# OpenGene/gencore

Measured on AMD Instinct MI355X. Metric: consensus read-pairs/sec (whole node) + clustering HBM GB/s vs roofline, higher is better.
Workload: dtype u8

## Files before the change

gencore_amd/csrc/engine.hip:

```cpp
#include <hip/hip_runtime.h>
#include <hip/hip_ext.h>
#include <cstdio>
#include <cstdlib>
#include <algorithm>
#include <cstring>
#include <ctime>
#include <string>
#include <vector>

#include "gce_entry.h"
#include "gce_kernels.hpp"
#include "gce_params.hpp"
#include "gce_pair2.hpp"
#include "gce_vote.hpp"
#include "gce_deep.hpp"
#include "gce_output.hpp"
#include "gce_depth.hpp"
#include "gce_inflate.hpp"
#include "gce_deflate.hpp"

namespace {

static thread_local double t_alloc_s = 0.0; static thread_local long t_alloc_n = 0; static thread_local size_t t_alloc_bytes = 0;
static inline double mono_s() { struct timespec ts; clock_gettime(CLOCK_MONOTONIC, &ts); return (double)ts.tv_sec + 1e-9 * (double)ts.tv_nsec; }
long long g_dev_live = 0, g_dev_peak = 0;
static int64_t g_pass_idx_ctr[4] = {0, 0, 0, 0};
inline void dev_bytes_add(long long d) {
    const long long now = __atomic_add_fetch(&g_dev_live, d, __ATOMIC_RELAXED);
    long long pk = __atomic_load_n(&g_dev_peak, __ATOMIC_RELAXED);
    while (now > pk && !__atomic_compare_exchange_n(&g_dev_peak, &pk, now, true, __ATOMIC_RELAXED, __ATOMIC_RELAXED)) {}
}
struct DevBuf {
    void *p = nullptr; size_t cap = 0;
    static size_t padded(size_t bytes) { return bytes + bytes / 8 + 256; }
    hipError_t ensure(size_t bytes) { return bytes <= cap && p ? hipSuccess : take(padded(bytes)); }
    hipError_t take(size_t want) {
        const double t0 = mono_s();
        release();
        hipError_t e = hipMalloc(&p, want);
        if (e == hipSuccess) { cap = want; dev_bytes_add((long long)want); } else p = nullptr;
        t_alloc_s += mono_s() - t0; t_alloc_n++; t_alloc_bytes += want;
        return e;
    }
    void release() { if (p) { (void)hipFree(p); dev_bytes_add(-(long long)cap); } p = nullptr; cap = 0; }
    template <class T> T *as() const { return (T *)p; }
};
struct ScopedBuf : DevBuf { ~ScopedBuf() { release(); } };
template <class T> inline hipError_t ensure_as(DevBuf &d, T *&dst, size_t bytes) { const hipError_t r = d.ensure(bytes); dst = d.as<T>(); return r; }

enum { EV_START = 0, EV_CLUSTER, EV_CSR, EV_DESCRIBE, EV_PAIRING, EV_SCORE, EV_CONSENSUS, EV_FINISH, EV_OUTPUT, EV_COUNT };

}

#include "gce_devstream.hpp"

struct HostRaw {
    uint8_t *p = nullptr; size_t n = 0, cap = 0;
    ~HostRaw() { free(p); }
    void resize(size_t k) { if (k > cap) { free(p); p = (uint8_t *)malloc(k ? k : 1); cap = p ? k : 0; } n = p ? k : 0; }
    uint8_t *data() { return p; }
    size_t size() const { return n; }
    bool empty() const { return n == 0; }
};

struct gce_engine {
    gce_params prm{};
    bool vote_off_logged = false;
    std::vector<uint32_t> target_len;
    std::string err;
    hipStream_t stream = nullptr;
    hipEvent_t ev[EV_COUNT]{};
    std::vector<DevBuf> ref_buf; std::vector<const uint8_t *> ref_ptr; std::vector<int64_t> ref_len, ref_win; bool have_win = false;
    DevBuf d_ref_ptr, d_ref_len, d_ref_win, d_target_len, d_target_cum;
    std::vector<const uint8_t *> up_ref_ptr; std::vector<int64_t> up_ref_len, up_win; std::vector<uint32_t> up_tl; const void *up_dev[5]{}; bool up_valid = false;
    std::vector<gce_core> h_core; std::vector<uint64_t> h_qoff, h_coff, h_soff, h_loff, h_mioff;
    std::vector<char> h_qname, h_mi; std::vector<uint32_t> h_cigar; std::vector<uint8_t> h_seq, h_qual, h_nmt; std::vector<int32_t> h_nm; std::vector<uint64_t> h_tick;
    std::vector<int32_t> h_ev_tid, h_ev_pos;
    bool have_mi = false, have_tick = false, have_events = false, host_mode = false, device_mode = false, processed = false;
    bool reserved = false; hipStream_t up_stream = nullptr; std::vector<hipEvent_t> up_events;
    hipStream_t aux_stream = nullptr; hipEvent_t aux_ev[4]{};
    size_t rs_n = 0, rs_q = 0, rs_c = 0, rs_s = 0, rs_l = 0, st_n = 0, st_q = 0, st_c = 0, st_s = 0, st_l = 0, st_m = 0; bool dev_concat = false;
    gce_batch dev_batch{};
    DevBuf b_core, b_qoff, b_qname, b_coff, b_cigar, b_soff, b_seq, b_loff, b_qual, b_nm, b_nmt, b_mioff, b_mi, b_tick;
    DevBuf uinfo, rdesc, spatch, slot, score, out_flag, orec, out_index, nmx;
    DevBuf o_src, o_kind, o_qsrc, o_nm, o_fr, o_rr, o_mate, o_soff, o_qoff, o_seq, o_qual, o_key, o_rec, o_ksoff, o_kqoff, o_krow, o_rank64, o_part3, ref_ascii;
    int64_t n_out = 0; size_t out_seq_bytes = 0, out_qual_bytes = 0; int dev_error = 0; uint32_t dev_error_read = 0;
    DevBuf lrec, lout, bhdr, blk_base, ev_tid, ev_pos, ev_read, table, toff;
    DevBuf raw, rw_tmp, rw_ncig, rw_nmpos, rw_rsize, rw_roff, rw_body; RecIdx rw;
    size_t raw_n = 0; bool raw_mode = false; int64_t raw_records = 0; uint64_t raw_body_bytes = 0;
    int64_t idx_ctr[4] = {0, 0, 0, 0};
    DevBuf z_comp, z_dir, z_err; size_t z_n = 0; std::vector<InfDir> z_members;
    DevBuf zo_slots, zo_sizes, zo_off, zo_out; uint64_t zo_bytes = 0;
    DevBuf sf_text; uint64_t sf_bytes = 0; int64_t raw_body_nrec = -1;
    std::vector<gce_engine *> mirrors;
    DevBuf sh_tickall, sh_shard, sh_flag, sh_sel, sh_core, sh_qoff, sh_coff, sh_soff, sh_loff, sh_nm, sh_nmt, sh_mioff, sh_tick, sh_roff, sh_nmpos, sh_keys, sh_stage; int64_t shard_n = -1;
    bool shard_cut_done = false;
    bool tab_clean = false; const void *tab_clean_ptr = nullptr; size_t tab_clean_cap = 0;
    DevBuf cl_ikey, cl_start, cl_n, cl_npairs, cl_ngroups, cl_gbase, cl_nresult, cl_hasumi, cl_tier;
    DevBuf members, sorted, pl, pr, pu, pg, gpl, gpr, grp_begin, grp_n, gl_cluster, g_begin, g_np;
    DevBuf slow_args, deep_list, k64, slow_list, left_list, pf_flag, pf_list, pq_flag, pq_list, p16_flag, p16_list, pd_slab, gen_flag, gen_list, score_list, gw, vlive, vb_start, rp_left, rp_right, rp_merge, rp_rmerge, rp_umi, rp_umilen, rp_state, rp_supp, rp_nm, rp_qsl, rp_qsr, scan_part, si;
    StreamInfo h_si{};
    void *si_pin = nullptr, *si_pin_dev = nullptr; unsigned long long si_seq = 0;
    gce_timing timing{};
    int64_t n = 0, n_pre = 0;
    DevBuf dp_binoff, dp_regoff, dp_rs, dp_re, dp_pmax, dp_sorted, dp_depth, dp_bed, dp_where;
    std::vector<int64_t> h_binoff, h_depth_pre, h_depth_post, h_bed_pre, h_bed_post; int64_t payload_words = 0;
    std::vector<uint8_t> r_kind; HostRaw r_seq, r_qual; std::vector<uint32_t> r_src, r_qsrc, r_mate; std::vector<int32_t> r_nm; std::vector<int16_t> r_fr, r_rr;
    std::vector<uint64_t> r_soff, r_qoff;
};

static int fail(gce_engine *e, int code, const std::string &msg) { if (e) e->err = msg; return code; }
#define HIPCHK(call) do { hipError_t _e = (call); if (_e != hipSuccess) return fail(e, _e == hipErrorOutOfMemory ? GCE_ERR_OOM : GCE_ERR_HIP, std::string(#call) + ": " + hipGetErrorString(_e)); } while (0)

extern "C" {

int gce_abi_version(void) { return GCE_ABI_VERSION; }

void gce_params_default(gce_params *p) {
    memset(p, 0, sizeof *p);
    p->abi_version = GCE_ABI_VERSION;
    p->proper_umi_diff_threshold = 1; p->unproper_umi_diff_threshold = 0; p->duplex_mismatch_threshold = 2;
    p->cluster_size_req = 1; p->base_score_req = 6; p->high_quality = 30; p->moderate_quality = 20; p->low_quality = 15;
    p->score_high = 8; p->score_moderate = 6; p->score_low = 4; p->score_bad = 2;
    p->skip_low_complexity_cluster_threshold = 1000; p->flush_period = 10000; p->score_percent_req = 0.8;
}

void gce_detect_umi_prefix(const char *q, char out[32]) {
    memset(out, 0, 32);
    if (strstr(q, "umi_")) strcpy(out, "umi");
    else if (strstr(q, "UMI_")) strcpy(out, "UMI");
}

const char *gce_status_message(int s) {
    switch (s) {
    case GCE_OK: return "ok";
    case GCE_ERR_INVALID: return "invalid argument or call order";
    case GCE_ERR_NO_DEVICE: return "no HIP device available (this engine has no CPU fallback)";
    case GCE_ERR_HIP: return "HIP runtime error";
    case GCE_ERR_OOM: return "out of device memory";
    case GCE_ERR_UNSORTED: return "ERROR: the input is unsorted. Please sort the input first.";
    case GCE_ERR_UMI_MISMATCH: return "The UMI of a read pair should be identical";
    case GCE_ERR_NM_MISSING: return "NM tag missing on a consensus template whose mismatch count changed";
    case GCE_ERR_UMI_PARSE: return "UMI parse: substr start beyond the end of the read name";
    case GCE_ERR_QNAME_SHORT: return "copyQName ERROR: desitination qname is shorter";
    case GCE_ERR_REF_WINDOW: return "reference window: a clustered read lies outside the bases staged for its contig";
    default: return "unknown status";
    }
}

const char *gce_last_error(const gce_engine *e) { return e ? e->err.c_str() : "null engine"; }

int gce_create(const gce_params *params, gce_engine **out) {
    if (!params || !out || params->abi_version != GCE_ABI_VERSION) return GCE_ERR_INVALID;
    if (params->proper_umi_diff_threshold < 0 || params->unproper_umi_diff_threshold < 0 || params->flush_period < 0) return GCE_ERR_INVALID;
    int ndev = 0;
    if (hipGetDeviceCount(&ndev) != hipSuccess || ndev <= 0 || params->device >= ndev) return GCE_ERR_NO_DEVICE;
    gce_engine *e = new gce_engine();
    e->prm = *params;
    if (e->prm.flush_period == 0) e->prm.flush_period = 10000;
    if (params->n_targets > 0 && params->target_len) e->target_len.assign(params->target_len, params->target_len + params->n_targets);
    e->prm.target_len = nullptr;
    if (hipSetDevice(params->device) != hipSuccess || hipStreamCreate(&e->stream) != hipSuccess) { delete e; return GCE_ERR_HIP; }
    for (auto &v : e->ev) (void)hipEventCreate(&v);
    *out = e;
    return GCE_OK;
}

void gce_destroy(gce_engine *e) {
    if (!e) return;
    (void)hipSetDevice(e->prm.device);
    (void)hipStreamSynchronize(e->stream);
    DevBuf *all[] = {&e->d_ref_ptr, &e->d_ref_len, &e->d_ref_win, &e->d_target_len, &e->d_target_cum, &e->b_core, &e->b_qoff, &e->b_qname, &e->b_coff, &e->b_cigar, &e->b_soff,
                     &e->b_seq, &e->b_loff, &e->b_qual, &e->b_nm, &e->b_nmt, &e->b_mioff, &e->b_mi, &e->b_tick, &e->uinfo, &e->rdesc, &e->spatch,
                     &e->slot, &e->score, &e->out_flag, &e->orec, &e->out_index, &e->nmx, &e->o_src, &e->o_kind, &e->o_qsrc, &e->o_nm, &e->o_fr, &e->o_rr, &e->o_mate,
                     &e->o_key, &e->o_rec, &e->o_ksoff, &e->o_kqoff, &e->o_krow, &e->o_rank64, &e->o_part3, &e->o_soff, &e->o_qoff, &e->o_seq, &e->o_qual, &e->ref_ascii, &e->lrec, &e->lout, &e->bhdr,
                     &e->blk_base, &e->ev_tid, &e->ev_pos, &e->ev_read, &e->table, &e->toff, &e->cl_ikey, &e->cl_start, &e->cl_n,
                     &e->cl_npairs, &e->cl_ngroups, &e->cl_gbase, &e->cl_nresult, &e->cl_hasumi, &e->cl_tier, &e->members, &e->sorted, &e->pl, &e->pr, &e->pu,
                     &e->pg, &e->gpl, &e->gpr, &e->grp_begin, &e->grp_n, &e->gl_cluster, &e->g_begin, &e->g_np, &e->deep_list, &e->k64, &e->slow_list, &e->pf_flag, &e->pf_list, &e->pq_flag, &e->pq_list, &e->left_list, &e->slow_args, &e->pd_slab, &e->gen_flag, &e->gen_list, &e->score_list, &e->gw, &e->vlive, &e->vb_start, &e->rp_left, &e->rp_right, &e->rp_merge, &e->rp_rmerge,
                     &e->rp_umi, &e->rp_umilen, &e->rp_state, &e->rp_supp, &e->rp_nm, &e->rp_qsl, &e->rp_qsr, &e->scan_part, &e->si};
    for (auto *b : all) b->release();
    for (DevBuf *b : {&e->z_comp, &e->z_dir, &e->z_err, &e->raw, &e->rw_tmp, &e->rw_ncig, &e->rw_nmpos, &e->rw_rsize, &e->rw_roff, &e->rw_body, &e->sf_text}) b->release();
    e->rw.release();
    for (DevBuf *b : {&e->zo_slots, &e->zo_sizes, &e->zo_off, &e->zo_out, &e->p16_flag, &e->p16_list}) b->release();
    for (DevBuf *b : {&e->sh_tickall, &e->sh_shard, &e->sh_flag, &e->sh_sel, &e->sh_core, &e->sh_qoff, &e->sh_coff, &e->sh_soff, &e->sh_loff, &e->sh_nm, &e->sh_nmt, &e->sh_mioff, &e->sh_tick, &e->sh_roff, &e->sh_nmpos, &e->sh_keys, &e->sh_stage}) b->release();
    for (DevBuf *b : {&e->dp_binoff, &e->dp_regoff, &e->dp_rs, &e->dp_re, &e->dp_pmax, &e->dp_sorted, &e->dp_depth, &e->dp_bed, &e->dp_where}) b->release();
    for (auto ev : e->up_events) (void)hipEventDestroy(ev);
    if (e->up_stream) { (void)hipStreamSynchronize(e->up_stream); (void)hipStreamDestroy(e->up_stream); }
    if (e->aux_stream) { (void)hipStreamSynchronize(e->aux_stream); (void)hipStreamDestroy(e->aux_stream); }
    for (auto &v : e->aux_ev) if (v) (void)hipEventDestroy(v);
    for (auto &b : e->ref_buf) b.release();
    for (auto &v : e->ev) if (v) (void)hipEventDestroy(v);
    if (e->stream) (void)hipStreamDestroy(e->stream);
    if (e->si_pin) (void)hipHostFree(e->si_pin);
    delete e;
}

void gce_pack_reference(const char *bases, int64_t n, uint8_t *out) {
    memset(out, 0, (size_t)((n + 1) / 2));
    for (int64_t i = 0; i < n; i++) {
        uint8_t code;
        switch (bases[i]) { case 'A': code = 1; break; case 'T': code = 2; break; case 'C': code = 3; break; case 'G': code = 4; break; default: code = 0; }
        out[i >> 1] |= (i & 1) ? (uint8_t)(code << 4) : code;
    }
}

int gce_set_reference(gce_engine *e, int32_t tid, const uint8_t *nibbles, int64_t n_bases) {
    if (!e || tid < 0 || n_bases < 0) return GCE_ERR_INVALID;
    (void)hipSetDevice(e->prm.device);
    if ((size_t)tid >= e->ref_buf.size()) { e->ref_buf.resize(tid + 1); e->ref_ptr.resize(tid + 1, nullptr); e->ref_len.resize(tid + 1, 0); }
    if (!nibbles) { e->ref_ptr[tid] = nullptr; e->ref_len[tid] = 0; return GCE_OK; }
    size_t bytes = (size_t)((n_bases + 1) / 2);
    HIPCHK(e->ref_buf[tid].ensure(bytes + 16));
    hipPointerAttribute_t attr; bool is_dev = hipPointerGetAttributes(&attr, nibbles) == hipSuccess && attr.type == hipMemoryTypeDevice;
    (void)hipGetLastError();
    HIPCHK(hipMemcpyAsync(e->ref_buf[tid].p, nibbles, bytes, is_dev ? hipMemcpyDeviceToDevice : hipMemcpyHostToDevice, e->stream));
    HIPCHK(hipStreamSynchronize(e->stream));
    e->ref_ptr[tid] = e->ref_buf[tid].as<uint8_t>(); e->ref_len[tid] = n_bases;
    if (2 * (size_t)tid + 1 < e->ref_win.size()) e->ref_win[2 * tid] = e->ref_win[2 * tid + 1] = 0;
    return GCE_OK;
}

int gce_set_reference_ascii(gce_engine *e, int32_t tid, const char *bases, int64_t n_bases) {
    if (!e || tid < 0 || n_bases < 0 || (!bases && n_bases > 0)) return GCE_ERR_INVALID;
    (void)hipSetDevice(e->prm.device);
    if ((size_t)tid >= e->ref_buf.size()) { e->ref_buf.resize(tid + 1); e->ref_ptr.resize(tid + 1, nullptr); e->ref_len.resize(tid + 1, 0); }
    const size_t bytes = (size_t)((n_bases + 1) / 2);
    HIPCHK(e->ref_buf[tid].ensure(bytes + 16));
    HIPCHK(e->ref_ascii.ensure((size_t)n_bases + 16));
    hipPointerAttribute_t attr; const bool is_dev = hipPointerGetAttributes(&attr, bases) == hipSuccess && attr.type == hipMemoryTypeDevice;
    (void)hipGetLastError();
    if (n_bases) {
        HIPCHK(hipMemcpyAsync(e->ref_ascii.p, bases, (size_t)n_bases, is_dev ? hipMemcpyDeviceToDevice : hipMemcpyHostToDevice, e->stream));
        const unsigned grid = (unsigned)std::min<uint64_t>((bytes + 255) / 256, 65535u * 4u);
        hipLaunchKernelGGL(k_pack_reference, dim3(grid), dim3(256), 0, e->stream, (const char *)e->ref_ascii.p, n_bases, e->ref_buf[tid].as<uint8_t>());
    }
    HIPCHK(hipStreamSynchronize(e->stream));
    HIPCHK(hipGetLastError());
    e->ref_ptr[tid] = e->ref_buf[tid].as<uint8_t>(); e->ref_len[tid] = n_bases;
    if (2 * (size_t)tid + 1 < e->ref_win.size()) e->ref_win[2 * tid] = e->ref_win[2 * tid + 1] = 0;
    return GCE_OK;
}

int gce_set_reference_window(gce_engine *e, int32_t tid, int64_t contig_len, int64_t win_start, const char *bases, int64_t n_bases) {
    if (!e || tid < 0 || contig_len < 0 || win_start < 0 || (win_start & 1) || n_bases < 0 || win_start + n_bases > contig_len || (!bases && n_bases > 0)) return GCE_ERR_INVALID;
    const int rc = gce_set_reference_ascii(e, tid, bases, n_bases);
    if (rc != GCE_OK) return rc;
    if (e->ref_win.size() < 2 * e->ref_ptr.size()) e->ref_win.resize(2 * e->ref_ptr.size(), 0);
    e->ref_ptr[tid] = e->ref_buf[tid].as<uint8_t>() - (win_start >> 1);
    e->ref_len[tid] = contig_len;
    e->ref_win[2 * tid] = win_start; e->ref_win[2 * tid + 1] = win_start + n_bases;
    e->have_win = true;
    return GCE_OK;
}

int gce_reset(gce_engine *e) {
    if (!e) return GCE_ERR_INVALID;
    e->h_core.clear(); e->h_qoff.clear(); e->h_coff.clear(); e->h_soff.clear(); e->h_loff.clear(); e->h_mioff.clear(); e->h_tick.clear();
    e->h_qname.clear(); e->h_mi.clear(); e->h_cigar.clear(); e->h_seq.clear(); e->h_qual.clear(); e->h_nmt.clear(); e->h_nm.clear();
    e->have_mi = e->have_tick = e->host_mode = e->device_mode = e->processed = e->raw_mode = false; e->n = 0; e->n_out = 0; e->shard_n = -1; e->shard_cut_done = false;
    e->st_n = e->st_q = e->st_c = e->st_s = e->st_l = e->st_m = 0; e->dev_concat = false;
    return GCE_OK;
}

int gce_set_flush_events(gce_engine *e, int32_t n_events, const int32_t *ev_tid, const int32_t *ev_pos) {
    if (!e || n_events < 0 || (n_events > 0 && (!ev_tid || !ev_pos))) return GCE_ERR_INVALID;
    e->h_ev_tid.assign(ev_tid, ev_tid + n_events); e->h_ev_pos.assign(ev_pos, ev_pos + n_events);
    e->have_events = true;
    return GCE_OK;
}

struct PreExtra { long long v[6]; };
__global__ void k_fold_stats(StreamInfo *si, PreExtra x) {
    const int k = threadIdx.x;
    if (k < 6) {
        long long a = 0, c = 0;
        for (int q = 0; q < GCE_PRE_SLOTS; q++) { a += si->pre_slot[q][k]; c += si->post_slot[q][k]; si->pre_slot[q][k] = 0; si->post_slot[q][k] = 0; }
        si->pre[k] += a + x.v[k]; si->post[k] += c;
    }
}
__global__ void k_first_contig_ge(const gce_core *core, int64_t n, int32_t maxc, unsigned int *out) {
    const int64_t i = (int64_t)blockIdx.x * blockDim.x + threadIdx.x;
    const bool hit = i < n && core[i].tid >= maxc;
    const unsigned long long m = __ballot(hit);
    if (m && (threadIdx.x & 63) == 0) { const unsigned int v = (unsigned int)(i + __ffsll((long long)m) - 1); if (v < *(volatile unsigned int *)out) atomicMin(out, v); }
}

__global__ void k_add_u64(uint64_t *a, uint64_t n, uint64_t base) {
    const uint64_t i = (uint64_t)blockIdx.x * blockDim.x + threadIdx.x;
    if (i < n) a[i] += base;
}

int gce_reserve(gce_engine *e, int64_t n_reads, size_t qname_bytes, size_t cigar_words, size_t seq_bytes, size_t qual_bytes) {
    if (!e || n_reads < 0) return GCE_ERR_INVALID;
    if (e->processed) gce_reset(e);
    if (e->host_mode || e->device_mode) return fail(e, GCE_ERR_INVALID, "gce_reserve after a submit");
    (void)hipSetDevice(e->prm.device);
    const size_t n = (size_t)n_reads;
    HIPCHK(e->b_core.ensure(n * sizeof(gce_core) + 64)); HIPCHK(e->b_qoff.ensure(n * 8 + 64)); HIPCHK(e->b_coff.ensure(n * 8 + 64));
    HIPCHK(e->b_soff.ensure(n * 8 + 64)); HIPCHK(e->b_loff.ensure(n * 8 + 64)); HIPCHK(e->b_nm.ensure(n * 4 + 64)); HIPCHK(e->b_nmt.ensure(n + 64));
    HIPCHK(e->b_qname.ensure(qname_bytes + 64)); HIPCHK(e->b_cigar.ensure(cigar_words * 4 + 64)); HIPCHK(e->b_seq.ensure(seq_bytes + 64)); HIPCHK(e->b_qual.ensure(qual_bytes + 64));
    if (!e->up_stream) HIPCHK(hipStreamCreate(&e->up_stream));
    e->reserved = true; e->rs_n = n; e->rs_q = qname_bytes; e->rs_c = cigar_words; e->rs_s = seq_bytes; e->rs_l = qual_bytes;
    e->st_n = e->st_q = e->st_c = e->st_s = e->st_l = 0;
    return GCE_OK;
}

static hipError_t grow_keep(DevBuf &d, size_t used, size_t need, hipStream_t s) {
    if (d.p && need <= d.cap) return hipSuccess;
    DevBuf nb;
    hipError_t rc = nb.ensure(need + need / 2 + 256);
    if (rc != hipSuccess) return rc;
    if (used && d.p && (rc = hipMemcpyAsync(nb.p, d.p, used, hipMemcpyDeviceToDevice, s)) != hipSuccess) { nb.release(); return rc; }
    if ((rc = hipStreamSynchronize(s)) != hipSuccess) { nb.release(); return rc; }
    d.release(); d = nb;
    return hipSuccess;
}
__global__ void k_rebase_mioff(uint64_t *a, uint64_t n, uint64_t base) {
    const uint64_t i = (uint64_t)blockIdx.x * blockDim.x + threadIdx.x;
    if (i < n && a[i] != 0xFFFFFFFFFFFFFFFFull) a[i] += base;
}

static int append_batch(gce_engine *e, const gce_batch *b, hipMemcpyKind kind) {
    const size_t n = (size_t)b->n_reads;
    if (!n) return GCE_OK;
    if (!b->core || !b->qname_off || !b->qname || !b->cigar_off || !b->seq_off || !b->seq || !b->qual_off || !b->qual || !b->nm || !b->nm_type)
        return fail(e, GCE_ERR_INVALID, "null array in gce_batch");
    if (e->st_n > 0 && (b->tick != nullptr) != e->have_tick) return fail(e, GCE_ERR_INVALID, "gce_batch.tick must be given for every batch of a stream or for none");
    if (!e->up_stream) HIPCHK(hipStreamCreate(&e->up_stream));
    hipStream_t s = e->up_stream;
    const bool mi = b->mi && b->mi_off;
    HIPCHK(grow_keep(e->b_core, e->st_n * sizeof(gce_core), (e->st_n + n) * sizeof(gce_core) + 64, s)); HIPCHK(grow_keep(e->b_nm, e->st_n * 4, (e->st_n + n) * 4 + 64, s)); HIPCHK(grow_keep(e->b_nmt, e->st_n, e->st_n + n + 64, s));
    HIPCHK(grow_keep(e->b_qoff, e->st_n * 8, (e->st_n + n) * 8 + 64, s)); HIPCHK(grow_keep(e->b_coff, e->st_n * 8, (e->st_n + n) * 8 + 64, s));
    HIPCHK(grow_keep(e->b_soff, e->st_n * 8, (e->st_n + n) * 8 + 64, s)); HIPCHK(grow_keep(e->b_loff, e->st_n * 8, (e->st_n + n) * 8 + 64, s));
    HIPCHK(grow_keep(e->b_qname, e->st_q, e->st_q + b->qname_bytes + 64, s)); HIPCHK(grow_keep(e->b_cigar, e->st_c * 4, (e->st_c + b->cigar_words) * 4 + 64, s));
    HIPCHK(grow_keep(e->b_seq, e->st_s, e->st_s + b->seq_bytes + 64, s)); HIPCHK(grow_keep(e->b_qual, e->st_l, e->st_l + b->qual_bytes + 64, s));
    auto cp = [&](DevBuf &d, size_t at, const void *src, size_t bytes) { return bytes ? hipMemcpyAsync((char *)d.p + at, src, bytes, kind, s) : hipSuccess; };
    HIPCHK(cp(e->b_core, e->st_n * sizeof(gce_core), b->core, n * sizeof(gce_core)));
    HIPCHK(cp(e->b_nm, e->st_n * 4, b->nm, n * 4)); HIPCHK(cp(e->b_nmt, e->st_n, b->nm_type, n));
    HIPCHK(cp(e->b_qoff, e->st_n * 8, b->qname_off, n * 8)); HIPCHK(cp(e->b_coff, e->st_n * 8, b->cigar_off, n * 8));
    HIPCHK(cp(e->b_soff, e->st_n * 8, b->seq_off, n * 8)); HIPCHK(cp(e->b_loff, e->st_n * 8, b->qual_off, n * 8));
    HIPCHK(cp(e->b_qname, e->st_q, b->qname, b->qname_bytes)); HIPCHK(cp(e->b_cigar, e->st_c * 4, b->cigar, b->cigar_words * 4));
    HIPCHK(cp(e->b_seq, e->st_s, b->seq, b->seq_bytes)); HIPCHK(cp(e->b_qual, e->st_l, b->qual, b->qual_bytes));
    const unsigned nb = (unsigned)((n + 255) / 256);
    if (e->st_q) hipLaunchKernelGGL(k_add_u64, dim3(nb), dim3(256), 0, s, e->b_qoff.as<uint64_t>() + e->st_n, (uint64_t)n, (uint64_t)e->st_q);
    if (e->st_c) hipLaunchKernelGGL(k_add_u64, dim3(nb), dim3(256), 0, s, e->b_coff.as<uint64_t>() + e->st_n, (uint64_t)n, (uint64_t)e->st_c);
    if (e->st_s) hipLaunchKernelGGL(k_add_u64, dim3(nb), dim3(256), 0, s, e->b_soff.as<uint64_t>() + e->st_n, (uint64_t)n, (uint64_t)e->st_s);
    if (e->st_l) hipLaunchKernelGGL(k_add_u64, dim3(nb), dim3(256), 0, s, e->b_loff.as<uint64_t>() + e->st_n, (uint64_t)n, (uint64_t)e->st_l);
    if (b->tick) {
        HIPCHK(grow_keep(e->b_tick, e->st_n * 8, (e->st_n + n) * 8 + 64, s));
        HIPCHK(cp(e->b_tick, e->st_n * 8, b->tick, n * 8));
        e->have_tick = true;
    }
    if (mi || e->have_mi) {
        const bool first = !e->have_mi;
        HIPCHK(grow_keep(e->b_mioff, first ? 0 : e->st_n * 8, (e->st_n + n) * 8 + 64, s));
        if (first && e->st_n) HIPCHK(hipMemsetAsync(e->b_mioff.p, 0xFF, e->st_n * 8, s));
        if (mi) {
            HIPCHK(grow_keep(e->b_mi, e->st_m, e->st_m + b->mi_bytes + 64, s));
            HIPCHK(cp(e->b_mioff, e->st_n * 8, b->mi_off, n * 8)); HIPCHK(cp(e->b_mi, e->st_m, b->mi, b->mi_bytes));
            if (e->st_m) hipLaunchKernelGGL(k_rebase_mioff, dim3(nb), dim3(256), 0, s, e->b_mioff.as<uint64_t>() + e->st_n, (uint64_t)n, (uint64_t)e->st_m);
            e->st_m += b->mi_bytes;
        } else HIPCHK(hipMemsetAsync((char *)e->b_mioff.p + e->st_n * 8, 0xFF, n * 8, s));
        e->have_mi = true;
    }
    e->st_n += n; e->st_q += b->qname_bytes; e->st_c += b->cigar_words; e->st_s += b->seq_bytes; e->st_l += b->qual_bytes;
    return GCE_OK;
}
static void publish_own_copy(gce_engine *e) {
    gce_batch &d = e->dev_batch; memset(&d, 0, sizeof d);
    d.n_reads = (int64_t)e->st_n; d.core = e->b_core.as<gce_core>();
    d.qname_off = e->b_qoff.as<uint64_t>(); d.qname = e->b_qname.as<char>(); d.cigar_off = e->b_coff.as<uint64_t>(); d.cigar = e->b_cigar.as<uint32_t>();
    d.seq_off = e->b_soff.as<uint64_t>(); d.seq = e->b_seq.as<uint8_t>(); d.qual_off = e->b_loff.as<uint64_t>(); d.qual = e->b_qual.as<uint8_t>();
    d.nm = e->b_nm.as<int32_t>(); d.nm_type = e->b_nmt.as<uint8_t>();
    d.qname_bytes = e->st_q; d.cigar_words = e->st_c; d.seq_bytes = e->st_s; d.qual_bytes = e->st_l;
    if (e->have_mi) { d.mi_off = e->b_mioff.as<uint64_t>(); d.mi = e->b_mi.as<char>(); d.mi_bytes = e->st_m; }
    if (e->have_tick) d.tick = e->b_tick.as<uint64_t>();
}

int gce_submit_async(gce_engine *e, const gce_batch *b, int32_t *ticket) {
    if (!e || !b || b->n_reads < 0) return GCE_ERR_INVALID;
    if (!e->reserved) return fail(e, GCE_ERR_INVALID, "gce_submit_async needs gce_reserve");
    if (e->device_mode && !e->processed) return fail(e, GCE_ERR_INVALID, "gce_submit after gce_submit_device");
    if (e->processed) gce_reset(e);
    (void)hipSetDevice(e->prm.device);
    e->host_mode = true;
    int rc = append_batch(e, b, hipMemcpyHostToDevice);
    if (rc != GCE_OK) return rc;
    hipEvent_t ev;
    HIPCHK(hipEventCreateWithFlags(&ev, hipEventDisableTiming));
    HIPCHK(hipEventRecord(ev, e->up_stream));
    e->up_events.push_back(ev);
    if (ticket) *ticket = (int32_t)e->up_events.size() - 1;
    return GCE_OK;
}

int gce_submit_wait(gce_engine *e, int32_t ticket) {
    if (!e || ticket < 0 || (size_t)ticket >= e->up_events.size()) return GCE_ERR_INVALID;
    HIPCHK(hipEventSynchronize(e->up_events[ticket]));
    for (gce_engine *m : e->mirrors)
        if ((size_t)ticket < m->up_events.size() && hipEventSynchronize(m->up_events[ticket]) != hipSuccess) return fail(e, GCE_ERR_HIP, "mirror engine: copy failed");
    return GCE_OK;
}

int gce_submit(gce_engine *e, const gce_batch *b) {
    if (!e || !b || b->n_reads < 0) return GCE_ERR_INVALID;
    if (e->device_mode && !e->processed) return fail(e, GCE_ERR_INVALID, "gce_submit after gce_submit_device");
    if (e->reserved) {
        int32_t t; int rc = gce_submit_async(e, b, &t);
        return rc != GCE_OK ? rc : gce_submit_wait(e, t);
    }
    if (e->processed) gce_reset(e);
    e->host_mode = true;
    const int64_t n = b->n_reads;
    if (n == 0) return GCE_OK;
    if (!b->core || !b->qname_off || !b->qname || !b->cigar_off || !b->seq_off || !b->seq || !b->qual_off || !b->qual || !b->nm || !b->nm_type)
        return fail(e, GCE_ERR_INVALID, "null array in gce_batch");
    const size_t old = e->h_core.size();
    if (old > 0 && (b->tick != nullptr) != e->have_tick) return fail(e, GCE_ERR_INVALID, "gce_batch.tick must be given for every batch of a stream or for none");
    const uint64_t q0 = e->h_qname.size(), c0 = e->h_cigar.size(), s0 = e->h_seq.size(), l0 = e->h_qual.size(), m0 = e->h_mi.size();
    e->h_core.insert(e->h_core.end(), b->core, b->core + n);
    e->h_nm.insert(e->h_nm.end(), b->nm, b->nm + n);
    e->h_nmt.insert(e->h_nmt.end(), b->nm_type, b->nm_type + n);
    e->h_qname.insert(e->h_qname.end(), b->qname, b->qname + b->qname_bytes);
    if (b->cigar_words) e->h_cigar.insert(e->h_cigar.end(), b->cigar, b->cigar + b->cigar_words);
    e->h_seq.insert(e->h_seq.end(), b->seq, b->seq + b->seq_bytes);
    e->h_qual.insert(e->h_qual.end(), b->qual, b->qual + b->qual_bytes);
    if (b->tick) { e->h_tick.insert(e->h_tick.end(), b->tick, b->tick + n); e->have_tick = true; }
    bool mi = b->mi && b->mi_off;
    if (mi && !e->have_mi) { e->h_mioff.assign(old, UINT64_MAX); e->have_mi = true; }
    if (mi) e->h_mi.insert(e->h_mi.end(), b->mi, b->mi + b->mi_bytes);
    e->h_qoff.reserve(old + n); e->h_coff.reserve(old + n); e->h_soff.reserve(old + n); e->h_loff.reserve(old + n);
    for (int64_t i = 0; i < n; i++) {
        e->h_qoff.push_back(b->qname_off[i] + q0); e->h_coff.push_back(b->cigar_off[i] + c0);
        e->h_soff.push_back(b->seq_off[i] + s0); e->h_loff.push_back(b->qual_off[i] + l0);
        if (e->have_mi) e->h_mioff.push_back(mi && b->mi_off[i] != UINT64_MAX ? b->mi_off[i] + m0 : UINT64_MAX);
    }
    return GCE_OK;
}

int gce_submit_device(gce_engine *e, const gce_batch *b) {
    if (!e || !b || b->n_reads < 0) return GCE_ERR_INVALID;
    if (e->processed) gce_reset(e);
    if (e->host_mode) return fail(e, GCE_ERR_INVALID, "gce_submit_device after gce_submit");
    (void)hipSetDevice(e->prm.device);
    if (!e->device_mode) {
        e->device_mode = true; e->dev_concat = false;
        e->dev_batch = *b;
        e->have_tick = b->tick != nullptr;
        return GCE_OK;
    }
    int rc;
    if (!e->dev_concat) {
        const gce_batch first = e->dev_batch;
        e->st_n = e->st_q = e->st_c = e->st_s = e->st_l = e->st_m = 0; e->have_tick = false; e->have_mi = false;
        if ((rc = append_batch(e, &first, hipMemcpyDeviceToDevice)) != GCE_OK) return rc;
        e->dev_concat = true;
    }
    if ((rc = append_batch(e, b, hipMemcpyDeviceToDevice)) != GCE_OK) return rc;
    HIPCHK(hipStreamSynchronize(e->up_stream));
    publish_own_copy(e);
    return GCE_OK;
}

static int upload(gce_engine *e) {
    if (e->reserved) {
        HIPCHK(hipStreamSynchronize(e->up_stream));
        for (auto ev : e->up_events) (void)hipEventDestroy(ev);
        e->up_events.clear();
        publish_own_copy(e);
        return GCE_OK;
    }
    struct { DevBuf *d; const void *src; size_t bytes; const void **dst; } items[] = {
        {&e->b_core, e->h_core.data(), e->h_core.size() * sizeof(gce_core), (const void **)&e->dev_batch.core},
        {&e->b_qoff, e->h_qoff.data(), e->h_qoff.size() * 8, (const void **)&e->dev_batch.qname_off},
        {&e->b_qname, e->h_qname.data(), e->h_qname.size(), (const void **)&e->dev_batch.qname},
        {&e->b_coff, e->h_coff.data(), e->h_coff.size() * 8, (const void **)&e->dev_batch.cigar_off},
        {&e->b_cigar, e->h_cigar.data(), e->h_cigar.size() * 4, (const void **)&e->dev_batch.cigar},
        {&e->b_soff, e->h_soff.data(), e->h_soff.size() * 8, (const void **)&e->dev_batch.seq_off},
        {&e->b_seq, e->h_seq.data(), e->h_seq.size(), (const void **)&e->dev_batch.seq},
        {&e->b_loff, e->h_loff.data(), e->h_loff.size() * 8, (const void **)&e->dev_batch.qual_off},
        {&e->b_qual, e->h_qual.data(), e->h_qual.size(), (const void **)&e->dev_batch.qual},
        {&e->b_nm, e->h_nm.data(), e->h_nm.size() * 4, (const void **)&e->dev_batch.nm},
        {&e->b_nmt, e->h_nmt.data(), e->h_nmt.size(), (const void **)&e->dev_batch.nm_type},
        {&e->b_mioff, e->h_mioff.data(), e->h_mioff.size() * 8, (const void **)&e->dev_batch.mi_off},
        {&e->b_mi, e->h_mi.data(), e->h_mi.size(), (const void **)&e->dev_batch.mi},
        {&e->b_tick, e->h_tick.data(), e->h_tick.size() * 8, (const void **)&e->dev_batch.tick},
    };
    for (auto &it : items) {
        HIPCHK(it.d->ensure(it.bytes + 64));
        if (it.bytes) HIPCHK(hipMemcpyAsync(it.d->p, it.src, it.bytes, hipMemcpyHostToDevice, e->stream));
        *it.dst = it.bytes ? it.d->p : nullptr;
    }
    if (!e->have_mi) { e->dev_batch.mi = nullptr; e->dev_batch.mi_off = nullptr; }
    if (!e->have_tick) e->dev_batch.tick = nullptr;
    e->dev_batch.n_reads = (int64_t)e->h_core.size();
    e->dev_batch.qname_bytes = e->h_qname.size(); e->dev_batch.cigar_words = e->h_cigar.size();
    e->dev_batch.seq_bytes = e->h_seq.size(); e->dev_batch.qual_bytes = e->h_qual.size(); e->dev_batch.mi_bytes = e->h_mi.size();
    if (e->h_cigar.empty()) e->dev_batch.cigar = e->b_cigar.as<uint32_t>();
    return GCE_OK;
}

__global__ __launch_bounds__(256) void k_publish_si(const StreamInfo *si, StreamInfo *host, unsigned long long *flag, unsigned long long seq) {
    const uint32_t *src = reinterpret_cast<const uint32_t *>(si);
    uint32_t *dst = reinterpret_cast<uint32_t *>(host);
    for (unsigned i = threadIdx.x; i < sizeof(StreamInfo) / 4; i += 256) dst[i] = src[i];
    __threadfence_system();
    __syncthreads();
    if (threadIdx.x == 0) __hip_atomic_store(flag, seq, __ATOMIC_RELEASE, __HIP_MEMORY_SCOPE_SYSTEM);
}
static_assert(sizeof(StreamInfo) % 4 == 0, "k_publish_si copies words");
static int read_si_begin(gce_engine *e, unsigned long long *seq_out) {
    *seq_out = 0;
    static const bool sync_copy = getenv("GCE_SYNC_COPY") != nullptr;
    if (!sync_copy && !e->si_pin) {
        void *hp = nullptr;
        if (hipHostMalloc(&hp, sizeof(StreamInfo) + 64, hipHostMallocMapped | hipHostMallocCoherent | hipHostMallocPortable) == hipSuccess) {
            void *dp = nullptr;
            if (hipHostGetDevicePointer(&dp, hp, 0) == hipSuccess) { memset(hp, 0, sizeof(StreamInfo) + 64); e->si_pin = hp; e->si_pin_dev = dp; }
            else (void)hipHostFree(hp);
        }
        (void)hipGetLastError();
    }
    if (!sync_copy && e->si_pin) {
        unsigned long long *dflag = reinterpret_cast<unsigned long long *>(reinterpret_cast<char *>(e->si_pin_dev) + ((sizeof(StreamInfo) + 7) & ~size_t(7)));
        const unsigned long long seq = ++e->si_seq;
        hipLaunchKernelGGL(k_publish_si, dim3(1), dim3(256), 0, e->stream, (const StreamInfo *)e->si.p, reinterpret_cast<StreamInfo *>(e->si_pin_dev), dflag, seq);
        HIPCHK(hipGetLastError());
        *seq_out = seq;
    }
    return GCE_OK;
}
static int read_si_end(gce_engine *e, unsigned long long seq) {
    bool published = false;
    if (seq) {
        StreamInfo *hs = reinterpret_cast<StreamInfo *>(e->si_pin);
        unsigned long long *hflag = reinterpret_cast<unsigned long long *>(reinterpret_cast<char *>(e->si_pin) + ((sizeof(StreamInfo) + 7) & ~size_t(7)));
        for (unsigned spins = 1;; spins++) {
            if (__atomic_load_n(hflag, __ATOMIC_ACQUIRE) == seq) { published = true; break; }
            if ((spins & 0x3FFF) == 0) {
                const hipError_t q = hipStreamQuery(e->stream);
                if (q == hipSuccess) { published = __atomic_load_n(hflag, __ATOMIC_ACQUIRE) == seq; break; }
                if (q != hipErrorNotReady) HIPCHK(q);
            }
            __builtin_ia32_pause();
        }
        if (published) memcpy(&e->h_si, hs, sizeof(StreamInfo));
    }
    if (!published) {
        HIPCHK(hipMemcpyAsync(&e->h_si, e->si.p, sizeof(StreamInfo), hipMemcpyDeviceToHost, e->stream));
        HIPCHK(hipStreamSynchronize(e->stream));
    }
    for (int k = 0; k < 6; k++) for (int q = 0; q < GCE_PRE_SLOTS; q++) { e->h_si.pre[k] += e->h_si.pre_slot[q][k]; e->h_si.post[k] += e->h_si.post_slot[q][k]; }
    if (e->h_si.err_key != ~0ull) { e->dev_error = -(int)(e->h_si.err_key & 0xFF); e->dev_error_read = (uint32_t)(e->h_si.err_key >> 8); }
    return GCE_OK;
}
static int read_si(gce_engine *e) {
    unsigned long long seq = 0;
    const int rc = read_si_begin(e, &seq);
    return rc != GCE_OK ? rc : read_si_end(e, seq);
}

static inline unsigned cdiv(uint64_t a, uint64_t b) { return (unsigned)((a + b - 1) / b); }
static const bool g_record_events = getenv("GCE_RECORD_EVENTS") != nullptr;
#define LAUNCH_EV(kernel, grid, block, stream, ev, ...) do { \
    if (g_record_events) { hipLaunchKernelGGL(kernel, grid, block, 0, stream, __VA_ARGS__); (void)hipEventRecord(ev, stream); } \
    else hipExtLaunchKernelGGL(kernel, grid, block, 0, stream, nullptr, ev, 0, __VA_ARGS__); } while (0)

struct FillSeg { void *p; uint64_t bytes; uint32_t val; uint32_t pad; };
struct FillArgs { FillSeg s[6]; };
__global__ __launch_bounds__(256) void k_fill_many(FillArgs a) {
    const FillSeg g = a.s[blockIdx.y];
    const uint64_t n16 = g.bytes >> 4;
    const uint32_t v = g.val * 0x01010101u;
    uint4 *q = reinterpret_cast<uint4 *>(g.p);
    for (uint64_t i = (uint64_t)blockIdx.x * 256 + threadIdx.x; i < n16; i += (uint64_t)gridDim.x * 256) q[i] = make_uint4(v, v, v, v);
    if (blockIdx.x == 0 && threadIdx.x < (g.bytes & 15)) reinterpret_cast<uint8_t *>(g.p)[(n16 << 4) + threadIdx.x] = (uint8_t)g.val;
}
static void fill_many(hipStream_t s, std::initializer_list<FillSeg> segs) {
    FillArgs a{}; int n = 0; uint64_t mx = 0;
    for (const FillSeg &g : segs) { a.s[n++] = g; mx = std::max<uint64_t>(mx, g.bytes); }
    const unsigned gx = (unsigned)std::min<uint64_t>(std::max<uint64_t>((mx >> 4) / (256 * 8), 1), 2048);
    hipLaunchKernelGGL(k_fill_many, dim3(gx, (unsigned)n), dim3(256), 0, s, a);
}

static int aux_ready(gce_engine *e) {
    if (e->aux_stream) return GCE_OK;
    HIPCHK(hipStreamCreateWithFlags(&e->aux_stream, hipStreamNonBlocking));
    for (auto &v : e->aux_ev) HIPCHK(hipEventCreateWithFlags(&v, hipEventDisableTiming));
    return GCE_OK;
}

#ifdef GCE_SI_CANARY
static void si_canary(gce_engine *e, const char *phase) {
    StreamInfo hs; (void)hipStreamSynchronize(e->stream); (void)hipMemcpy(&hs, e->si.p, sizeof hs, hipMemcpyDeviceToHost);
    for (int k = 14; k < GCE_STATS_WORDS; k++) if ((k != 15 && hs.post[k] != 0) || hs.pre[k] < 0 || hs.post[k] < 0) { fprintf(stderr, "SI_CANARY after %s: pre[%d] = %lld post[%d] = %lld\n", phase, k, hs.pre[k], k, hs.post[k]); break; }
}
#define CANARY(x) si_canary(e, x)
#else
#define CANARY(x) do { } while (0)
#endif

static int gce_process_impl(gce_engine *e);
int gce_process(gce_engine *e) {
    static const bool tlog = getenv("GCE_RAW_TIMING") != nullptr;
    if (!tlog) return gce_process_impl(e);
    const double a0 = t_alloc_s, w0 = mono_s(); const long n0 = t_alloc_n; const size_t b0 = t_alloc_bytes;
    const int rc = gce_process_impl(e);
    fprintf(stderr, "gce_process (device %d): %.4f s wall, of it %.4f s in %ld hipMalloc / hipFree calls for %.2f GB; kernels %.1f ms\n", e ? e->prm.device : -1, mono_s() - w0, t_alloc_s - a0, t_alloc_n - n0,
            (double)(t_alloc_bytes - b0) / 1e9, e ? e->timing.total_ms : 0.0);
    return rc;
}
#define TAKE(buf, dst, bytes) HIPCHK(ensure_as(e->buf, dst, bytes))
namespace {
struct Step {
    gce_engine *const e; const hipStream_t s; const gce_batch &hb;
    DevBatch b{}; DevParams p{}; Work w{}; OutTable o{};
    int64_t N = 0; size_t n1 = 1; uint32_t C = 0, NG = 0;
    PreExtra pre_extra{};
    int64_t n_sblk = 0, max_events = 0; unsigned nblk_N = 0;
    bool si_behind_describe = false;
    explicit Step(gce_engine *e_) : e(e_), s(e_->stream), hb(e_->dev_batch) {}

    int check_and_cut() {
        if (!e->host_mode && !e->device_mode) return fail(e, GCE_ERR_INVALID, "nothing submitted");
        if (e->processed) return fail(e, GCE_ERR_INVALID, "gce_process called twice without a new submit (the stream was mutated in place)");
        if (e->have_tick && !e->have_events) return fail(e, GCE_ERR_INVALID, "gce_batch.tick needs gce_set_flush_events");
        (void)hipSetDevice(e->prm.device);
        int rc;
        if (e->host_mode && (rc = upload(e)) != GCE_OK) return rc;
        N = hb.n_reads;
        e->n_pre = N;
        if (e->prm.max_contig > 0 && N > 0 && !e->shard_cut_done) {
            HIPCHK(e->si.ensure(sizeof(StreamInfo)));
            unsigned int first = NONE32;
            HIPCHK(hipMemcpyAsync(e->si.p, &first, 4, hipMemcpyHostToDevice, s));
            hipLaunchKernelGGL(k_first_contig_ge, dim3((unsigned)((N + 255) / 256)), dim3(256), 0, s, hb.core, N, e->prm.max_contig, (unsigned int *)e->si.p);
            HIPCHK(hipMemcpyAsync(&first, e->si.p, 4, hipMemcpyDeviceToHost, s));
            HIPCHK(hipStreamSynchronize(s));
            if (first != NONE32) {
                gce_core c2; int32_t nm = 0; uint8_t nmt = 0;
                HIPCHK(hipMemcpy(&c2, hb.core + first, sizeof(gce_core), hipMemcpyDeviceToHost));
                HIPCHK(hipMemcpy(&nm, hb.nm + first, 4, hipMemcpyDeviceToHost)); HIPCHK(hipMemcpy(&nmt, hb.nm_type + first, 1, hipMemcpyDeviceToHost));
                const int mism = nmt != 0 ? nm : 0;
                pre_extra.v[0] = 1; pre_extra.v[1] = c2.l_qseq; pre_extra.v[4] = mism; pre_extra.v[5] = mism > 0;
                N = (int64_t)first; e->n_pre = N + 1;
            }
        }
        e->n = N; e->n_out = 0; e->out_seq_bytes = e->out_qual_bytes = 0; e->dev_error = 0; e->dev_error_read = 0;
        e->processed = true;
        memset(&e->timing, 0, sizeof e->timing);
        memset(&e->h_si, 0, sizeof e->h_si);
        if (N >= (int64_t)0xFFFFFC00ll) return fail(e, GCE_ERR_INVALID, "more than 2^32 reads in one engine");
        if ((uint64_t)(VB_MINW + 3) * (uint64_t)(N > 0 ? N : 0) >= (1ull << 32)) return fail(e, GCE_ERR_INVALID, "too many reads in one engine for the batch scan of k_vote (weight sum >= 2^32)");
        n1 = (size_t)(N > 0 ? N : 1);
        b.n = N; b.core = hb.core; b.qname_off = hb.qname_off; b.qname = hb.qname; b.cigar_off = hb.cigar_off; b.cigar = hb.cigar;
        b.seq_off = hb.seq_off; b.seq = hb.seq; b.qual_off = hb.qual_off; b.qual = hb.qual; b.nm = hb.nm; b.nm_type = hb.nm_type;
        b.mi_off = hb.mi_off; b.mi = hb.mi; b.tick = e->have_tick ? hb.tick : nullptr;
        return GCE_OK;
    }

    int stage_constants() {
        const int nref = (int)e->ref_ptr.size();
        HIPCHK(e->d_ref_ptr.ensure((size_t)(nref + 1) * 8)); HIPCHK(e->d_ref_len.ensure((size_t)(nref + 1) * 8));
        HIPCHK(e->d_target_len.ensure(e->target_len.size() * 4 + 4));
        HIPCHK(e->d_target_cum.ensure(e->target_len.size() * 8 + 8));
        std::vector<int64_t> win;
        if (e->have_win && nref) {
            win.assign(2 * (size_t)nref, 0);
            for (int t = 0; t < nref; t++) { const bool wd = 2 * (size_t)t + 1 < e->ref_win.size() && e->ref_win[2 * t + 1] > 0; win[2 * t] = wd ? e->ref_win[2 * t] : 0; win[2 * t + 1] = wd ? e->ref_win[2 * t + 1] : e->ref_len[t]; }
            HIPCHK(e->d_ref_win.ensure(win.size() * 8));
        }
        const void *dev_now[5] = {e->d_ref_ptr.p, e->d_ref_len.p, e->d_target_len.p, e->d_target_cum.p, e->d_ref_win.p};
        const bool same = e->up_valid && e->up_ref_ptr == e->ref_ptr && e->up_ref_len == e->ref_len && e->up_tl == e->target_len && e->up_win == win && memcmp(dev_now, e->up_dev, sizeof dev_now) == 0;
        if (!same) {
            e->up_valid = false;
            if (nref) {
                HIPCHK(hipMemcpyAsync(e->d_ref_ptr.p, e->ref_ptr.data(), (size_t)nref * 8, hipMemcpyHostToDevice, s));
                HIPCHK(hipMemcpyAsync(e->d_ref_len.p, e->ref_len.data(), (size_t)nref * 8, hipMemcpyHostToDevice, s));
            }
            std::vector<uint64_t> cum(e->target_len.size()); uint64_t acc = 0;
            for (size_t i = 0; i < cum.size(); i++) { cum[i] = acc; acc += e->target_len[i]; }
            if (!e->target_len.empty()) {
                HIPCHK(hipMemcpyAsync(e->d_target_len.p, e->target_len.data(), e->target_len.size() * 4, hipMemcpyHostToDevice, s));
                HIPCHK(hipMemcpyAsync(e->d_target_cum.p, cum.data(), cum.size() * 8, hipMemcpyHostToDevice, s));
            }
            if (!win.empty()) HIPCHK(hipMemcpyAsync(e->d_ref_win.p, win.data(), win.size() * 8, hipMemcpyHostToDevice, s));
            HIPCHK(hipStreamSynchronize(s));
            e->up_ref_ptr = e->ref_ptr; e->up_ref_len = e->ref_len; e->up_tl = e->target_len; e->up_win = win; memcpy(e->up_dev, dev_now, sizeof dev_now);
            e->up_valid = true;
        }
        p.target_len = e->d_target_len.as<uint32_t>(); p.target_cum = e->target_len.empty() ? nullptr : e->d_target_cum.as<uint64_t>();
        p.n_ref = nref; p.ref_data = e->d_ref_ptr.as<const uint8_t *>(); p.ref_len = e->d_ref_len.as<int64_t>(); p.ref_win = win.empty() ? nullptr : e->d_ref_win.as<int64_t>();
        return GCE_OK;
    }

    int size_by_reads() {
        const uint64_t T = ((uint64_t)n1 + (uint64_t)n1 / 4 + 2 * SCAN_TILE - 1) / SCAN_TILE * SCAN_TILE;
        const char *vote_off_why = nullptr;
        if (make_dev_params(e->prm, e->target_len, e->have_tick, N, T, &p, &vote_off_why) != GCE_OK) return fail(e, GCE_ERR_INVALID, "score constants out of range");
        if (vote_off_why && !e->vote_off_logged) {
            e->vote_off_logged = true;
            fprintf(stderr, "gencore_amd: k_vote off for this engine (%s): every group goes to the per-side kernels\n", vote_off_why);
        }
        n_sblk = (N + SB_READS - 1) / SB_READS;
        w.n_sblk = n_sblk;
        max_events = e->have_tick ? (int64_t)e->h_ev_tid.size() + 2 : (p.tick_offset % p.period + N) / p.period + 2;
        w.max_events = (int)max_events;
        w.tsize = T; w.tinv = 1.0 / (double)T;
        const size_t qual_bytes = hb.qual_bytes ? hb.qual_bytes : 1;
        const size_t nsb1 = (size_t)(n_sblk > 0 ? n_sblk : 1);
        TAKE(uinfo, w.uinfo, n1 * 8); TAKE(rdesc, w.rdesc, n1 * sizeof(ReadDescP)); TAKE(spatch, w.spatch, n1 * 4); TAKE(slot, w.slot, n1 * 4 + 16); TAKE(score, w.score, qual_bytes + 64);
        TAKE(out_flag, w.out_flag, n1 + 144);        TAKE(nmx, w.nmx, n1 * 4); TAKE(orec, w.orec, n1 * sizeof(OutRec)); TAKE(out_index, w.out_index, n1 * 4);
        TAKE(lrec, w.lrec, nsb1 * SB_READS * sizeof(LeadRec)); TAKE(lout, w.lout, nsb1 * SB_READS * sizeof(LeadOut));
        TAKE(bhdr, w.bhdr, nsb1 * sizeof(BlkHdr)); TAKE(blk_base, w.blk_base, nsb1 * 4);
        TAKE(ev_tid, w.ev_tid, (size_t)max_events * 4); TAKE(ev_pos, w.ev_pos, (size_t)max_events * 4); TAKE(ev_read, w.ev_read, (size_t)max_events * 4);
        TAKE(table, w.tab, T * sizeof(TabEntry)); TAKE(toff, w.toff, T * 4);
        TAKE(k64, w.k64, n1 * 24); TAKE(members, w.members, n1 * 4); TAKE(sorted, w.sorted, n1 * 4); TAKE(pl, w.pl, n1 * 4); TAKE(pr, w.pr, n1 * 4); TAKE(pu, w.pu, n1 * 4); TAKE(pg, w.pg, n1 * 4);
        TAKE(gpl, w.gpl, n1 * 4); TAKE(gpr, w.gpr, n1 * 4); TAKE(grp_begin, w.grp_begin, n1 * 4); TAKE(grp_n, w.grp_n, n1 * 4); TAKE(slow_list, w.slow_list, n1 * 4 + 64);
        TAKE(deep_list, w.deep_list, (n1 / 64 + 64) * 16);
        nblk_N = cdiv(n1, SCAN_TILE);
        TAKE(scan_part, w.scan_part, std::max<size_t>(2 * nsb1, (size_t)2 * nblk_N) * 8 + 16);
        TAKE(si, w.si, sizeof(StreamInfo));
        TAKE(cl_ikey, w.cl_ikey, n1 * 4); TAKE(cl_start, w.cl_start, n1 * 4); TAKE(cl_n, w.cl_n, n1 * 4);

        StreamInfo init{}; init.first_unmapped = NONE32; init.err_key = ~0ull; init.lq_min = 0x7FFFFFFF; init.lq_max = -1;
        if (e->have_tick) { init.n_events = init.n_events_a = (int)e->h_ev_tid.size(); }
        HIPCHK(hipMemcpyAsync(e->si.p, &init, sizeof init, hipMemcpyHostToDevice, s));
        if (e->have_tick && !e->h_ev_tid.empty()) {
            HIPCHK(hipMemcpyAsync(e->ev_tid.p, e->h_ev_tid.data(), e->h_ev_tid.size() * 4, hipMemcpyHostToDevice, s));
            HIPCHK(hipMemcpyAsync(e->ev_pos.p, e->h_ev_pos.data(), e->h_ev_pos.size() * 4, hipMemcpyHostToDevice, s));
        }
        if (!e->tab_clean || e->tab_clean_ptr != e->table.p || e->tab_clean_cap != e->table.cap) {
            HIPCHK(hipMemsetAsync(e->table.p, 0, e->table.cap, s));
            e->tab_clean_ptr = e->table.p; e->tab_clean_cap = e->table.cap;
        }
        e->tab_clean = false;
        HIPCHK(hipEventRecord(e->ev[EV_START], s));
        HIPCHK(hipMemsetAsync(e->out_flag.p, 0, n1, s));
        return GCE_OK;
    }

    int form_clusters() {
        if (N > 0) LAUNCH_EV(k_cluster, dim3((unsigned)n_sblk), dim3(SB_T), s, e->ev[EV_CLUSTER], b, p, w);
#ifdef CL_PROF
        dump_cluster_prof();
#endif
        if (N <= 0) HIPCHK(hipEventRecord(e->ev[EV_CLUSTER], s));
        CANARY("EV_CLUSTER");
        if (N > 0) {
            if (!e->have_tick) {
                hipLaunchKernelGGL(k_blk_scan, dim3(1), dim3(1024), 0, s, w, p);
                hipLaunchKernelGGL(k_events, dim3(cdiv(max_events, EV_T / 64)), dim3(EV_T), 0, s, b, p, w);
            }
            const unsigned nb4 = cdiv(n_sblk, 4);
            hipLaunchKernelGGL(k_leaders, dim3(nb4), dim3(256), 0, s, b, p, w);
            hipLaunchKernelGGL(k_num_reduce, dim3(nb4), dim3(256), 0, s, w, p.nw_cb);
            hipLaunchKernelGGL(k_scan_partials, dim3(1), dim3(1024), 0, s, w.scan_part, (uint64_t)nb4, &w.si->n_clusters, (unsigned long long *)nullptr);
            hipLaunchKernelGGL(k_num_apply, dim3(nb4), dim3(256), 0, s, w);
            LAUNCH_EV(k_scatter, dim3((unsigned)n_sblk), dim3(SB_T), s, e->ev[EV_CSR], N, w);
        } else HIPCHK(hipEventRecord(e->ev[EV_CSR], s));
        CANARY("EV_CSR");
        return GCE_OK;
    }

    int describe() {
        int rc;
        unsigned long long si_seq1 = 0;
        if ((rc = read_si_begin(e, &si_seq1)) != GCE_OK) return rc;
        if (N > 0) {
#ifndef GCE_DESCRIBE_BLOCKS
#define GCE_DESCRIBE_BLOCKS 32768
#endif
            const int64_t n_tiles = (N + 255) / 256;
            int tpb = (int)((n_tiles + GCE_DESCRIBE_BLOCKS - 1) / GCE_DESCRIBE_BLOCKS); if (tpb < 1) tpb = 1;
            LAUNCH_EV(k_describe, dim3(cdiv(n_tiles, tpb)), dim3(256), s, e->ev[EV_DESCRIBE], b, p, w, tpb);
        } else HIPCHK(hipEventRecord(e->ev[EV_DESCRIBE], s));
        CANARY("EV_DESCRIBE");
        if ((rc = read_si_end(e, si_seq1)) != GCE_OK) return rc;
        HIPCHK(hipGetLastError());
        e->tab_clean = true;
        C = (uint32_t)e->h_si.n_clusters;
        const size_t c1 = C ? C : 1;
        TAKE(cl_npairs, w.cl_npairs, c1 * 4); TAKE(cl_ngroups, w.cl_ngroups, c1 * 4); TAKE(cl_gbase, w.cl_gbase, c1 * 4); TAKE(cl_nresult, w.cl_nresult, c1 * 4);
        TAKE(cl_hasumi, w.cl_hasumi, c1); TAKE(cl_tier, w.cl_tier, c1);
        return GCE_OK;
    }

    void compact_flags(uint8_t *flag, uint32_t *list, unsigned long long *count) {
        const unsigned nbc = cdiv(C, SCAN_TILE);
        hipLaunchKernelGGL(k_flag_reduce, dim3(nbc), dim3(256), 0, s, (const uint8_t *)flag, (uint64_t)C, w.scan_part);
        hipLaunchKernelGGL(k_scan_partials, dim3(1), dim3(1024), 0, s, w.scan_part, (uint64_t)nbc, count, (unsigned long long *)nullptr);
        hipLaunchKernelGGL(k_flag_apply, dim3(nbc), dim3(256), 0, s, (const uint8_t *)flag, (uint64_t)C, (const uint64_t *)w.scan_part, list);
    }

    int pair_clusters() {
        if (!(C > 0 && e->dev_error == 0)) { HIPCHK(hipEventRecord(e->ev[EV_PAIRING], s)); return GCE_OK; }
        int rc;
        const size_t c1 = C;
        TAKE(left_list, w.left_list, c1 * 4 + 64);
        TAKE(pf_flag, w.pf_flag, c1 + 64); TAKE(pf_list, w.pf_list, c1 * 4); TAKE(pq_flag, w.pq_flag, c1 + 64); TAKE(pq_list, w.pq_list, c1 * 4); TAKE(p16_flag, w.p16_flag, c1 + 64); TAKE(p16_list, w.p16_list, c1 * 4);
        const bool pair_classes = (double)N > 10.0 * (double)C;
        if (!pair_classes) fill_many(s, {FillSeg{e->pf_flag.p, c1, 0u, 0u}, FillSeg{e->pq_flag.p, c1, 0u, 0u}});
        const unsigned nbc = cdiv(C, SCAN_TILE);
#ifdef PS_STOP
        return time_pairing_sub_and_stop();
#endif
        HIPCHK(e->pd_slab.ensure(PD_BIG_BLOCKS * PD_SLAB));
        if (pair_classes) {
            hipLaunchKernelGGL(k_pair_class_reduce, dim3(nbc), dim3(256), 0, s, (const uint32_t *)w.cl_n, C, w.scan_part);
            hipLaunchKernelGGL(k_scan_partials, dim3(1), dim3(1024), 0, s, w.scan_part, (uint64_t)nbc, &w.si->n_p16_items, &w.si->n_pq_items);
            hipLaunchKernelGGL(k_pair_class_apply, dim3(nbc), dim3(256), 0, s, (const uint32_t *)w.cl_n, C, (const uint64_t *)w.scan_part, w.p16_list, w.pq_list, w.pf_list, w.si);
            static const bool tiers_aux = getenv("GCE_NO_AUX_STREAM") == nullptr;
            hipStream_t s2 = s;
            if (tiers_aux) {
                if ((rc = aux_ready(e)) != GCE_OK) return rc;
                s2 = e->aux_stream;
                HIPCHK(hipEventRecord(e->aux_ev[0], s));
                HIPCHK(hipStreamWaitEvent(s2, e->aux_ev[0], 0));
            }
            hipLaunchKernelGGL(k_pairing_fast, dim3(2048), dim3(256), 0, s2, b, p, w, C, (const uint32_t *)w.pf_list);
            hipLaunchKernelGGL(k_pairing_deep<false>, dim3(256), dim3(PD_T), 0, s2, b, p, w, (uint8_t *)nullptr);
            if (tiers_aux) HIPCHK(hipEventRecord(e->aux_ev[1], s2));
            hipLaunchKernelGGL(k_pairing_sub<16>, dim3(cdiv(C, 4 * WAVES_PER_BLOCK)), dim3(256), 0, s, b, p, w, C, (const uint32_t *)w.p16_list, (const unsigned long long *)&w.si->n_p16_items, w.pq_flag, 1);
            hipLaunchKernelGGL(k_pairing_sub<32>, dim3(cdiv(C, 2 * WAVES_PER_BLOCK)), dim3(256), 0, s, b, p, w, C, (const uint32_t *)w.pq_list, (const unsigned long long *)&w.si->n_pq_items, w.pf_flag, 1);
            if (tiers_aux) HIPCHK(hipStreamWaitEvent(s, e->aux_ev[1], 0));
        } else {
            hipLaunchKernelGGL(k_pairing_sub<16>, dim3(cdiv(C, 4 * WAVES_PER_BLOCK)), dim3(256), 0, s, b, p, w, C, (const uint32_t *)nullptr, (const unsigned long long *)nullptr, w.pq_flag, 0);
            compact_flags(w.pq_flag, w.pq_list, &w.si->n_pq_items);
            hipLaunchKernelGGL(k_pairing_sub<32>, dim3(cdiv(C, 2 * WAVES_PER_BLOCK)), dim3(256), 0, s, b, p, w, C, (const uint32_t *)w.pq_list, (const unsigned long long *)&w.si->n_pq_items, w.pf_flag, 0);
            compact_flags(w.pf_flag, w.pf_list, &w.si->n_pf_items);
            hipLaunchKernelGGL(k_pairing_fast, dim3(2048), dim3(256), 0, s, b, p, w, C, (const uint32_t *)w.pf_list);
            hipLaunchKernelGGL(k_pairing_deep<false>, dim3(256), dim3(PD_T), 0, s, b, p, w, (uint8_t *)nullptr);
        }
        hipLaunchKernelGGL(k_pairing_deep<true>, dim3(PD_BIG_BLOCKS), dim3(PD_T), 0, s, b, p, w, e->pd_slab.as<uint8_t>());
        hipLaunchKernelGGL(k_pairing_slow<0>, dim3(1024), dim3(256), 0, s, b, p, w);
        hipLaunchKernelGGL(k_pairing_slow<1>, dim3(1024, 16), dim3(256), 0, s, b, p, w);
        hipLaunchKernelGGL(k_pairing_slow<2>, dim3(1024), dim3(256), 0, s, b, p, w);
        hipLaunchKernelGGL(k_scan_reduce, dim3(nbc), dim3(256), 0, s, (const uint32_t *)w.cl_ngroups, (uint64_t)C, w.scan_part);
        hipLaunchKernelGGL(k_scan_partials, dim3(1), dim3(1024), 0, s, w.scan_part, (uint64_t)nbc, &w.si->n_pairs , &w.si->n_groups);
        hipLaunchKernelGGL(k_u32_apply, dim3(nbc), dim3(256), 0, s, (const uint32_t *)w.cl_ngroups, w.cl_gbase, (uint64_t)C, (const uint64_t *)w.scan_part);
        TAKE(gl_cluster, w.gl_cluster, n1 * 4); TAKE(g_begin, w.g_begin, n1 * 4); TAKE(g_np, w.g_np, n1 * 4); TAKE(gw, w.gw, n1 * 8); TAKE(vlive, w.vlive, n1 * 16);
        const size_t vb_cap = ((VB_MINW + 3) * n1) / VB_W + 8;
        TAKE(vb_start, w.vb_start, vb_cap * 4);
        HIPCHK(hipMemsetAsync(e->vb_start.p, 0xFF, vb_cap * 4, s));
        hipLaunchKernelGGL(k_group_fill, dim3(cdiv(C, 256)), dim3(256), 0, s, p, w, C, (uint32_t)VB_W, (uint32_t)VB_MINW);
        hipLaunchKernelGGL(k_u64_reduce, dim3(nblk_N), dim3(256), 0, s, (const uint64_t *)w.gw, (const unsigned long long *)&w.si->n_groups, w.scan_part);
        hipLaunchKernelGGL(k_u64_partials, dim3(1), dim3(1024), 0, s, w.scan_part, (const unsigned long long *)&w.si->n_groups, &w.si->vote_weight, &w.si->n_live);
        LAUNCH_EV(k_vote_batches, dim3(nblk_N), dim3(256), s, e->ev[EV_PAIRING], w, (const unsigned long long *)&w.si->n_groups, (const uint64_t *)w.scan_part);
        CANARY("EV_PAIRING");
        if ((rc = read_si(e)) != GCE_OK) return rc;
        HIPCHK(hipGetLastError());
        si_behind_describe = true;
        NG = (uint32_t)e->h_si.n_groups;
        return GCE_OK;
    }

    int consensus() {
        int rc;
        const size_t g1 = NG ? NG : 1;
        TAKE(gen_list, w.gen_list, g1 * 8); TAKE(gen_flag, w.gen_flag, g1 * 2 + 64);
        TAKE(score_list, w.score_list, n1 * 4 + 64);
        TAKE(rp_left, w.rp_left, g1 * 4); TAKE(rp_right, w.rp_right, g1 * 4); TAKE(rp_merge, w.rp_merge, g1 * 4); TAKE(rp_rmerge, w.rp_rmerge, g1 * 4); TAKE(rp_umi, w.rp_umi, g1 * 8);
        TAKE(rp_umilen, w.rp_umilen, g1 * 2); TAKE(rp_state, w.rp_state, g1); TAKE(rp_supp, w.rp_supp, g1 * 4); TAKE(rp_nm, w.rp_nm, g1 * 8); TAKE(rp_qsl, w.rp_qsl, g1 * 4); TAKE(rp_qsr, w.rp_qsr, g1 * 4);
        if (NG > 0 && e->dev_error == 0) {
            {
                SlowArgs sa; sa.b = b; sa.p = p; sa.w = w;
                HIPCHK(e->slow_args.ensure(sizeof sa));
                HIPCHK(hipMemcpyAsync(e->slow_args.p, &sa, sizeof sa, hipMemcpyHostToDevice, s));
            }
            fill_many(s, {FillSeg{e->gen_flag.p, g1 * 2, 0u, 0u},
                          FillSeg{e->rp_nm.p, g1 * 8, 0xFFu, 0u},
                          FillSeg{e->rp_left.p, g1 * 4, 0xFFu, 0u}, FillSeg{e->rp_right.p, g1 * 4, 0xFFu, 0u}});
            const uint32_t n_live = (uint32_t)e->h_si.n_live;
#ifdef VB_XCD
            const unsigned nbatch = (((unsigned)(e->h_si.vote_weight / VB_W) + 1u) + 7u) & ~7u;
#else
            const unsigned nbatch = (unsigned)(e->h_si.vote_weight / VB_W) + 1u;
#endif
#ifdef VB_STOP
            return time_vote_and_stop(nbatch, n_live);
#endif
            LAUNCH_EV(k_vote, dim3(nbatch), dim3(VB_T), s, e->ev[EV_SCORE], b, p, w, n_live);
            CANARY("EV_SCORE");
            const bool deep_stream = ((double)N > 48.0 * (double)NG || getenv("GCE_FORCE_AUX_STREAM")) && !getenv("GCE_NO_AUX_STREAM");
            const unsigned cf_cap = deep_stream ? 32768u : 4096u, sc2_cap = deep_stream ? 16384u : 2048u;
            const unsigned cf_grid = std::min<unsigned>(cdiv(2ull * NG, WAVES_PER_BLOCK), cf_cap);
            const unsigned sc2_grid = std::min<unsigned>(cdiv(N, 2 * WAVES_PER_BLOCK * 64), sc2_cap);
            if (deep_stream) {
                if ((rc = aux_ready(e)) != GCE_OK) return rc;
                HIPCHK(hipEventRecord(e->aux_ev[0], s));
                HIPCHK(hipStreamWaitEvent(e->aux_stream, e->aux_ev[0], 0));
                hipLaunchKernelGGL(k_score2, dim3(sc2_grid), dim3(256), 0, e->aux_stream, b, p, w);
                HIPCHK(hipEventRecord(e->aux_ev[1], e->aux_stream));
                hipLaunchKernelGGL(k_deep_prepare, dim3(1024), dim3(256), 0, s, b, p, w);
                HIPCHK(hipStreamWaitEvent(s, e->aux_ev[1], 0));
                hipLaunchKernelGGL(k_consensus_fast, dim3(cf_grid), dim3(256), 0, s, b, p, w);
            } else {
                hipLaunchKernelGGL(k_score2, dim3(sc2_grid), dim3(256), 0, s, b, p, w);
                hipLaunchKernelGGL(k_deep_prepare, dim3(1024), dim3(256), 0, s, b, p, w);
                hipLaunchKernelGGL(k_consensus_fast, dim3(cf_grid), dim3(256), 0, s, b, p, w);
            }
            hipLaunchKernelGGL(k_vote_deep, dim3(1024), dim3(DV_T), 0, s, b, p, w);
            LAUNCH_EV(k_consensus_slow, dim3(512), dim3(256), s, e->ev[EV_CONSENSUS], (const SlowArgs *)e->slow_args.p);
            CANARY("EV_CONSENSUS");
            hipLaunchKernelGGL(k_group_tail, dim3(cdiv(NG, 256)), dim3(256), 0, s, b, p, w, NG);
            if (!p.disable_duplex) {
                hipLaunchKernelGGL(k_finish_screen, dim3(cdiv(C, 256)), dim3(256), 0, s, w, C, w.pf_flag);
                compact_flags(w.pf_flag, w.pf_list, &w.si->n_pf_items);
                hipLaunchKernelGGL(k_finish, dim3(4096), dim3(256), 0, s, b, p, w, (const uint32_t *)w.pf_list, (const unsigned long long *)&w.si->n_pf_items);
            }
        } else { HIPCHK(hipEventRecord(e->ev[EV_SCORE], s)); HIPCHK(hipEventRecord(e->ev[EV_CONSENSUS], s)); }
#ifdef VB_PROF
        dump_vote_prof();
#endif
        return GCE_OK;
    }

    int output_table() {
        HIPCHK(hipEventRecord(e->ev[EV_FINISH], s));
        CANARY("EV_FINISH");
        if (N > 0 && e->dev_error == 0) {
            size_t seq_cap = hb.seq_bytes + 16 * n1 + 64, qual_cap = hb.qual_bytes + 16 * n1 + 64;
            if (e->h_si.lq_max >= 0) {
                const size_t lqm = (size_t)e->h_si.lq_max;
                seq_cap = std::min(seq_cap, n1 * ((lqm + 1) / 2 + 16) + 64); qual_cap = std::min(qual_cap, n1 * (lqm + 16) + 64);
            }
            TAKE(o_src, o.src, n1 * 4); TAKE(o_kind, o.kind, n1); TAKE(o_qsrc, o.qname_src, n1 * 4); TAKE(o_nm, o.nm_new, n1 * 4); TAKE(o_fr, o.fr, n1 * 2); TAKE(o_rr, o.rr, n1 * 2); TAKE(o_mate, o.mate, n1 * 4);
            TAKE(o_soff, o.seq_off, n1 * 8); TAKE(o_qoff, o.qual_off, n1 * 8); TAKE(o_seq, o.seq, seq_cap); TAKE(o_qual, o.qual, qual_cap);
            TAKE(o_key, o.key, n1 * sizeof(OutKey)); TAKE(o_rec, o.rec, n1 * sizeof(OutRec)); TAKE(o_ksoff, o.ksoff, n1 * 8); TAKE(o_kqoff, o.kqoff, n1 * 8); TAKE(o_krow, o.krow, n1 * 4); TAKE(o_rank64, o.rank64, (n1 / 64 + 2) * 4);
            const unsigned nblk_O = cdiv(n1, OUT_TILE); TAKE(o_part3, o.part3, (size_t)nblk_O * 24 + 64);
            if (e->h_si.n_raw > 0 && C > 0) hipLaunchKernelGGL(k_raw_emit, dim3(cdiv(C, 256)), dim3(256), 0, s, b, p, w, C);
            hipLaunchKernelGGL(k_stats, dim3(1024), dim3(256), 0, s, b, w, (NG > 0 ? C : 0u), NG);
            CANARY("k_stats");
            hipLaunchKernelGGL(k_out_reduce, dim3(nblk_O), dim3(OUT_T), 0, s, b, w, o);
            CANARY("k_out_reduce");
            hipLaunchKernelGGL(k_out_partials, dim3(1), dim3(1024), 0, s, o, (uint64_t)nblk_O, w);
            CANARY("k_out_partials");
            const bool lq_uniform = si_behind_describe && e->h_si.lq_max >= 0 && e->h_si.lq_min == e->h_si.lq_max;
            if (lq_uniform) hipLaunchKernelGGL(k_out_meta<true>, dim3(nblk_O), dim3(OUT_T), 0, s, b, w, o, (int)e->h_si.lq_max);
            else hipLaunchKernelGGL(k_out_meta<false>, dim3(nblk_O), dim3(OUT_T), 0, s, b, w, o, -1);
            CANARY("k_out_meta");
            const unsigned og = std::min<unsigned>(cdiv(n1, 256), 8192u);
            hipLaunchKernelGGL(k_out_rows, dim3(og), dim3(256), 0, s, w, o);
            CANARY("k_out_rows");
            hipLaunchKernelGGL(k_out_mate, dim3(og), dim3(256), 0, s, w, o);
            CANARY("k_out_mate");
            hipLaunchKernelGGL(k_out_gather, dim3(std::min<unsigned>(cdiv(n1, 16), 16384u)), dim3(256), 0, s, b, w, o);
            CANARY("k_out_gather");
        }
        HIPCHK(hipEventRecord(e->ev[EV_OUTPUT], s));
        CANARY("EV_OUTPUT");
        return GCE_OK;
    }

    int close_step() {
        int rc;
        hipLaunchKernelGGL(k_fold_stats, dim3(1), dim3(64), 0, s, w.si, pre_extra);
        if ((rc = read_si(e)) != GCE_OK) return rc;
        HIPCHK(hipGetLastError());
#ifdef GCE_SI_CHECK
        si_check();
#endif
        e->h_si.n_groups = NG;
        float ms = 0;
        auto el = [&](int a, int c) { ms = 0; (void)hipEventElapsedTime(&ms, e->ev[a], e->ev[c]); return (double)ms; };
        e->timing.total_ms = el(EV_START, EV_OUTPUT);
        e->timing.cluster_ms = el(EV_START, EV_CLUSTER); e->timing.csr_ms = el(EV_CLUSTER, EV_CSR); e->timing.describe_ms = el(EV_CSR, EV_DESCRIBE);
        e->timing.pairing_ms = el(EV_DESCRIBE, EV_PAIRING); e->timing.score_ms = el(EV_PAIRING, EV_SCORE); e->timing.consensus_ms = el(EV_SCORE, EV_CONSENSUS);
        e->timing.finish_ms = el(EV_CONSENSUS, EV_FINISH); e->timing.output_ms = el(EV_FINISH, EV_OUTPUT);
        e->timing.n_clusters = C; e->timing.n_groups = NG;
        if (e->dev_error != 0) {
            char buf[160]; snprintf(buf, sizeof buf, "%s (read %u)", gce_status_message(e->dev_error), e->dev_error_read);
            return fail(e, e->dev_error, buf);
        }
        e->n_out = (int64_t)e->h_si.n_out;
        e->out_seq_bytes = (size_t)(e->h_si.out_units >> 32) * 16; e->out_qual_bytes = (size_t)(e->h_si.out_units & 0xFFFFFFFFull) * 16;
        e->timing.n_pairs = (int64_t)e->h_si.n_pairs_total; e->timing.n_leaders = (int64_t)e->h_si.n_leaders;
        return GCE_OK;
    }

#ifdef CL_PROF
    void dump_cluster_prof() {
        if (N <= 0) return;
        StreamInfo hs; (void)hipStreamSynchronize(s); (void)hipMemcpy(&hs, e->si.p, sizeof hs, hipMemcpyDeviceToHost);
        static const char *nm[3] = {"key records + keys", "LDS leaders", "stores"};
        const double blocks = (double)hs.prof[15];
        fprintf(stderr, "k_cluster phases, mean per block (us), %.0f blocks:", blocks);
        for (int k = 0; k < 3; k++) fprintf(stderr, " %s %.2f;", nm[k], blocks ? hs.prof[k] / blocks / 100.0 : 0.0);
        fprintf(stderr, "\n");
    }
#endif
#ifdef PS_STOP
    int time_pairing_sub_and_stop() {
        hipEvent_t a_, b_, c_; (void)hipEventCreate(&a_); (void)hipEventCreate(&b_); (void)hipEventCreate(&c_);
        (void)hipEventRecord(a_, s);
        hipLaunchKernelGGL(k_pairing_sub<16>, dim3(cdiv(C, 4 * WAVES_PER_BLOCK)), dim3(256), 0, s, b, p, w, C, (const uint32_t *)nullptr, (const unsigned long long *)nullptr, w.pq_flag, 0);
        (void)hipEventRecord(b_, s);
        hipLaunchKernelGGL(k_pairing_sub<32>, dim3(cdiv(C, 2 * WAVES_PER_BLOCK)), dim3(256), 0, s, b, p, w, C, (const uint32_t *)nullptr, (const unsigned long long *)nullptr, w.pf_flag, 0);
        (void)hipEventRecord(c_, s); (void)hipEventSynchronize(c_);
        float m1 = 0, m2 = 0; (void)hipEventElapsedTime(&m1, a_, b_); (void)hipEventElapsedTime(&m2, b_, c_);
        fprintf(stderr, "k_pairing_sub up to tick %d: <16> %.3f ms, <32> over ALL clusters %.3f ms\n", PS_STOP, m1, m2);
        return fail(e, GCE_ERR_INVALID, "experiment build");
    }
#endif
#ifdef VB_STOP
    int time_vote_and_stop(unsigned nbatch, uint32_t n_live) {
        hipEvent_t a_, b_; (void)hipEventCreate(&a_); (void)hipEventCreate(&b_);
        (void)hipEventRecord(a_, s); hipLaunchKernelGGL(k_vote, dim3(nbatch), dim3(VB_T), 0, s, b, p, w, n_live); (void)hipEventRecord(b_, s); (void)hipEventSynchronize(b_);
        float ms_ = 0; (void)hipEventElapsedTime(&ms_, a_, b_); fprintf(stderr, "k_vote up to tick %d: %.3f ms\n", VB_STOP, ms_);
        return fail(e, GCE_ERR_INVALID, "experiment build");
    }
#endif
#ifdef VB_PROF
    void dump_vote_prof() {
        if (NG == 0) return;
        StreamInfo hs; (void)hipStreamSynchronize(s); (void)hipMemcpy(&hs, e->si.p, sizeof hs, hipMemcpyDeviceToHost);
        static const char *nm[11] = {"P0 groups", "P1 pairs", "P2 classes", "P3 overlap", "P4 pass A", "P5 lists", "P5 items", "P5 decide", "P5 tail", "P6 results", "P7 write"};
        const double blocks = (double)hs.prof[15];
        fprintf(stderr, "k_vote phases, mean per block (100 MHz ticks -> us), %.0f blocks:", blocks);
        for (int k = 0; k < 11; k++) fprintf(stderr, " %s %.2f;", nm[k], blocks ? hs.prof[k] / blocks / 100.0 : 0.0);
#ifndef VB_COUNT
        fprintf(stderr, " [of P2: (a) reads vs class %.2f; (b) sides' states %.2f; the rest = order, prefixes, barrier]", blocks ? hs.prof[11] / blocks / 100.0 : 0.0, blocks ? hs.prof[12] / blocks / 100.0 : 0.0);
#endif
        fprintf(stderr, "\n");
#ifdef VB_COUNT
        fprintf(stderr, "k_vote columns in the full vote: %.0f, one base only: %.0f, of those unchanged: %.0f\n", (double)hs.prof[11], (double)hs.prof[12], (double)hs.prof[13]);
#endif
#ifdef DV_PROF
        fprintf(stderr, "k_deep_prepare: %.0f sides, mean %.1f us per side, mean %.0f pairs per side\n", (double)hs.prof[14], hs.prof[14] ? hs.prof[6] / (double)hs.prof[14] / 100.0 : 0.0, hs.prof[14] ? hs.prof[7] / (double)hs.prof[14] / 100.0 : 0.0);
#endif
        static const char *pn[8] = {"windows", "name sort", "pairs", "umi words", "umi sort", "grouping", "layout sort", "layout write"};
        const double cl = (double)hs.prof[30];
        fprintf(stderr, "k_pairing_deep phases, mean per cluster (us), %.0f clusters:", cl);
        for (int k = 0; k < 8; k++) fprintf(stderr, " %s %.1f;", pn[k], cl ? hs.prof[16 + k] / cl / 100.0 : 0.0);
        fprintf(stderr, "\n");
    }
#endif
#ifdef GCE_SI_CHECK
    void si_check() {
        bool badw = false;
        for (int k = 14; k < GCE_STATS_WORDS; k++) if ((k != 15 && e->h_si.post[k] != 0) || e->h_si.pre[k] < 0) badw = true;
        if (!badw) return;
        StreamInfo again; (void)hipMemcpy(&again, e->si.p, sizeof again, hipMemcpyDeviceToHost);
        fprintf(stderr, "SI_CHECK: N %lld NG %u C %u n_out %llu\n post:", (long long)N, NG, C, (unsigned long long)e->h_si.n_out);
        for (int k = 0; k < 30; k++) fprintf(stderr, " %lld", e->h_si.post[k]);
        fprintf(stderr, "\n post again:"); for (int k = 0; k < 30; k++) fprintf(stderr, " %lld", again.post[k]);
        fprintf(stderr, "\n pre:"); for (int k = 0; k < 30; k++) fprintf(stderr, " %lld", e->h_si.pre[k]);
        fprintf(stderr, "\n other nonzero post words:"); for (int k = 30; k < GCE_STATS_WORDS; k++) if (e->h_si.post[k]) fprintf(stderr, " [%d]=%lld", k, e->h_si.post[k]);
        fprintf(stderr, "\n post_slot col 0..7 sums:"); for (int k = 0; k < 8; k++) { long long a = 0; for (int q = 0; q < GCE_PRE_SLOTS; q++) a += e->h_si.post_slot[q][k]; fprintf(stderr, " %lld", a); }
        fprintf(stderr, "\n scalars: n_clustered %llu n_slow %u n_deep %u n_slow_pair %u n_gen %llu n_pf %llu n_pq %llu vote_weight %llu\n", e->h_si.n_clustered, e->h_si.n_slow, e->h_si.n_deep, e->h_si.n_slow_pair, (unsigned long long)(e->h_si.hand_on >> 32), e->h_si.n_pf_items, e->h_si.n_pq_items, e->h_si.vote_weight);
    }
#endif
};
}
#undef TAKE

static int gce_process_impl(gce_engine *e) {
    if (!e) return GCE_ERR_INVALID;
    Step st(e);
    int (Step::*const stages[])() = {&Step::check_and_cut, &Step::stage_constants, &Step::size_by_reads, &Step::form_clusters, &Step::describe,
                                     &Step::pair_clusters, &Step::consensus, &Step::output_table, &Step::close_step};
    for (auto stage : stages) { const int rc = (st.*stage)(); if (rc != GCE_OK) return rc; }
    return GCE_OK;
}

static void fill_stats(gce_stats *dst, const long long *src) { memcpy(dst, src, sizeof(gce_stats)); }

int gce_result_device(gce_engine *e, gce_result *out) {
    if (!e || !out || !e->processed || e->dev_error) return GCE_ERR_INVALID;
    memset(out, 0, sizeof *out);
    out->n_reads = e->n; out->n_out = e->n_out;
    out->src = e->o_src.as<uint32_t>(); out->kind = e->o_kind.as<uint8_t>(); out->qname_src = e->o_qsrc.as<uint32_t>(); out->nm_new = e->o_nm.as<int32_t>();
    out->fr = e->o_fr.as<int16_t>(); out->rr = e->o_rr.as<int16_t>(); out->mate = e->o_mate.as<uint32_t>();
    out->seq_off = e->o_soff.as<uint64_t>(); out->qual_off = e->o_qoff.as<uint64_t>(); out->seq = e->o_seq.as<uint8_t>(); out->qual = e->o_qual.as<uint8_t>();
    out->seq_bytes = e->out_seq_bytes; out->qual_bytes = e->out_qual_bytes;
    fill_stats(&out->pre, e->h_si.pre); fill_stats(&out->post, e->h_si.post);
    return GCE_OK;
}

int gce_drain(gce_engine *e, gce_result *out) {
    if (!e || !out || !e->processed || e->dev_error) return GCE_ERR_INVALID;
    (void)hipSetDevice(e->prm.device);
    const size_t n = (size_t)e->n_out;
    e->r_src.resize(n); e->r_kind.resize(n); e->r_qsrc.resize(n); e->r_nm.resize(n); e->r_fr.resize(n); e->r_rr.resize(n); e->r_mate.resize(n);
    e->r_soff.resize(n); e->r_qoff.resize(n); e->r_seq.resize(e->out_seq_bytes); e->r_qual.resize(e->out_qual_bytes);
    if (e->r_seq.size() != e->out_seq_bytes || e->r_qual.size() != e->out_qual_bytes) return GCE_ERR_OOM;
    hipStream_t s = e->stream;
    if (n) {
        HIPCHK(hipMemcpyAsync(e->r_src.data(), e->o_src.p, n * 4, hipMemcpyDeviceToHost, s));
        HIPCHK(hipMemcpyAsync(e->r_kind.data(), e->o_kind.p, n, hipMemcpyDeviceToHost, s));
        HIPCHK(hipMemcpyAsync(e->r_qsrc.data(), e->o_qsrc.p, n * 4, hipMemcpyDeviceToHost, s));
        HIPCHK(hipMemcpyAsync(e->r_nm.data(), e->o_nm.p, n * 4, hipMemcpyDeviceToHost, s));
        HIPCHK(hipMemcpyAsync(e->r_fr.data(), e->o_fr.p, n * 2, hipMemcpyDeviceToHost, s));
        HIPCHK(hipMemcpyAsync(e->r_rr.data(), e->o_rr.p, n * 2, hipMemcpyDeviceToHost, s));
        HIPCHK(hipMemcpyAsync(e->r_mate.data(), e->o_mate.p, n * 4, hipMemcpyDeviceToHost, s));
        HIPCHK(hipMemcpyAsync(e->r_soff.data(), e->o_soff.p, n * 8, hipMemcpyDeviceToHost, s));
        HIPCHK(hipMemcpyAsync(e->r_qoff.data(), e->o_qoff.p, n * 8, hipMemcpyDeviceToHost, s));
        if (!e->r_seq.empty()) HIPCHK(hipMemcpyAsync(e->r_seq.data(), e->o_seq.p, e->r_seq.size(), hipMemcpyDeviceToHost, s));
        if (!e->r_qual.empty()) HIPCHK(hipMemcpyAsync(e->r_qual.data(), e->o_qual.p, e->r_qual.size(), hipMemcpyDeviceToHost, s));
        HIPCHK(hipStreamSynchronize(s));
    }
    memset(out, 0, sizeof *out);
    out->n_reads = e->n; out->n_out = e->n_out;
    out->src = e->r_src.data(); out->kind = e->r_kind.data(); out->qname_src = e->r_qsrc.data(); out->nm_new = e->r_nm.data();
    out->fr = e->r_fr.data(); out->rr = e->r_rr.data(); out->mate = e->r_mate.data();
    out->seq_off = e->r_soff.data(); out->qual_off = e->r_qoff.data(); out->seq = e->r_seq.data(); out->qual = e->r_qual.data();
    out->seq_bytes = e->out_seq_bytes; out->qual_bytes = e->out_qual_bytes;
#ifdef GCE_SI_CHECK
    for (int k = 14; k < GCE_STATS_WORDS; k++) if (k != 15 && e->h_si.post[k] != 0) fprintf(stderr, "SI_CHECK(gce_drain): the engine's host copy has post[%d] = %lld\n", k, e->h_si.post[k]);
#endif
    fill_stats(&out->pre, e->h_si.pre); fill_stats(&out->post, e->h_si.post);
    return GCE_OK;
}

__global__ void k_payload_finish(const StreamInfo *si, const int32_t *where, int32_t n_regions, const unsigned long long *bed_grouped, int32_t nreg, long long *payload, int64_t nbins) {
    const int i = blockIdx.x * blockDim.x + threadIdx.x;
    if (i < 2 * GCE_STATS_WORDS) payload[i] = i < GCE_STATS_WORDS ? si->pre[i] : si->post[i - GCE_STATS_WORDS];
    if (i < n_regions) {
        const int w = where[i];
        long long *bed = payload + 2 * GCE_STATS_WORDS + 2 * nbins;
        bed[i] = w >= 0 ? (long long)bed_grouped[w] : 0; bed[n_regions + i] = w >= 0 ? (long long)bed_grouped[nreg + w] : 0;
    }
}

int gce_stats_payload_device(gce_engine *e, int32_t step, int32_t n_regions, const int32_t *r_tid, const int32_t *r_start, const int32_t *r_end, const int64_t **payload, gce_payload_layout *layout) {
    if (!e || !payload || !layout || step <= 0 || n_regions < 0 || (n_regions > 0 && (!r_tid || !r_start || !r_end))) return GCE_ERR_INVALID;
    if (!e->processed || e->dev_error) return fail(e, GCE_ERR_INVALID, "gce_stats_payload_device before a successful gce_process");
    (void)hipSetDevice(e->prm.device);
    hipStream_t s = e->stream;
    const int nt = (int)e->target_len.size();
    e->h_binoff.assign(nt + 1, 0);
    for (int t = 0; t < nt; t++) e->h_binoff[t + 1] = e->h_binoff[t] + 1 + (int64_t)e->target_len[t] / step;
    const int64_t nbins = e->h_binoff[nt];
    std::vector<int32_t> off(nt + 1, 0), rs(n_regions), re(n_regions), pm(n_regions), where(n_regions);
    for (int k = 0; k < n_regions; k++) if (r_tid[k] >= 0 && r_tid[k] < nt) off[r_tid[k] + 1]++;
    for (int t = 0; t < nt; t++) off[t + 1] += off[t];
    std::vector<int32_t> fill(off.begin(), off.end() - 1);
    std::vector<uint8_t> sorted(std::max(nt, 1), 1);
    std::fill(where.begin(), where.end(), -1);
    for (int k = 0; k < n_regions; k++) {
        if (r_tid[k] < 0 || r_tid[k] >= nt) continue;
        const int t = r_tid[k], at = fill[t]++;
        rs[at] = r_start[k]; re[at] = r_end[k]; where[k] = at;
        pm[at] = at > off[t] ? std::max(pm[at - 1], r_end[k]) : r_end[k];
        if (at > off[t] && rs[at] < rs[at - 1]) sorted[t] = 0;
    }
    const int nreg = off[nt];
    auto up = [&](DevBuf &d, const void *src, size_t bytes) -> int { HIPCHK(d.ensure(bytes + 64)); if (bytes) HIPCHK(hipMemcpyAsync(d.p, src, bytes, hipMemcpyHostToDevice, s)); return GCE_OK; };
    int rc;
    if ((rc = up(e->dp_binoff, e->h_binoff.data(), (nt + 1) * 8)) || (rc = up(e->dp_regoff, off.data(), (nt + 1) * 4)) || (rc = up(e->dp_rs, rs.data(), (size_t)nreg * 4)) ||
        (rc = up(e->dp_re, re.data(), (size_t)nreg * 4)) || (rc = up(e->dp_pmax, pm.data(), (size_t)nreg * 4)) || (rc = up(e->dp_sorted, sorted.data(), sorted.size())) ||
        (rc = up(e->dp_where, where.data(), (size_t)n_regions * 4))) return rc;
    const int64_t words = 2 * GCE_STATS_WORDS + 2 * nbins + 2 * (int64_t)n_regions;
    HIPCHK(e->dp_depth.ensure((size_t)words * 8 + 64)); HIPCHK(e->dp_bed.ensure((size_t)nreg * 16 + 64));
    HIPCHK(hipMemsetAsync(e->dp_depth.p, 0, (size_t)words * 8, s)); HIPCHK(hipMemsetAsync(e->dp_bed.p, 0, (size_t)nreg * 16 + 16, s));
    DepthCtx c; c.bin_off = e->dp_binoff.as<int64_t>(); c.n_targets = nt; c.step = step; c.reg_off = e->dp_regoff.as<int32_t>();
    c.r_start = e->dp_rs.as<int32_t>(); c.r_end = e->dp_re.as<int32_t>(); c.r_pmax = e->dp_pmax.as<int32_t>(); c.contig_sorted = e->dp_sorted.as<uint8_t>();
    long long *pay = e->dp_depth.as<long long>();
    unsigned long long *dpre = (unsigned long long *)pay + 2 * GCE_STATS_WORDS, *dpost = dpre + nbins, *bpre = e->dp_bed.as<unsigned long long>(), *bpost = bpre + nreg;
    const uint64_t n = (uint64_t)e->n_pre, no = (uint64_t)e->n_out;
    if (n) hipLaunchKernelGGL(k_depth, dim3(cdiv(n, DP_T * DP_RPT)), dim3(DP_T), 0, s, e->dev_batch.core, (const uint32_t *)nullptr, n, c, dpre, bpre);
    if (no) hipLaunchKernelGGL(k_depth, dim3(cdiv(no, DP_T * DP_RPT)), dim3(DP_T), 0, s, e->dev_batch.core, (const uint32_t *)e->o_src.p, no, c, dpost, bpost);
    const int fin = std::max(2 * GCE_STATS_WORDS, (int)n_regions);
    hipLaunchKernelGGL(k_payload_finish, dim3(cdiv(fin, 256)), dim3(256), 0, s, (const StreamInfo *)e->si.p, (const int32_t *)e->dp_where.p, n_regions, (const unsigned long long *)e->dp_bed.p, nreg, pay, nbins);
    HIPCHK(hipGetLastError());
    HIPCHK(hipStreamSynchronize(s));
    layout->stats_words = 2 * GCE_STATS_WORDS; layout->n_targets = nt; layout->n_bins = nbins; layout->n_regions = n_regions; layout->total_words = words; layout->bin_off = e->h_binoff.data();
    e->payload_words = words;
    *payload = (const int64_t *)pay;
    return GCE_OK;
}

int gce_stats_payload_read(gce_engine *e, const int64_t *payload, int64_t n_words, int64_t *host) {
    if (!e || !payload || !host || n_words < 0) return GCE_ERR_INVALID;
    (void)hipSetDevice(e->prm.device);
    if (n_words) HIPCHK(hipMemcpyAsync(host, payload, (size_t)n_words * 8, hipMemcpyDeviceToHost, e->stream));
    HIPCHK(hipStreamSynchronize(e->stream));
    return GCE_OK;
}

int gce_depth_stats(gce_engine *e, int32_t step, int32_t n_regions, const int32_t *r_tid, const int32_t *r_start, const int32_t *r_end, gce_depth *out) {
    if (!e || !out) return GCE_ERR_INVALID;
    const int64_t *pay = nullptr; gce_payload_layout lay;
    int rc = gce_stats_payload_device(e, step, n_regions, r_tid, r_start, r_end, &pay, &lay);
    if (rc != GCE_OK) return rc;
    hipStream_t s = e->stream;
    const int64_t nbins = lay.n_bins;
    e->h_depth_pre.resize(nbins); e->h_depth_post.resize(nbins); e->h_bed_pre.assign(n_regions, 0); e->h_bed_post.assign(n_regions, 0);
    const int64_t *d0 = pay + lay.stats_words;
    if (nbins) { HIPCHK(hipMemcpyAsync(e->h_depth_pre.data(), d0, nbins * 8, hipMemcpyDeviceToHost, s)); HIPCHK(hipMemcpyAsync(e->h_depth_post.data(), d0 + nbins, nbins * 8, hipMemcpyDeviceToHost, s)); }
    if (n_regions) { HIPCHK(hipMemcpyAsync(e->h_bed_pre.data(), d0 + 2 * nbins, (size_t)n_regions * 8, hipMemcpyDeviceToHost, s)); HIPCHK(hipMemcpyAsync(e->h_bed_post.data(), d0 + 2 * nbins + n_regions, (size_t)n_regions * 8, hipMemcpyDeviceToHost, s)); }
    HIPCHK(hipStreamSynchronize(s));
    out->n_targets = lay.n_targets; out->bin_off = e->h_binoff.data(); out->pre_depth = e->h_depth_pre.data(); out->post_depth = e->h_depth_post.data();
    out->n_regions = n_regions; out->pre_bed = e->h_bed_pre.data(); out->post_bed = e->h_bed_post.data();
    return GCE_OK;
}

int gce_stats_device(gce_engine *e, const int64_t **pre_then_post) {
    if (!e || !pre_then_post || !e->processed || e->dev_error) return GCE_ERR_INVALID;
    *pre_then_post = (const int64_t *)e->si.as<StreamInfo>()->pre;
    return GCE_OK;
}

int gce_get_timing(gce_engine *e, gce_timing *out) {
    if (!e || !out) return GCE_ERR_INVALID;
    *out = e->timing;
    return GCE_OK;
}

int gce_get_vote_counters(gce_engine *e, int64_t out[4]) {
    if (!e || !out || !e->processed) return GCE_ERR_INVALID;
    out[0] = (int64_t)e->h_si.vote_rounds2; out[1] = (int64_t)e->h_si.vote_rounds2_unaligned;
    out[2] = (int64_t)(e->h_si.hand_on >> 32); out[3] = (int64_t)e->h_si.n_groups;
    return GCE_OK;
}

int gce_get_consensus_counters(gce_engine *e, int64_t out[5]) {
    if (!e || !out || !e->processed) return GCE_ERR_INVALID;
    out[0] = 2 * (int64_t)(e->h_si.n_groups ? e->h_si.n_live : 0) - (int64_t)(e->h_si.hand_on >> 32);
    out[1] = (int64_t)e->h_si.cs_fast; out[2] = (int64_t)e->h_si.cs_prep; out[3] = (int64_t)e->h_si.cs_deep; out[4] = (int64_t)e->h_si.cs_slow;
    return GCE_OK;
}

int gce_get_skipped_groups(gce_engine *e, int64_t out[2]) {
    if (!e || !out || !e->processed) return GCE_ERR_INVALID;
    out[0] = e->h_si.n_groups ? (int64_t)e->h_si.n_groups - (int64_t)e->h_si.n_live : 0;
    out[1] = e->h_si.n_groups ? (int64_t)(e->h_si.vote_weight / VB_W) + 1 : 0;
    return GCE_OK;
}

int gce_get_index_counters(gce_engine *e, int64_t out[4]) {
    if (!out) return GCE_ERR_INVALID;
    for (int k = 0; k < 4; k++) out[k] = e ? e->idx_ctr[k] : __atomic_load_n(&g_pass_idx_ctr[k], __ATOMIC_RELAXED);
    return GCE_OK;
}
// ... 38 lines not shown
```

gencore_amd/csrc/gce_cluster.hpp:

```cpp
#pragma once

#ifndef SB_T
#define SB_T 512
#endif
#ifndef SB_U
#define SB_U 2
#endif
#define SB_READS (SB_T * SB_U)
#define SB_LDS_SLOTS (2 * SB_READS)
#define SB_OFF_BITS (SB_READS == 1024 ? 10 : 9)
static_assert(SB_READS == 512 || SB_READS == 1024, "LeadRec.info packs a place and a count of SB_READS");

struct __attribute__((aligned(16))) LeadRec { unsigned long long kw; uint32_t info, runlen; };
static_assert(sizeof(LeadRec) == 16, "LeadRec must stay 16 bytes");
#define LI_ODD (1u << 22)
struct __attribute__((aligned(8))) BlkHdr { uint32_t n_lead, n_clu; };
struct __attribute__((aligned(8))) LeadOut { uint32_t h, rb; };
#define LO_OWNER 0x80000000u

#define IKEY_RAW (1u << 30)
__device__ __forceinline__ uint32_t d_thr_mode(uint32_t ikey, const StreamInfo *si, const DevParams &p) {
    uint32_t inst = ikey & 0x3FFFFFFFu, seg_b = ikey >> 31;
    if (!seg_b) {
        if ((int)(inst + 1) <= si->n_events_a) return THR_PROPER;
// ... 167 lines not shown
        }
    };
    unsigned int v = 0, nl = 0;
    for (int64_t i = w0 + 4 * lane; i < w1; i += 256) { unsigned int c[4]; load4(i, c, nl); v += c[0] + c[1] + c[2] + c[3]; }
    v = (unsigned int)wave_sum((int)v); nl = (unsigned int)wave_sum((int)nl);
    if (lane == 0) { s_w[wv] = v; s_l[wv] = nl; }
    __syncthreads();
    unsigned int carry = 0, tot = 0; unsigned long long leaders = 0;
#pragma unroll
    for (int k = 0; k < 16; k++) { const unsigned int t = s_w[k]; tot += t; carry += k < wv ? t : 0u; leaders += s_l[k]; }
    for (int64_t i0 = w0; i0 < w1; i0 += 256) {
        const int64_t i = i0 + 4 * lane;
        unsigned int c[4], dummy = 0; load4(i, c, dummy);
        const unsigned int sum = c[0] + c[1] + c[2] + c[3];
        const unsigned int x = (unsigned int)wave_scan_incl((int)sum);
        unsigned int run = carry + x - sum;
#pragma unroll
        for (int k = 0; k < 4; k++) { if (i + k < w1) w.blk_base[i + k] = run; run += c[k]; }
        carry += (unsigned int)__builtin_amdgcn_readlane((int)x, 63);
    }
    if (threadIdx.x == 0) {
        unsigned long long total = tot;
        w.si->n_clustered = total;
        w.si->n_leaders = leaders;
        long long per_ = p.period;
        long long e = (p.tick_offset + (long long)total) / per_ - p.tick_offset / per_;
        w.si->n_events = (int)(e < w.max_events ? e : w.max_events);
        if (e > w.max_events) raise_error(w.si, GCE_ERR_INVALID, 0);
    }
}

#define EV_T 1024
__global__ __launch_bounds__(EV_T) void k_events(DevBatch b, DevParams p, Work w) {
    __shared__ int s_a;
    if (threadIdx.x == 0) s_a = 0;
    __syncthreads();
    const int j = (int)((blockIdx.x * blockDim.x + threadIdx.x) >> 6), lane = lane_id();
    const int E = w.si->n_events;
    if (j < E) {
        const long long per = p.period;
        const long long gt = (p.tick_offset / per + (j + 1)) * per;
        const unsigned int t = (unsigned int)(gt - p.tick_offset);
        int64_t lo = 0, hi = w.n_sblk - 1;
        while (lo < hi) {
            const int64_t step = (hi - lo + 63) / 64, probe = lo + (int64_t)(lane + 1) * step;
            const bool below = probe <= hi && w.blk_base[probe] < t;
            const int k = __popcll(__ballot(below));
            hi = min(hi, lo + (int64_t)(k + 1) * step - 1);
            lo = lo + (int64_t)k * step;
        }
        unsigned int need = t - w.blk_base[lo];
        const int64_t i0 = lo * SB_READS, end = min(b.n, i0 + SB_READS);
        int64_t i = end;
        bool clq[SB_READS / 64];
#pragma unroll
        for (int q = 0; q < SB_READS / 64; q++) {
            const int64_t idx = i0 + 64 * q + lane;
            clq[q] = idx < end && w.slot[idx] != NONE32;
        }
#pragma unroll
        for (int q = 0; q < SB_READS / 64; q++) {
            const bool cl = clq[q];
            const unsigned long long m = __ballot(cl);
            const unsigned int cnt = (unsigned int)__popcll(m);
            if (need <= cnt) {
                const unsigned long long hit = __ballot(cl && (unsigned int)__popcll(m & ((1ull << lane) - 1ull)) + 1u == need);
                i = i0 + 64 * q + (__ffsll((long long)hit) - 1);
                break;
            }
            need -= cnt;
        }
        if (lane == 0) {
            w.ev_read[j] = (uint32_t)i;
            w.ev_tid[j] = b.core[i].tid;
            w.ev_pos[j] = b.core[i].pos;
            if ((uint32_t)i < w.si->first_unmapped) atomicAdd(&s_a, 1);
        }
    }
    __syncthreads();
    if (threadIdx.x == 0 && s_a) atomicAdd(&w.si->n_events_a, s_a);
}

__global__ __launch_bounds__(256) void k_leaders(DevBatch b, DevParams p, Work w) {
    const int lane = lane_id();
    const int64_t blk = (int64_t)blockIdx.x * (blockDim.x >> 6) + (threadIdx.x >> 6);
    if (blk >= w.n_sblk) return;
    const uint32_t nl = w.bhdr[blk].n_lead;
    if (nl == 0) return;
    const StreamInfo *si = w.si;
    const unsigned int first_unm = si->first_unmapped;
    const int n_ev_a = si->n_events_a, n_ev = si->n_events;
    const long long per = p.period;
    const int ev_last = max(n_ev - 1, 0);
    unsigned int E = 0, r = 0;
    if (!b.tick) {
        const unsigned long long t0 = (unsigned long long)(unsigned int)p.tick_rem0 + w.blk_base[blk];
        const unsigned int uper = (unsigned int)per;
        if ((t0 >> 32) == 0) { E = (unsigned int)t0 / uper; r = (unsigned int)t0 - E * uper; }
        else { E = (unsigned int)(t0 / uper); r = (unsigned int)(t0 - (unsigned long long)E * uper); }
    }
    for (uint32_t kq = (uint32_t)lane; kq < nl; kq += 64) {
        const size_t LR = (size_t)blk * SB_READS + kq;
        union { LeadRec r; uint4 q; } in; in.q = *reinterpret_cast<const uint4 *>(w.lrec + LR);
        const uint32_t off = in.r.info & ((1u << SB_OFF_BITS) - 1u), rk = (in.r.info >> SB_OFF_BITS) & 0x7FFu;
        const bool odd = (in.r.info & LI_ODD) != 0;
        const uint32_t idx = (uint32_t)(blk * SB_READS + off);
        ClusterKey key;
        if (in.r.kw) key = d_unpack_key(in.r.kw, p);
        else {
            union { gce_core c; uint4 q[2]; } t; const uint4 *src = reinterpret_cast<const uint4 *>(b.core + idx); t.q[0] = src[0]; t.q[1] = src[1];
            key = d_key(t.c, p);
        }
        int e;
        if (b.tick) e = (int)(((long long)b.tick[idx] - 1) / per - p.tick_epoch0);
        else { const unsigned int x = r + rk; e = (int)(E + x / (unsigned int)per); }
        const bool seg_b = (first_unm != NONE32) && (idx > first_unm);
        const int lo = seg_b ? n_ev_a : 0, hi = seg_b ? n_ev : n_ev_a;
        const int g = min(max(e, lo), hi);
        auto takes = [&](int T, int P) { return key.tid < T || (key.tid == T && key.left < P && key.right < (long long)P); };
        const int j0 = min(max(g - 1, 0), ev_last), j1 = min(g, ev_last), j2 = min(g + 1, ev_last);
        const int T0 = w.ev_tid[j0], P0 = w.ev_pos[j0], T1 = w.ev_tid[j1], P1 = w.ev_pos[j1], T2 = w.ev_tid[j2], P2 = w.ev_pos[j2];
        const int cb = p.nw_cb, bd = p.nw_bd;
        const long long delta1 = key.right - (long long)key.left + 1;
        bool fits = false; uint64_t h = 0; unsigned long long id_w = 0, cur = 0;
        if (p.nw_ok && in.r.kw != 0ull && !seg_b && key.tid < p.n_targets && (uint32_t)key.left < p.target_len[key.tid]) {
            uint64_t q;
            d_divmod(d_tab_index(key, 0u, p), w.tsize, w.tinv, q, h);
            fits = (q >> (62 - cb - bd)) == 0 && ((uint64_t)delta1 >> bd) == 0;
            id_w = TAB_OCC | (q << (cb + bd)) | ((uint64_t)delta1 << cb);
        }
        const bool early = fits && !odd;
        if (early) cur = __hip_atomic_load(&w.tab[h].key, __ATOMIC_RELAXED, __HIP_MEMORY_SCOPE_AGENT);
        int a, z;
        if (odd && g > lo && takes(T0, P0)) { a = lo; z = g - 1; }
        else if (g >= hi || takes(T1, P1)) a = z = g;
        else if (g + 1 >= hi || takes(T2, P2)) a = z = g + 1;
        else { a = g + 2; z = hi; }
        while (a < z) {
            const int mid = (a + z) >> 1;
            if (takes(w.ev_tid[mid], w.ev_pos[mid])) z = mid; else a = mid + 1;
        }
        const bool implied = e <= a;
        const uint32_t ikey = (seg_b ? 0x80000000u : 0u) | (key.left < 0 ? IKEY_RAW : 0u) | (uint32_t)max(e, a);
        const bool normal = fits && implied;
        bool owner = false, exotic = !normal, first_miss = true; uint32_t rbase = 0;
        auto next_probe = [&]() {
            if (first_miss) {
                uint64_t x = ((uint64_t)(uint32_t)key.tid * 0x9E3779B97F4A7C15ull) ^ ((uint64_t)(uint32_t)key.left * 0xC2B2AE3D27D4EB4Full) ^ ((uint64_t)key.right * 0x165667B19E3779F9ull) ^ ((uint64_t)ikey * 0xD6E8FEB86659FD93ull);
                x ^= x >> 31; x *= 0xBF58476D1CE4E5B9ull; x ^= x >> 29;
                h = d_bucket(x >> 14, w.tsize, w.tinv);
                first_miss = false;
            } else h = h + 1 == w.tsize ? 0 : h + 1;
        };
        if (normal) {
            const unsigned long long cmask = (1ull << cb) - 1ull;
            if (!early) cur = __hip_atomic_load(&w.tab[h].key, __ATOMIC_RELAXED, __HIP_MEMORY_SCOPE_AGENT);
            for (;;) {
                if (cur == 0ull) {
                    const unsigned long long o = atomicCAS(&w.tab[h].key, 0ull, id_w | in.r.runlen);
                    if (o == 0ull) { owner = true; break; }
                    cur = o;
                }
                if ((cur >> cb) != (id_w >> cb)) { exotic = true; break; }
                if ((cur & cmask) + in.r.runlen > cmask) { raise_error(w.si, GCE_ERR_INVALID, idx); break; }
                const unsigned long long o = atomicCAS(&w.tab[h].key, cur, cur + in.r.runlen);
                if (o == cur) { rbase = (uint32_t)(cur & cmask); break; }
                cur = o;
            }
            if (owner) w.lrec[LR].runlen = ikey;
            if (exotic) next_probe();
        } else h = d_bucket(d_tab_index(key, ikey, p), w.tsize, w.tinv);
        if (exotic) {
            const unsigned long long tk = d_exotic_key(ikey, idx);
            if ((ikey & 0x3FFFFFFFu) >= (1u << 29)) raise_error(w.si, GCE_ERR_INVALID, idx);
            for (;;) {
                const unsigned long long c = atomicCAS(&w.tab[h].key, 0ull, tk);
                if (c == 0ull) { owner = true; break; }
                bool mine = false;
                if ((c >> 32) == (tk >> 32)) { const ClusterKey ok = d_key(b.core[(uint32_t)c], p); mine = ok.tid == key.tid && ok.left == key.left && ok.right == key.right; }
                if (mine) break;
                next_probe();
            }
            rbase = (uint32_t)atomicAdd(&w.tab[h].ic, (unsigned long long)in.r.runlen | (owner ? (unsigned long long)ikey << 32 : 0ull));
            if (owner && (ikey & IKEY_RAW)) atomicAdd(&w.si->n_raw, 1u);
        }
        LeadOut o; o.h = (uint32_t)h; o.rb = rbase | (owner ? LO_OWNER : 0u);
        w.lout[LR] = o;
    }
}

#define SCAN_TILE 2048
__global__ __launch_bounds__(256) void k_num_reduce(Work w, int p_cb) {
    const int lane = lane_id();
    const int64_t blk = (int64_t)blockIdx.x * (blockDim.x >> 6) + (threadIdx.x >> 6);
    const bool on = blk < w.n_sblk;
    const uint32_t nl = on ? w.bhdr[blk].n_lead : 0u;
    uint64_t v = 0;
    for (uint32_t kq = (uint32_t)lane; kq < nl; kq += 64) {
        const size_t LR = (size_t)blk * SB_READS + kq;
        const LeadOut o = w.lout[LR];
        if (o.rb & LO_OWNER) {
            const TabEntry t = w.tab[o.h];
            const unsigned long long ic = (t.key & TAB_EXO) ? t.ic : (((unsigned long long)w.lrec[LR].runlen << 32) | (t.key & ((1ull << p_cb) - 1ull)));
            w.lrec[LR].kw = ic;
            v += (1ull << 32) | (uint32_t)ic;
        }
    }
    v = (uint64_t)wave_sum64((long long)v);
    __shared__ uint64_t s_v[4];
    if (lane == 0) { s_v[threadIdx.x >> 6] = v; if (on) w.scan_part[gridDim.x + blk] = v; }
    __syncthreads();
    if (threadIdx.x == 0) w.scan_part[blockIdx.x] = s_v[0] + s_v[1] + s_v[2] + s_v[3];
}
__device__ __forceinline__ uint64_t tab_elem(const uint32_t *cnt, uint64_t h, uint64_t n) {
    if (h >= n) return 0;
    uint32_t c = cnt[h];
    return ((uint64_t)(c > 0) << 32) | c;
}
__global__ __launch_bounds__(256) void k_scan_reduce(const uint32_t *cnt, uint64_t n, uint64_t *part) {
    __shared__ uint64_t s[4];
    uint64_t base = (uint64_t)blockIdx.x * SCAN_TILE, v = 0;
    for (int k = 0; k < SCAN_TILE / 256; k++) v += tab_elem(cnt, base + k * 256 + threadIdx.x, n);
    v = (uint64_t)wave_sum64((long long)v);
    if (lane_id() == 0) s[threadIdx.x >> 6] = v;
    __syncthreads();
    if (threadIdx.x == 0) part[blockIdx.x] = s[0] + s[1] + s[2] + s[3];
}
__global__ __launch_bounds__(1024) void k_scan_partials(uint64_t *part, uint64_t nparts, unsigned long long *total_hi, unsigned long long *total_lo) {
    __shared__ uint64_t s_w[2][16];
    const int lane = lane_id(), wv = threadIdx.x >> 6;
    uint64_t carry = 0;
    int it = 0;
    for (uint64_t base = 0; base < nparts; base += 8192, it ^= 1) {
        const uint64_t i0 = base + 8 * (uint64_t)threadIdx.x;
        uint64_t c[8], v = 0;
#pragma unroll
        for (int k = 0; k < 8; k++) { c[k] = i0 + k < nparts ? part[i0 + k] : 0; v += c[k]; }
        uint64_t x = v;
        for (int o = 1; o < 64; o <<= 1) { uint64_t t = (uint64_t)__shfl_up((long long)x, o); if (lane >= o) x += t; }
        if (lane == 63) s_w[it][wv] = x;
        __syncthreads();
        uint64_t woff = 0, tot = 0;
#pragma unroll
        for (int k = 0; k < 16; k++) { const uint64_t t = s_w[it][k]; tot += t; woff += k < wv ? t : 0ull; }
        uint64_t run = carry + woff + x - v;
#pragma unroll
        for (int k = 0; k < 8; k++) { if (i0 + k < nparts) part[i0 + k] = run; run += c[k]; }
        carry += tot;
    }
    if (threadIdx.x == 0) { *total_hi = carry >> 32; if (total_lo) *total_lo = carry & 0xFFFFFFFFull; }
}
__global__ __launch_bounds__(256) void k_num_apply(Work w) {
    const int lane = lane_id();
    const int64_t blk = (int64_t)blockIdx.x * (blockDim.x >> 6) + (threadIdx.x >> 6);
    if (blk >= w.n_sblk) return;
    const uint32_t nl = w.bhdr[blk].n_lead;
    uint64_t carry = w.scan_part[blockIdx.x];
    for (int q = 0; q < (int)(threadIdx.x >> 6); q++) carry += w.scan_part[gridDim.x + blk - (threadIdx.x >> 6) + q];
    for (uint32_t k0 = 0; k0 < nl; k0 += 64) {
        const uint32_t kq = k0 + (uint32_t)lane;
        uint64_t v = 0, ic = 0; uint32_t h = 0;
        if (kq < nl) {
            const size_t LR = (size_t)blk * SB_READS + kq;
            const LeadOut o = w.lout[LR];
            if (o.rb & LO_OWNER) { h = o.h; ic = w.lrec[LR].kw; v = (1ull << 32) | (uint32_t)ic; }
        }
        uint64_t x = v;
        for (int o = 1; o < 64; o <<= 1) { uint64_t t = (uint64_t)__shfl_up((long long)x, o); if (lane >= o) x += t; }
        if (v) {
            const uint64_t ex = carry + x - v;
            const uint32_t cid = (uint32_t)(ex >> 32);
            w.cl_start[cid] = (uint32_t)ex; w.cl_n[cid] = (uint32_t)v; w.cl_ikey[cid] = (uint32_t)(ic >> 32); w.toff[h] = (uint32_t)ex;
        }
        carry += rl64(x, 63);
    }
}
__global__ __launch_bounds__(SB_T) void k_scatter(int64_t n, Work w) {
    __shared__ uint32_t s_dst[SB_READS];
    const int64_t blk = blockIdx.x;
    const uint32_t nl = w.bhdr[blk].n_lead;
    uint32_t v[SB_U];
#pragma unroll
    for (int u = 0; u < SB_U; u++) { const int64_t i = (blk * SB_U + u) * SB_T + threadIdx.x; v[u] = i < n ? w.slot[i] : NONE32; }
    for (uint32_t kq = threadIdx.x; kq < nl; kq += SB_T) {
        const LeadOut o = w.lout[(size_t)blk * SB_READS + kq];
        s_dst[kq] = w.toff[o.h] + (o.rb & ~LO_OWNER);
        if (o.rb & LO_OWNER) *reinterpret_cast<uint4 *>(&w.tab[o.h]) = make_uint4(0, 0, 0, 0);
    }
    __syncthreads();
#pragma unroll
    for (int u = 0; u < SB_U; u++) {
        const int64_t i = (blk * SB_U + u) * SB_T + threadIdx.x;
        if (v[u] != NONE32) w.members[s_dst[v[u] & 0xFFFFu] + (v[u] >> 16)] = (uint32_t)i;
    }
}

#ifndef DESC_WPE
#define DESC_WPE 8
#endif
__global__ __launch_bounds__(256, DESC_WPE) void k_describe(DevBatch b, DevParams p, Work w, int tiles_per_block) {
    __shared__ long long s_stat[WAVES_PER_BLOCK][6];
    long long st[6] = {0, 0, 0, 0, 0, 0};
    int lqmin = 0x7FFFFFFF, lqmax = -1;
    const int lane = lane_id(), wv = threadIdx.x >> 6;
    for (int cb = 0; cb < tiles_per_block; cb++) {
        const int64_t i = ((int64_t)blockIdx.x * tiles_per_block + cb) * 256 + threadIdx.x;
        if (i < b.n) {
            union { gce_core c; uint4 q[2]; } t; const uint4 *src = reinterpret_cast<const uint4 *>(b.core + i); t.q[0] = src[0]; t.q[1] = src[1];
            const gce_core k = t.c;
            const uint8_t c = d_classify(k);
            bool mapped = k.tid >= 0;
            const int nmv = b.nm[i]; const bool has_nm = b.nm_type[i] != 0;
            int mism = (mapped && has_nm) ? nmv : 0;
            w.nmx[i] = ((uint32_t)nmv << 1) | (has_nm ? 1u : 0u);
            st[0] += 1; st[1] += k.l_qseq; st[4] += mism;
            if (!mapped) { st[2] += 1; st[3] += k.l_qseq; }
            if (mism > 0) st[5] += 1;
            if (c != CLS_DROP) { lqmin = min(lqmin, k.l_qseq); lqmax = max(lqmax, k.l_qseq); }
            if (c == CLS_CLUSTERED) {
                const uint32_t *cg = b.cigar + b.cigar_off[i];
                const uint32_t c0w = k.n_cigar ? cg[0] : 0;
                int mo_ = 0, ml_ = 0;
                if (k.n_cigar == 1) ml_ = cig_op(c0w) == 0 ? cig_len(c0w) : 0;
                else d_first_m(cg, k.n_cigar, mo_, ml_);
                if (k.l_qseq > 65535) raise_error(w.si, GCE_ERR_INVALID, (uint32_t)i);
                if (p.ref_win && k.isize != 0 && k.tid < p.n_ref && p.ref_data[k.tid]) {
                    const int64_t rl = k.n_cigar == 1 ? (int64_t)cig_len(c0w) * consumes_ref(cig_op(c0w)) : (int64_t)d_cigar_rlen(cg, k.n_cigar);
                    const int64_t end_in = min((int64_t)k.pos + rl, p.ref_len[k.tid]);
                    if ((int64_t)k.pos < p.ref_win[2 * k.tid] || end_in > p.ref_win[2 * k.tid + 1]) raise_error(w.si, GCE_ERR_REF_WINDOW, (uint32_t)i);
                }
                store_desc(w.rdesc, (uint64_t)i, b.seq_off[i], b.qual_off[i], c0w, k.pos, k.isize != 0, k.l_qseq, mo_, ml_, k.n_cigar, k.tid, k.n_cigar > 1 ? cg[k.n_cigar - 1] : c0w);
                const char *src2; uint8_t hm = 0;
                if (b.mi && b.mi_off[i] != 0xFFFFFFFFFFFFFFFFull) { src2 = b.mi + b.mi_off[i]; hm = 1; }
                else src2 = b.qname + b.qname_off[i];
                int s0, l0;
                if (!d_umi_slice(src2, p, s0, l0, hm ? -1 : (int)k.l_qname - 1)) { raise_error(w.si, GCE_ERR_UMI_PARSE, (uint32_t)i); s0 = 0; l0 = 0; }
                if (l0 > UINFO_MAXLEN) { raise_error(w.si, GCE_ERR_UMI_PARSE, (uint32_t)i); l0 = 0; }
                w.uinfo[i] = uinfo_pack((hm ? b.mi_off[i] : b.qname_off[i]) + (uint64_t)s0, hm != 0, k.l_qname, l0);
            }
        }
    }
    for (int k = 0; k < 6; k++) { long long v = wave_sum64(st[k]); if (lane == 0) s_stat[wv][k] = v; }
    lqmin = wave_min(lqmin); lqmax = wave_max(lqmax);
    if (lane == 0) {
        if (lqmin < *(volatile int *)&w.si->lq_min) atomicMin(&w.si->lq_min, lqmin);
        if (lqmax > *(volatile int *)&w.si->lq_max) atomicMax(&w.si->lq_max, lqmax);
    }
    __syncthreads();
    if (threadIdx.x < 6) {
        long long v = s_stat[0][threadIdx.x] + s_stat[1][threadIdx.x] + s_stat[2][threadIdx.x] + s_stat[3][threadIdx.x];
        if (v) atomicAdd((unsigned long long *)&w.si->pre_slot[blockIdx.x & (GCE_PRE_SLOTS - 1)][threadIdx.x], (unsigned long long)v);
    }
}
```

gencore_amd/csrc/gce_device.hpp:

```cpp
#pragma once
#include <hip/hip_runtime.h>
#include <stdint.h>
#include "../../include/gencore_amd.h"

#define GCE_WAVE 64
#define NONE32 0xFFFFFFFFu
#define EMPTY64 0xFFFFFFFFFFFFFFFFull

enum : uint32_t { THR_PROPER = 0, THR_UNPROPER = 1, THR_NEVER = 2, THR_RAW = 3 };
enum : uint8_t { TIER_NEVER = 0, TIER_SUB16 = 1, TIER_SUB32 = 2, TIER_FAST = 3, TIER_DEEP_LDS = 4, TIER_DEEP_DEVICE = 5, TIER_GENERIC = 6 };
enum : uint8_t { CLS_DROP = 0, CLS_CLUSTERED = 1, CLS_BYPASS = 2 };

struct DevBatch {
    int64_t n;
    const gce_core *core;
    const uint64_t *qname_off; const char *qname;
    const uint64_t *cigar_off; const uint32_t *cigar;
    const uint64_t *seq_off;   uint8_t *seq;
    const uint64_t *qual_off;  uint8_t *qual;
    const int32_t *nm; const uint8_t *nm_type;
    const uint64_t *mi_off; const char *mi;
    const uint64_t *tick;
};

struct DevParams {
    int32_t proper_thr, unproper_thr, duplex_mismatch_thr, cluster_size_req, base_score_req;
    int32_t high_q, moderate_q, low_q;
    int32_t s_high, s_moderate, s_low, s_bad;
    int32_t skip_low_complexity_thr, duplex_only, disable_duplex, period;
    int32_t score_bias, score_max;
    uint32_t q2s_lut;
    uint32_t thr_low4, thr_mod4, thr_high4;
    int32_t q2s_swar_ok;
    double score_percent_req;
    char prefix[32];
    int32_t prefix_len;
    int32_t n_targets;
    const uint32_t *target_len;
    const uint64_t *target_cum;
    int32_t key_bt, key_bl;
    int32_t nw_ok, nw_cb, nw_bd;
    int32_t vote_ok, vote_accept_by_qual, s_min_lb;
    int64_t tick_offset;
    int64_t tick_epoch0; int32_t tick_rem0;
    int32_t trailing_flush;
    int32_t n_ref;
    const uint8_t *const *ref_data;
    const int64_t *ref_len;
    const int64_t *ref_win;
};

#define GCE_PRE_SLOTS 64
struct StreamInfo {
    unsigned long long n_clustered;
    unsigned int first_unmapped;
    unsigned long long err_key;
    int n_events;
    int n_events_a;
    unsigned int n_slow;
    unsigned long long prof[32];
    unsigned int n_deep;
    unsigned long long hand_on;
    unsigned int n_slow_pair;
    unsigned int n_slow_pair2;
    unsigned int pair_next, pair_next2;
    unsigned int prep_next, deep_next;
    int lq_min, lq_max;
    unsigned long long n_clusters, n_groups, n_pairs, n_out;
    unsigned long long n_pairs_total;
    unsigned long long vote_weight;
    unsigned long long n_live;
    unsigned long long n_leaders;
    unsigned long long out_units;
    unsigned long long n_pf_items;
    unsigned long long n_pq_items;
    unsigned long long n_p16_items;
    unsigned long long vote_rounds2;
    unsigned long long vote_rounds2_unaligned;
    unsigned int n_raw;
    unsigned int cs_fast, cs_prep, cs_deep, cs_slow;
    long long pre[GCE_STATS_WORDS];
    long long post[GCE_STATS_WORDS];
    long long post_slot[GCE_PRE_SLOTS][8];
    long long pre_slot[GCE_PRE_SLOTS][8];
};

__device__ __forceinline__ void raise_error(StreamInfo *si, int code, uint32_t read) {
    atomicMin(&si->err_key, ((unsigned long long)read << 8) | (unsigned long long)((-code) & 0xFF));
}

__device__ __forceinline__ int lane_id() { return threadIdx.x & 63; }

__device__ __forceinline__ int cig_op(uint32_t w) { return (int)(w & 0xF); }
__device__ __forceinline__ int cig_len(uint32_t w) { return (int)(w >> 4); }
__device__ __forceinline__ int consumes_query(int op) { return (0x193 >> op) & 1; }
__device__ __forceinline__ int consumes_ref(int op) { return (0x18D >> op) & 1; }

struct __attribute__((aligned(16))) ReadDescP {
    uint32_t so_lo, qo_lo;
    uint32_t c0;
    uint32_t pos_fl;
    uint16_t lq, mo, ml, nc;
    int32_t tid;
    uint32_t hi;
};
static_assert(sizeof(ReadDescP) == 32, "ReadDescP must stay 32 bytes");
struct ReadDesc {
    uint64_t so, qo;
    uint32_t c0;
    int32_t pos, lq, isize;
    int32_t mo, ml;
    int32_t tid;
    uint16_t nc, lastm;
    int32_t rlen;
};
#define RLEN_WALK (-0x40000000)
__device__ __forceinline__ void store_desc(ReadDescP *base, uint64_t i, uint64_t so, uint64_t qo, uint32_t c0, int32_t pos, bool isize_nz, int lq, int mo, int ml, int nc, int32_t tid, uint32_t last_op) {
    union { ReadDescP d; uint4 q[2]; } u;
    u.d.so_lo = (uint32_t)so; u.d.qo_lo = (uint32_t)qo; const uint32_t lastm = cig_op(last_op) == 0 ? min((uint32_t)cig_len(last_op), 65535u) : 0u;
    u.d.hi = ((uint32_t)(so >> 32) & 0xFFu) | ((uint32_t)(qo >> 32) & 0xFFu) << 8 | lastm << 16;
    u.d.c0 = c0; u.d.pos_fl = (uint32_t)pos | (isize_nz ? 0x80000000u : 0u);
    u.d.lq = (uint16_t)lq; u.d.mo = (uint16_t)mo; u.d.ml = (uint16_t)ml; u.d.nc = (uint16_t)nc; u.d.tid = tid;
    uint4 *dst = reinterpret_cast<uint4 *>(base + i); dst[0] = u.q[0]; dst[1] = u.q[1];
}
__device__ __forceinline__ ReadDesc load_desc(const ReadDescP *base, uint32_t i) {
    union { ReadDescP d; uint4 q[2]; } u;
    const uint4 *src = reinterpret_cast<const uint4 *>(base + i);
    u.q[0] = src[0]; u.q[1] = src[1];
    ReadDesc r;
    r.so = (uint64_t)u.d.so_lo | (uint64_t)(u.d.hi & 0xFFu) << 32; r.qo = (uint64_t)u.d.qo_lo | (uint64_t)((u.d.hi >> 8) & 0xFFu) << 32;
    r.c0 = u.d.c0; r.pos = (int32_t)(u.d.pos_fl & 0x7FFFFFFFu); r.isize = (int32_t)(u.d.pos_fl >> 31);
    r.lq = u.d.lq; r.mo = u.d.mo; r.ml = u.d.ml; r.nc = u.d.nc; r.tid = u.d.tid; r.lastm = (uint16_t)(u.d.hi >> 16);
    r.rlen = u.d.nc == 1 ? (int32_t)(cig_len(u.d.c0) * consumes_ref(cig_op(u.d.c0))) : (u.d.nc == 0 ? 0 : RLEN_WALK);
    return r;
}


__device__ inline bool d_is_part_of(const uint32_t *part, int np, const uint32_t *whole, int nw, bool left) {
    if (nw < np) return false;
    for (int i = 0; i < np; i++) {
        uint32_t a = left ? part[i] : part[np - 1 - i];
        uint32_t b = left ? whole[i] : whole[nw - 1 - i];
        if (cig_op(a) != cig_op(b)) return false;
        int la = cig_len(a), lb = cig_len(b);
        if (la > lb) return false;
        if (la < lb && i != np - 1) {
            if (i != np - 2) return false;
            uint32_t nx = left ? part[i + 1] : part[np - 2 - i];
            if (cig_op(nx) != 5 ) return false;
        }
    }
    return true;
}

__device__ inline int d_ref_offset(const uint32_t *cig, int n, int qpos) {
    int ref = 0, query = 0;
    for (int i = 0; i < n; i++) {
        int op = cig_op(cig[i]), len = cig_len(cig[i]);
        int cq = consumes_query(op), cr = consumes_ref(op);
        query += len * cq;
        ref += len * cr;
        if (query > qpos) {
            if (op == 1 || op == 4) return -1;
            return ref - cr * (query - qpos);
        }
    }
    return -1;
}

__device__ inline void d_first_m(const uint32_t *cig, int n, int &off, int &len) {
    int query = 0;
    for (int i = 0; i < n; i++) {
        int op = cig_op(cig[i]), l = cig_len(cig[i]);
        if (op == 0) { off = query; len = l; return; }
        query += l * consumes_query(op);
    }
    off = 0; len = 0;
}

__device__ inline int d_cigar_rlen(const uint32_t *cig, int n) {
    int l = 0;
    for (int i = 0; i < n; i++) l += cig_len(cig[i]) * consumes_ref(cig_op(cig[i]));
    return l;
}

__device__ __forceinline__ int d_nib(const uint8_t *s, int i) {
    uint8_t b = s[i >> 1];
    return (i & 1) ? (b & 0xF) : (b >> 4);
}
__device__ __forceinline__ int d_base_class(int nib4) { return (nib4 == 1 || nib4 == 2 || nib4 == 4 || nib4 == 8) ? nib4 : 15; }

__device__ __forceinline__ int d_ref_nib(const uint8_t *ref, int64_t pos) {
    int b = ref[pos >> 1];
    int code = (pos & 1) ? (b >> 4) : (b & 0xF);
    return (int)((0x42810u >> (4 * (code < 5 ? code : 5))) & 0xFu);
}

__device__ __forceinline__ int d_qual2score(const DevParams &p, int q) {
    if (p.q2s_swar_ok) {
        const int nthr = (q >= p.low_q) + (q >= p.moderate_q) + (q >= p.high_q);
        return (int)((p.q2s_lut >> (8 * nthr)) & 0xFFu) - p.score_bias;
    }
    return q >= p.high_q ? p.s_high : q >= p.moderate_q ? p.s_moderate : q >= p.low_q ? p.s_low : p.s_bad;
}

__device__ __forceinline__ uint32_t d_q2s4_biased(const DevParams &p, uint32_t q4) {
    if (p.q2s_swar_ok) {
        const uint32_t t = q4 | 0x80808080u;
        const uint32_t c = (((t - p.thr_low4) & 0x80808080u) >> 7) + (((t - p.thr_mod4) & 0x80808080u) >> 7) + (((t - p.thr_high4) & 0x80808080u) >> 7);
        return __builtin_amdgcn_perm(0u, p.q2s_lut, c);
    }
    uint32_t r = 0;
#pragma unroll
    for (int k = 0; k < 4; k++) r |= (uint32_t)((d_qual2score(p, (q4 >> (8 * k)) & 0xFF) + p.score_bias) & 0xFF) << (8 * k);
    return r;
}
#define GCE_PATCH_CONST 0xFFFFFFFFu
__device__ __forceinline__ int d_score_at(const DevParams &p, const int8_t *score_row, uint32_t patch, int pos, int q) {
    if (patch == GCE_PATCH_CONST) return p.s_moderate;
    if ((unsigned)(pos - (int)(patch & 0xFFFF)) < (patch >> 16)) return (int)(uint8_t)score_row[pos] - p.score_bias;
    return d_qual2score(p, q);
}

__device__ __forceinline__ bool d_is_umi_char(char c) { return c == 'A' || c == 'T' || c == 'C' || c == 'G' || c == '_'; }

typedef uint64_t u64_unaligned_t __attribute__((aligned(1)));
__device__ __forceinline__ uint64_t d_zero_bytes(uint64_t x) {
    const uint64_t m = 0x7F7F7F7F7F7F7F7Full;
    return ~(((x & m) + m) | x | m);
}
__device__ __forceinline__ uint64_t d_eq_bytes(uint64_t w, char c) { return d_zero_bytes(w ^ (0x0101010101010101ull * (uint8_t)c)); }
__device__ __forceinline__ uint64_t d_umi_bytes(uint64_t w) {
    return d_eq_bytes(w, 'A') | d_eq_bytes(w, 'T') | d_eq_bytes(w, 'C') | d_eq_bytes(w, 'G') | d_eq_bytes(w, '_');
}
__device__ __forceinline__ uint64_t d_range_bytes(int lo, int hi, int k) {
    const int a = min(max(lo - 8 * k, 0), 8), z = min(max(hi - 8 * k, 0), 8);
    const uint64_t upto_z = z >= 8 ? ~0ull : ((1ull << (8 * z)) - 1ull), upto_a = a >= 8 ? ~0ull : ((1ull << (8 * a)) - 1ull);
    return upto_z & ~upto_a;
}

__device__ inline bool d_umi_slice_bytes(const char *s, const DevParams &p, int &start, int &len, int n);

__device__ inline bool d_umi_slice(const char *s, const DevParams &p, int &start, int &len, int n = -1) {
    if (n < 0 || p.prefix_len > 4) return d_umi_slice_bytes(s, p, start, len, n);
    const int base = n > 32 ? n - 32 : 0, nwin = n - base;
    uint64_t w[4];
#pragma unroll
    for (int k = 0; k < 4; k++) w[k] = 8 * k < nwin ? *(const u64_unaligned_t *)(s + base + 8 * k) : 0ull;
    start = 0; len = 0;
    int wpos = -1;
#pragma unroll
    for (int k = 3; k >= 0; k--) {
        if (wpos < 0 && 8 * k < nwin) {
            uint64_t h = 0;
            if (p.prefix_len > 0) { for (int c = 0; c < p.prefix_len; c++) h |= d_eq_bytes(w[k], p.prefix[c]); }
            else h = d_eq_bytes(w[k], ':');
            h &= d_range_bytes(0, nwin, k);
            if (h) wpos = 8 * k + ((63 - __clzll((long long)h)) >> 3);
        }
    }
    if (wpos < 0) {
        if (base == 0) return true;
        return d_umi_slice_bytes(s, p, start, len, n);
    }
    if (p.prefix_len > 0) {
        const int wst = wpos + 2;
        if (base + wst > n) return false;
        int l = nwin - wst;
        bool open = true;
#pragma unroll
        for (int k = 0; k < 4; k++) {
            if (open && 8 * k + 8 > wst && 8 * k < nwin) {
                const uint64_t stop = ~d_umi_bytes(w[k]) & 0x8080808080808080ull & d_range_bytes(wst, nwin, k);
                if (stop) { l = 8 * k + ((__ffsll((long long)stop) - 1) >> 3) - wst; open = false; }
            }
        }
        start = base + wst; len = l;
        return true;
    }
    const int sep = base + wpos;
    if (sep >= n - 1) return true;
    bool ok = true; int us = 0;
#pragma unroll
    for (int k = 0; k < 4; k++) {
        const uint64_t tail = d_range_bytes(wpos + 1, nwin, k);
        if (~d_umi_bytes(w[k]) & 0x8080808080808080ull & tail) ok = false;
        us += __popcll(d_eq_bytes(w[k], '_') & tail);
    }
    int st = sep + 1;
    { const int j = wpos + 1; const char c = (char)(w[j >> 3] >> (8 * (j & 7))); if (st < n - 1 && c == '_') { st++; us--; } }
    if (!ok || us > 1) return true;
    start = st; len = n - st;
    return true;
}

__device__ inline bool d_umi_slice_bytes(const char *s, const DevParams &p, int &start, int &len, int n) {
    if (n < 0) { n = 0; while (s[n]) n++; }
    start = 0; len = 0;
    if (p.prefix_len > 0) {
        int pos = -1;
        for (int i = n - 1; i >= 0; i--) {
            char c = s[i];
            bool hit = false;
            for (int k = 0; k < p.prefix_len; k++) hit |= (p.prefix[k] == c);
            if (hit) { pos = i; break; }
        }
        if (pos < 0) return true;
        int st = pos + 2;
        if (st > n) return false;
        int l = 0;
        while (st + l < n && d_is_umi_char(s[st + l])) l++;
        start = st; len = l;
        return true;
    }
    int sep = -1, us = 0;
    bool ok = true;
    for (int i = n - 1; i >= 0; i--) {
        char c = s[i];
        if (c == ':') { sep = i; break; }
        if (!d_is_umi_char(c)) ok = false;
        if (c == '_') us++;
    }
    if (sep < 0 || sep >= n - 1) return true;
    int st = sep + 1;
    if (st < n - 1 && s[st] == '_') { st++; us--; }
    if (!ok || us > 1) return true;
    start = st; len = n - st;
    return true;
}

__device__ inline int d_umi_diff(const char *a, int la, const char *b, int lb) {
    int m = la < lb ? la : lb;
    int d = la > lb ? la - lb : lb - la;
    for (int i = 0; i < m; i++) d += (a[i] != b[i]);
    return d;
}
__device__ inline bool d_bytes_equal(const char *a, int la, const char *b, int lb) {
    if (la != lb) return false;
    for (int i = 0; i < la; i++) if (a[i] != b[i]) return false;
    return true;
}
__device__ inline int d_slice_cmp(const char *a, int la, const char *b, int lb) {
    int m = la < lb ? la : lb;
    for (int i = 0; i < m; i++) {
        unsigned char x = (unsigned char)a[i], y = (unsigned char)b[i];
        if (x != y) return x < y ? -1 : 1;
    }
    return la - lb;
}
__device__ inline int d_strcmp(const char *a, const char *b) {
    for (int i = 0;; i++) {
        unsigned char x = (unsigned char)a[i], y = (unsigned char)b[i];
        if (x != y) return x < y ? -1 : 1;
        if (x == 0) return 0;
    }
}

__device__ inline int d_split2(const char *s, int n, int &s0, int &l0, int &s1, int &l1) {
    int i = 0;
    while (i < n && s[i] == '_') i++;
    if (i >= n) return 0;
    int cnt = 0, ts = i;
    s0 = l0 = s1 = l1 = 0;
    for (;; ) {
        int j = ts;
        while (j < n && s[j] != '_') j++;
        if (cnt == 0) { s0 = ts; l0 = j - ts; }
        else if (cnt == 1) { s1 = ts; l1 = j - ts; }
        cnt++;
        if (j >= n) break;
        ts = j + 1;
    }
    return cnt;
}
__device__ inline bool d_is_duplex(const char *a, int la, const char *b, int lb) {
    int a0, al0, a1, al1, b0, bl0, b1, bl1;
    if (d_split2(a, la, a0, al0, a1, al1) != 2) return false;
    if (d_split2(b, lb, b0, bl0, b1, bl1) != 2) return false;
    return d_bytes_equal(a + a0, al0, b + b1, bl1) && d_bytes_equal(a + a1, al1, b + b0, bl0);
}

struct ClusterKey { int32_t tid, left; int64_t right; };

__device__ __forceinline__ uint8_t d_classify(const gce_core &c) {
    if (c.tid < 0 || c.pos < 0) return CLS_DROP;
    if (c.flag & (0x100 | 0x800)) return CLS_DROP;
    long long d = (long long)c.mpos - (long long)c.pos;
    if (d < 0) d = -d;
    if (c.mtid == c.tid && d < 100000) return CLS_CLUSTERED;
    if (c.mtid < 0) return CLS_BYPASS;
    return CLS_CLUSTERED;
}
__device__ __forceinline__ ClusterKey d_key(const gce_core &c, const DevParams &p) {
    ClusterKey k;
    k.tid = c.tid; k.left = c.pos;
    long long d = (long long)c.mpos - (long long)c.pos;
    if (d < 0) d = -d;
    if (c.mtid == c.tid && d < 100000) {
        if (c.isize < 0) k.left = c.mpos;
        long long a = c.isize; if (a < 0) a = -a;
        k.right = (long long)k.left + a - 1;
    } else {
        long long tl = (c.tid < p.n_targets && p.target_len) ? (long long)p.target_len[c.tid] : 0;
        k.right = -1LL * tl * (long long)(c.mtid + 1) + (long long)c.mpos;
    }
    return k;
}
__device__ __forceinline__ void d_divmod(uint64_t x, uint64_t T, double tinv, uint64_t &q, uint64_t &r) {
    if (x >> 52) { q = x / T; r = x - q * T; return; }
    uint64_t qq = (uint64_t)((double)x * tinv);
    long long rr = (long long)(x - qq * T);
    while (rr < 0) { rr += (long long)T; qq--; }
    while (rr >= (long long)T) { rr -= (long long)T; qq++; }
    q = qq; r = (uint64_t)rr;
}
__device__ __forceinline__ uint64_t d_bucket(uint64_t x, uint64_t T, double tinv) {
    if (x >> 52) return x % T;
    const uint64_t q = (uint64_t)((double)x * tinv);
    long long r = (long long)(x - q * T);
    while (r < 0) r += (long long)T;
    while (r >= (long long)T) r -= (long long)T;
    return (uint64_t)r;
}

__device__ __forceinline__ int d_lqname_pad(const gce_core &c) { return ((int)c.l_qname + 3) & ~3; }

__device__ __forceinline__ int wave_sum(int v) {
    for (int o = 32; o > 0; o >>= 1) v += __shfl_xor(v, o);
    return v;
}
__device__ __forceinline__ int wave_max(int v) {
    for (int o = 32; o > 0; o >>= 1) { int t = __shfl_xor(v, o); v = t > v ? t : v; }
    return v;
}
__device__ __forceinline__ int wave_min(int v) {
    for (int o = 32; o > 0; o >>= 1) { int t = __shfl_xor(v, o); v = t < v ? t : v; }
    return v;
}
__device__ __forceinline__ int wave_scan_incl(int v) {
    v += __builtin_amdgcn_update_dpp(0, v, 0x111, 0xf, 0xf, false);
    v += __builtin_amdgcn_update_dpp(0, v, 0x112, 0xf, 0xf, false);
    v += __builtin_amdgcn_update_dpp(0, v, 0x114, 0xf, 0xf, false);
    v += __builtin_amdgcn_update_dpp(0, v, 0x118, 0xf, 0xf, false);
    v += __builtin_amdgcn_update_dpp(0, v, 0x142, 0xa, 0xf, false);
    v += __builtin_amdgcn_update_dpp(0, v, 0x143, 0xc, 0xf, false);
    return v;
}

template <int CTRL> __device__ __forceinline__ int dpp_move(int v) { return __builtin_amdgcn_update_dpp(v, v, CTRL, 0xf, 0xf, false); }
__device__ __forceinline__ int row_max16(int v) {
    v = max(v, dpp_move<0x128>(v));
    v = max(v, dpp_move<0x124>(v));
    v = max(v, dpp_move<0x122>(v));
    v = max(v, dpp_move<0x121>(v));
    return v;
}
__device__ __forceinline__ int wave_max_u(int v) {
    const int r = row_max16(v);
    return max(max(__builtin_amdgcn_readlane(r, 0), __builtin_amdgcn_readlane(r, 16)), max(__builtin_amdgcn_readlane(r, 32), __builtin_amdgcn_readlane(r, 48)));
}
__device__ __forceinline__ int lanes_below(unsigned long long mask) {
    return __popcll(mask & ((1ull << lane_id()) - 1ull));
}
```

gencore_amd/csrc/gce_kernels.hpp:

```cpp
#pragma once
#include "gce_device.hpp"

#define CHUNK 256
#define WAVES_PER_BLOCK 4

struct __attribute__((aligned(16))) OutRec { uint32_t qname_src, mate; int16_t nm_new, fr, rr; uint16_t pad; };
static_assert(sizeof(OutRec) == 16, "OutRec must stay 16 bytes");

struct Work {
    uint64_t *uinfo;
    ReadDescP *rdesc;
    uint32_t *spatch;
    uint32_t *slot;
    int8_t *score;
    uint8_t *out_flag; OutRec *orec;
    uint32_t *nmx;
    uint32_t *out_index;
    struct LeadRec *lrec; struct LeadOut *lout;
    struct BlkHdr *bhdr; uint32_t *blk_base; int64_t n_sblk;
    int32_t *ev_tid, *ev_pos; uint32_t *ev_read; int max_events;
    struct TabEntry *tab; uint32_t *toff; uint64_t tsize; double tinv;
    uint32_t *cl_ikey, *cl_start, *cl_n, *cl_npairs, *cl_ngroups, *cl_gbase, *cl_nresult; uint8_t *cl_hasumi;
    uint8_t *cl_tier;
    uint32_t *members, *sorted, *pl, *pr, *pu, *pg, *gpl, *gpr, *grp_begin, *grp_n;
// ... 1241 lines not shown
    if ((double)bc < (double)np * 0.4 && np != 1) { if (lane == 0) rp_out[gi] = NONE32; return true; }
    const uint32_t out = (uint32_t)rl32((int)rd, best);
    if (out == NONE32) { if (lane == 0) rp_out[gi] = NONE32; return true; }
    const int o_pos = rl32(pos, best), o_lq = rl32(lq, best), o_nc = rl32(nc, best); const uint32_t o_c0 = (uint32_t)rl32((int)c0, best);
    const uint64_t o_cigo = rl64(cigo, best), o_so = rl64(so, best), o_qo = rl64(qo, best);
    const uint32_t *ocig = b.cigar + o_cigo;
    bool take = false; int ld = 0;
    if (uniform) take = has;
    else if (has) {
        take = lane == best || part_of_fast(o_c0, o_nc, ocig, c0, nc, b.cigar + cigo, left_mode);
        if (take) { ld = lq - o_lq; if (ld != 0 && pos == o_pos && part_of_fast(o_c0, o_nc, ocig, c0, nc, b.cigar + cigo, true)) ld = 0; }
    }
    const unsigned long long vmask = __ballot(take);
    int len = o_lq;
    if (o_nc == 0) len = wave_min(take ? lq : 0x7FFFFFFF);
    const int nbytes = (len + 1) >> 1;
    if (nbytes > 256) {
        if (lane == 0) w.slow_list[atomicAdd(&w.si->n_slow, 1u)] = gi * 2 + (is_left ? 0 : 1);
        return false;
    }
    const int o_isz = rl32(isz, best), o_tid = rl32(rtid, best);
    const int o_nm_type = b.nm_type[out], o_nm = b.nm[out];
    const uint8_t *ref = nullptr; int64_t ref_len = 0;
    if (o_isz != 0 && o_tid >= 0 && o_tid < p.n_ref) {
        const uint8_t *rdp = p.ref_data[o_tid];
        int64_t need_len = (int64_t)ref_off_fast(ocig, o_nc, o_c0, len - 1) + 1;
        if (rdp && (int64_t)o_pos + need_len < p.ref_len[o_tid]) { ref = rdp; ref_len = p.ref_len[o_tid]; }
    }
    uint8_t *oseq = b.seq + o_so, *oqual = b.qual + o_qo;
    uint8_t *resb = s_res_wave, *resq = s_res_wave + 512;
    uint16_t *cplx = (uint16_t *)(s_res_wave + 1024);
    const int accept_score = max(p.base_score_req, 1);
    int n_cplx = 0; bool odd = false;
    const bool even_ld = left_mode || !__any(take && (ld & 1));
    const int nvot = __popcll(vmask);
    const bool swar_ok = even_ld && len <= 256 && nvot * (p.score_max + p.score_bias) <= 255 && p.q2s_swar_ok && accept_score + nvot * p.score_bias <= 255;
    if (swar_ok) {
        const int c4 = 4 * lane;
        const bool act = c4 < len;
        const int nval = act ? min(4, len - c4) : 0;
        const uint32_t nmask = nval >= 4 ? 0xFFFFu : nval == 3 ? 0xF0FFu : nval == 2 ? 0x00FFu : nval == 1 ? 0x00F0u : 0u;
        const uint32_t bmask = nval >= 4 ? 0xFFFFFFFFu : nval == 0 ? 0u : ((1u << (8 * nval)) - 1u);
        uint32_t t16 = 0;
        if (act) t16 = *(const u16_unaligned *)(oseq + 2 * lane);
        uint32_t dacc = 0, ssum = 0, tqm = 0, qor = 0, cnt = 0;
        const int s_min = min(min(p.s_high, p.s_moderate), min(p.s_low, p.s_bad));
        const bool lower_bound_ok = nvot * s_min >= accept_score;
        const uint32_t smin4 = 0x01010101u * (uint32_t)((s_min + p.score_bias) & 0xFF);
        unsigned long long m = vmask;
        while (m) {
            int vv[4]; uint32_t s16[4], q4[4], sc4[4], vm[4];
#pragma unroll
            for (int u = 0; u < 4; u++) { vv[u] = m ? __ffsll((long long)m) - 1 : -1; if (m) m &= m - 1; }
#pragma unroll
            for (int u = 0; u < 4; u++) {
                s16[u] = t16; q4[u] = 0; sc4[u] = 0; vm[u] = 0;
                if (vv[u] >= 0) {
                    const int v = vv[u];
                    const uint64_t vso = rl64(so, v), vqo = rl64(qo, v); const int vld = left_mode ? 0 : rl32(ld, v), vlq = rl32(lq, v);
                    const uint32_t vpatch = (uint32_t)rl32((int)patch, v);
                    const int r0 = c4 + vld;
                    if (act) {
                        if (r0 >= 0 && r0 + nval <= vlq) {
                            s16[u] = *(const u16_unaligned *)(b.seq + vso + (r0 >> 1));
                            q4[u] = *(const u32_unaligned *)(b.qual + vqo + r0);
                            if (vpatch == 0u) sc4[u] = lower_bound_ok ? smin4 : d_q2s4_biased(p, q4[u]);
                            else if (vpatch == GCE_PATCH_CONST) sc4[u] = 0x01010101u * (uint32_t)((p.s_moderate + p.score_bias) & 0xFF);
                            else {
                                const int ps = (int)(vpatch & 0xFFFF), pe = ps + (int)(vpatch >> 16);
                                const int a_ = max(ps - r0, 0), z_ = min(pe - r0, 4);
                                const uint32_t pmk = z_ > a_ ? ((z_ >= 4 ? 0xFFFFFFFFu : ((1u << (8 * z_)) - 1u)) & ~((1u << (8 * a_)) - 1u)) : 0u;
                                const uint32_t st4 = *(const u32_unaligned *)((const uint8_t *)w.score + vqo + r0);
                                sc4[u] = ((lower_bound_ok ? smin4 : d_q2s4_biased(p, q4[u])) & ~pmk) | (st4 & pmk);
                            }
                            vm[u] = bmask;
                        } else {
                            uint32_t sx = t16;
                            for (int k = 0; k < nval; k++) {
                                const int rp = r0 + k;
                                if (rp >= 0 && rp < vlq) {
                                    const int nb = d_nib(b.seq + vso, rp), sh = 8 * (k >> 1) + ((k & 1) ? 0 : 4);
                                    sx = (sx & ~(0xFu << sh)) | ((uint32_t)nb << sh);
                                    q4[u] |= (uint32_t)b.qual[vqo + rp] << (8 * k);
                                    sc4[u] |= (uint32_t)((d_score_at(p, w.score + vqo, vpatch, rp, b.qual[vqo + rp]) + p.score_bias) & 0xFF) << (8 * k);
                                    vm[u] |= 0xFFu << (8 * k);
                                }
                            }
                            s16[u] = sx;
                        }
                    }
                }
            }
#pragma unroll
            for (int u = 0; u < 4; u++) {
                const uint32_t qv = q4[u] & vm[u];
                dacc |= (s16[u] ^ t16) & nmask;
                ssum += sc4[u] & vm[u];
                cnt += vm[u] & 0x01010101u;
                qor |= qv;
                const uint32_t ge = ((tqm | 0x80808080u) - qv) & 0x80808080u;
                const uint32_t sel = (ge - (ge >> 7)) | ge;
                tqm = (tqm & sel) | (qv & ~sel);
            }
        }
        if (qor & 0x80808080u) odd = true;
        bool cq[4];
        {
            const uint32_t tn4 = __builtin_amdgcn_perm(0u, ((t16 >> 4) & 0x0F0Fu) | ((t16 & 0x0F0Fu) << 16), 0x03010200u);
            const uint32_t dn4 = __builtin_amdgcn_perm(0u, ((dacc >> 4) & 0x0F0Fu) | ((dacc & 0x0F0Fu) << 16), 0x03010200u);
            const uint32_t differ = (dn4 + 0x7F7F7F7Fu) & 0x80808080u;
            const uint32_t sel = tn4 & 0x07070707u;
            const uint32_t v_lo = __builtin_amdgcn_perm(0x000000FFu, 0x00FFFF00u, sel);
            const uint32_t v_hi = __builtin_amdgcn_perm(0xFF000000u, 0x000000FFu, sel);
            const uint32_t hi8 = ((tn4 >> 3) & 0x01010101u) * 0xFFu;
            const uint32_t valid = (v_hi & hi8) | (v_lo & ~hi8);
            const uint32_t ge_q = ((tqm | 0x80808080u) - 0x01010101u * (uint32_t)p.moderate_q) & 0x80808080u;
            const uint32_t rhs = cnt * (uint32_t)p.score_bias + 0x01010101u * (uint32_t)accept_score;
            const uint32_t ge_e = (((ssum & 0x00FF00FFu) | 0x01000100u) - (rhs & 0x00FF00FFu)) & 0x01000100u;
            const uint32_t ge_o = ((((ssum >> 8) & 0x00FF00FFu) | 0x01000100u) - ((rhs >> 8) & 0x00FF00FFu)) & 0x01000100u;
            const uint32_t ge_s = (ge_e >> 1) | (ge_o << 7);
            const uint32_t contested = ~(ge_q & ge_s & ~differ & valid) & bmask & 0x80808080u;
            if (act) { *(uint32_t *)(resb + c4) = tn4; *(uint32_t *)(resq + c4) = tqm; }
#pragma unroll
            for (int k = 0; k < 4; k++) cq[k] = (contested >> (8 * k + 7)) & 1u;
        }
#pragma unroll
        for (int k = 0; k < 4; k++) {
            const unsigned long long mk = __ballot(cq[k]);
            if (cq[k]) cplx[n_cplx + lanes_below(mk)] = (uint16_t)(c4 + k);
            n_cplx += __popcll(mk);
        }
    } else
    for (int it = 0; it * 64 < nbytes; it++) {
        const int bi = it * 64 + lane, col0 = bi * 2;
        const bool a0 = col0 < len, a1 = col0 + 1 < len;
        uint32_t pm0 = 0, pm1 = 0; int ss0 = 0, ss1 = 0, tq0 = 0, tq1 = 0, qor = 0;
        for (unsigned long long m = vmask; m; m &= m - 1) {
            const int v = __ffsll((long long)m) - 1;
            const uint64_t vso = rl64(so, v), vqo = rl64(qo, v); const int vld = left_mode ? 0 : rl32(ld, v), vlq = rl32(lq, v);
            const int r0 = col0 + vld, r1 = r0 + 1;
            const uint8_t *vs = b.seq + vso; const uint8_t *vq = b.qual + vqo; const int8_t *vsc = w.score + vqo;
            const uint32_t vpatch = (uint32_t)rl32((int)patch, v);
            const bool in0 = a0 && r0 >= 0 && r0 < vlq, in1 = a1 && r1 >= 0 && r1 < vlq;
            if (in0 && in1 && !(r0 & 1)) {
                uint8_t sb = vs[r0 >> 1];
                uint16_t qq = *(const u16_unaligned *)(vq + r0);
                int q0 = qq & 0xFF, q1 = qq >> 8;
                pm0 |= 1u << (sb >> 4); pm1 |= 1u << (sb & 0xF);
                ss0 += d_score_at(p, vsc, vpatch, r0, q0); ss1 += d_score_at(p, vsc, vpatch, r1, q1);
                tq0 = max(tq0, q0); tq1 = max(tq1, q1); qor |= q0 | q1;
            } else {
                if (in0) { int q0 = vq[r0]; pm0 |= 1u << d_nib(vs, r0); ss0 += d_score_at(p, vsc, vpatch, r0, q0); tq0 = max(tq0, q0); qor |= q0; }
                if (in1) { int q1 = vq[r1]; pm1 |= 1u << d_nib(vs, r1); ss1 += d_score_at(p, vsc, vpatch, r1, q1); tq1 = max(tq1, q1); qor |= q1; }
            }
        }
        if ((qor & 0x80) || ((pm0 | pm1) & ~0x8116u)) odd = true;
        bool c0 = false, c1 = false;
        if (a0) {
            uint8_t ob = oseq[bi];
            resb[col0] = ob >> 4; resq[col0] = (uint8_t)tq0;
            c0 = !(__popc(pm0) == 1 && ss0 >= accept_score && tq0 >= p.moderate_q);
            if (a1) { resb[col0 + 1] = ob & 0xF; resq[col0 + 1] = (uint8_t)tq1; c1 = !(__popc(pm1) == 1 && ss1 >= accept_score && tq1 >= p.moderate_q); }
        }
        unsigned long long m0 = __ballot(c0), m1 = __ballot(c1);
        if (c0) cplx[n_cplx + lanes_below(m0)] = (uint16_t)col0;
        n_cplx += __popcll(m0);
        if (c1) cplx[n_cplx + lanes_below(m1)] = (uint16_t)(col0 + 1);
        n_cplx += __popcll(m1);
    }
    WAVE_SYNC();
    int minc = 0;
    {
        uint32_t *tl = (uint32_t *)(s_res_wave + 2048);
        uint8_t *vlist = s_res_wave + 2048 + 32 * 5 * 4 * 4;
        if (take) vlist[lanes_below(vmask)] = (uint8_t)lane;
        const uint32_t magic = ((1u << 20) + (uint32_t)nvot - 1) / (uint32_t)nvot;
        for (int cbase = 0; cbase < n_cplx; cbase += 32) {
            const int ncol = min(32, n_cplx - cbase);
            for (int k = lane; k < 32 * 5; k += 64) *(uint4 *)(tl + 4 * k) = make_uint4(0, 0, 0, 0);
            WAVE_SYNC();
            int ref4 = 0;
            if (ref && lane < ncol) {
                const int ro = ref_off_fast(ocig, o_nc, o_c0, cplx[cbase + lane]);
                if (ro >= 0 && (int64_t)o_pos + ro < ref_len) ref4 = d_ref_nib(ref, (int64_t)o_pos + ro);
            }
            const int items = ncol * nvot;
            for (int ibase = 0; ibase < items; ibase += 64) {
                const int item = ibase + lane;
                const bool live = item < items;
                const int it_ = live ? item : 0;
                const int c = (int)(((uint32_t)it_ * magic) >> 20), kx = it_ - c * nvot;
                const int vl = vlist[kx], col = cplx[cbase + c];
                const uint64_t vso = (uint64_t)__shfl((long long)so, vl), vqo = (uint64_t)__shfl((long long)qo, vl);
                const int vld = left_mode ? 0 : __shfl(ld, vl), vlq = __shfl(lq, vl);
                const uint32_t vpatch = (uint32_t)__shfl((int)patch, vl);
                const int rp = col + vld;
                if (live && rp >= 0 && rp < vlq) {
                    const int nb = d_nib(b.seq + vso, rp), q = b.qual[vqo + rp], sc = d_score_at(p, w.score + vqo, vpatch, rp, q);
                    const int bin = nb == 1 ? 0 : nb == 2 ? 1 : nb == 4 ? 2 : nb == 8 ? 3 : nb == 15 ? 4 : -1;
                    if (bin < 0 || (q & 0x80)) odd = true;
                    else {
                        uint32_t *t4 = tl + (c * 5 + bin) * 4;
                        atomicAdd(t4, 1u); atomicAdd(t4 + 1, (uint32_t)sc); atomicAdd(t4 + 2, (uint32_t)q); atomicMax(t4 + 3, (uint32_t)q);
                    }
                }
            }
            WAVE_SYNC();
            if (lane < ncol) {
                const int col = cplx[cbase + lane];
                Tally5 t; t.total = 0;
#pragma unroll
                for (int k = 0; k < 5; k++) {
                    const uint4 v4 = *(const uint4 *)(tl + (lane * 5 + k) * 4);
                    t.cnt[k] = (int)v4.x; t.ss[k] = (int)v4.y; t.qs[k] = (int)v4.z; t.tq[k] = (int)v4.w; t.total += (int)v4.y;
                }
                ColOut r = decide_column_packed(t, p, resb[col], ref4);
                resb[col] = (uint8_t)r.base; resq[col] = (uint8_t)r.qual; minc += r.minc;
            }
            WAVE_SYNC();
        }
    }
    WAVE_SYNC();
    if (__any(odd)) {
        if (lane == 0) w.slow_list[atomicAdd(&w.si->n_slow, 1u)] = gi * 2 + (is_left ? 0 : 1);
        return false;
    }
    minc = wave_sum(minc);
    bool restore = false;
    if (minc != 0) {
        if (o_nm_type == 0) { if (lane == 0) raise_error(w.si, GCE_ERR_NM_MISSING, out); restore = true; }
        else if (minc > 5) restore = true;
        else if (lane == 0) { int nn = o_nm + minc; if (o_nm_type == 'C' && nn >= 0 && nn <= 255) w.rp_nm[gi * 2 + (is_left ? 0 : 1)] = nn; }
    }
    if (!restore) {
        for (int bi = lane; bi < nbytes; bi += 64) {
            const int c0 = 2 * bi;
            if (c0 + 1 < len) { oseq[bi] = (uint8_t)((resb[c0] << 4) | resb[c0 + 1]); *(u16_unaligned *)(oqual + c0) = (uint16_t)(resq[c0] | (resq[c0 + 1] << 8)); }
            else { oseq[bi] = (uint8_t)((resb[c0] << 4) | (oseq[bi] & 0xF)); oqual[c0] = resq[c0]; }
        }
    }
    if (lane == 0) rp_out[gi] = out;
    return true;
}

__global__ __launch_bounds__(256, 5) void k_consensus_fast(DevBatch b, DevParams p, Work w) {
    __shared__ __attribute__((aligned(16))) uint8_t s_res[WAVES_PER_BLOCK][2048 + 2560 + 64];
    const int lane = lane_id(), wv = threadIdx.x >> 6;
    const uint32_t n = (uint32_t)(w.si->hand_on >> 32);
    uint32_t n_done = 0;
    for (uint32_t idx = blockIdx.x * WAVES_PER_BLOCK + wv; idx < n; idx += gridDim.x * WAVES_PER_BLOCK) {
        const uint32_t e = w.gen_list[idx];
        if (consensus_fast_side(b, p, w, e >> 1, !(e & 1), s_res[wv], lane)) n_done++;
        WAVE_SYNC();
    }
    if (lane == 0 && n_done) atomicAdd(&w.si->cs_fast, n_done);
}

__device__ inline int d_duplex_merge_bam(const DevBatch &b, uint32_t r1, uint32_t r2, int lane) {
    int l1 = b.core[r1].l_qseq, l2 = b.core[r2].l_qseq;
    int len = min(l1, l2), diff = 0;
    uint8_t *s1 = b.seq + b.seq_off[r1], *q1 = b.qual + b.qual_off[r1];
    const uint8_t *s2 = b.seq + b.seq_off[r2];
    const int nb = (len + 1) >> 1;
    bool phase_odd = false;
    for (int base = 0; base < nb; base += 64) {
        int k = base + lane;
        bool valid = k < nb;
        uint8_t x = valid ? s1[k] : 0, y = valid ? s2[k] : 0;
        int xh = x >> 4, xl = x & 0xF, yh = y >> 4, yl = y & 0xF;
        bool has_lo = (2 * k + 1) < len;
        bool ne = valid && x != y;
        bool mark_hi = ne && d_base_class(xh) != d_base_class(yh);
        bool to_odd = mark_hi && xl == yl && has_lo;
        unsigned long long EQ = __ballot(!ne), TO = __ballot(to_odd);
        unsigned long long oddin = 0;
        int pos = 0; bool st = phase_odd;
        while (pos < 64) {
            if (!st) {
                unsigned long long m = TO & (~0ull << pos);
                if (!m) { pos = 64; break; }
                pos = __ffsll((long long)m);
                st = true;
            } else {
                unsigned long long m = ~EQ & (~0ull << pos);
                int nx = m ? __ffsll((long long)m) - 1 : 64;
                unsigned long long upto = nx >= 63 ? ~0ull : ((2ull << nx) - 1ull);
                oddin |= upto & (~0ull << pos);
                if (nx == 64) pos = 64; else { pos = nx + 1; st = false; }
            }
        }
        phase_odd = st;
        bool in_odd = (oddin >> lane) & 1ull;
        if (ne) {
            if (!in_odd) {
                if (mark_hi) { diff++; xh = 15; q1[2 * k] = 0; }
                if (has_lo && !(mark_hi && xl == yl) && d_base_class(xl) != d_base_class(yl)) { diff++; xl = 15; q1[2 * k + 1] = 0; }
            } else if (has_lo && d_base_class(xl) != d_base_class(yl)) { diff++; xl = 15; q1[2 * k + 1] = 0; }
            s1[k] = (uint8_t)((xh << 4) | xl);
        }
    }
    return wave_sum(diff) + (l1 > l2 ? l1 - l2 : l2 - l1);
}

__device__ inline void d_emit_pair(const Work &w, uint32_t gi, bool duplex) {
    uint32_t l = w.rp_left[gi], r = w.rp_right[gi];
    int fr = (int)min(w.rp_merge[gi], 65535u) & 0xFF;
    int rr = (int)min(w.rp_rmerge[gi], 65535u) & 0xFF;
    OutRec o; o.fr = (int16_t)fr; o.rr = duplex ? (int16_t)rr : (int16_t)-1; o.pad = 0;
    if (l != NONE32) { w.out_flag[l] = 1; o.qname_src = w.rp_qsl[gi]; o.mate = r; o.nm_new = (int16_t)w.rp_nm[gi * 2]; w.orec[l] = o; }
    if (r != NONE32) { w.out_flag[r] = 1; o.qname_src = w.rp_qsr[gi]; o.mate = l; o.nm_new = (int16_t)w.rp_nm[gi * 2 + 1]; w.orec[r] = o; }
}

__global__ __launch_bounds__(256) void k_group_tail(DevBatch b, DevParams p, Work w, uint32_t n_groups) {
    const uint32_t gi = blockIdx.x * blockDim.x + threadIdx.x;
    if (gi >= n_groups) return;
    const uint32_t c = w.gl_cluster[gi];
    const uint32_t begin = w.g_begin[gi], np = w.g_np[gi];
    const uint8_t cflags = w.cl_hasumi[c];
    const uint32_t G = w.cl_ngroups[c];
    if (d_group_skipped(p, cflags, G, np)) {
        w.rp_left[gi] = w.gpl[begin]; w.rp_right[gi] = w.gpr[begin];
        w.rp_supp[gi] = 1; w.rp_state[gi] = RP_DROPPED;
        return;
    }
    uint32_t left = w.rp_left[gi], right = w.rp_right[gi];
    {
        const int2 nv = *reinterpret_cast<const int2 *>(w.rp_nm + 2 * (size_t)gi);
        if (NM_IS_DEFERRED(nv.x) || NM_IS_DEFERRED(nv.y)) {
            int2 o = nv;
            auto resolve = [&](int v, uint32_t out) -> int {
                if (!NM_IS_DEFERRED(v)) return v;
                const int minc = v - NM_DEFER, ty = b.nm_type[out], nn = b.nm[out] + minc;
                if (ty == 0) { raise_error(w.si, GCE_ERR_NM_MISSING, out); return -1; }
                return (minc <= 5 && ty == 'C' && nn >= 0 && nn <= 255) ? nn : -1;
            };
            o.x = resolve(nv.x, left); o.y = resolve(nv.y, right);
            *reinterpret_cast<int2 *>(w.rp_nm + 2 * (size_t)gi) = o;
        }
    }
    const bool single = np == 1 && w.gpr[begin] == NONE32;
    uint32_t qsl = left, qsr = right;
    const uint64_t uL = left != NONE32 ? w.uinfo[left] : 0ull, uR = right != NONE32 ? w.uinfo[right] : 0ull;
    if (!single) {
        if (cflags & 2) {
            uint32_t ntc = NONE32; int bl = 0;
            for (uint32_t k = 0; k < np; k++) {
                uint32_t l = w.gpl[begin + k];
                int ll = d_lqname_pad(b.core[l]);
                if (ntc == NONE32 || ll < bl || (ll == bl && d_strcmp(d_qname(b, l), d_qname(b, ntc)) < 0)) { ntc = l; bl = ll; }
            }
            if (left != NONE32 && ntc != NONE32 && ntc != left) {
                if (d_lqname_pad(b.core[left]) < d_lqname_pad(b.core[ntc])) raise_error(w.si, GCE_ERR_QNAME_SHORT, left);
                qsl = ntc;
            }
        } else if (left != NONE32 && right != NONE32) {
            if (uinfo_lqname_pad(uL) <= uinfo_lqname_pad(uR)) qsr = left;
            else qsl = right;
        }
    }
    w.rp_qsl[gi] = qsl; w.rp_qsr[gi] = qsr;
    const uint32_t merge = single ? 1 : np;
    const bool duplex_cluster = (cflags & 1) && !p.disable_duplex && G >= 2;
    const char *u = nullptr; int ul = 0;
    if ((cflags & 1) || b.mi) {
        auto rec_umi = [&](uint64_t vrec, uint32_t src, const char *&uo, int &ulo) {
            if (uinfo_hm(vrec)) { uo = uinfo_ptr(b, vrec); ulo = uinfo_len(vrec); return; }
            const uint64_t vn = src == left ? uL : (src == right ? uR : w.uinfo[src]);
            if (!uinfo_hm(vn)) { uo = uinfo_ptr(b, vn); ulo = uinfo_len(vn); return; }
            const char *q = d_qname(b, src); int s0, l0;
            d_umi_slice(q, p, s0, l0);
            uo = q + s0; ulo = l0;
        };
        if (left != NONE32) rec_umi(uL, qsl, u, ul);
        if (right != NONE32) {
            const char *u2; int ul2;
            rec_umi(uR, qsr, u2, ul2);
            if (left != NONE32 && ul != 0) {
                bool same = ul == ul2;
                if (same && u == u2) { }
                else if (same && ul <= 24) { uint64_t a[3], c3[3]; load_be_words<3>(u, ul, a); load_be_words<3>(u2, ul2, c3); same = a[0] == c3[0] && a[1] == c3[1] && a[2] == c3[2]; }
                else if (same) same = d_bytes_equal(u, ul, u2, ul2);
                if (!same) raise_error(w.si, GCE_ERR_UMI_MISMATCH, right);
            }
            u = u2; ul = ul2;
        }
    }
    w.rp_merge[gi] = merge; w.rp_rmerge[gi] = 0; w.rp_umi[gi] = u; w.rp_umilen[gi] = (uint16_t)ul;
    if (duplex_cluster) { w.rp_state[gi] = RP_PENDING; w.rp_supp[gi] = -1; return; }
    const bool outp = !p.duplex_only && (int)merge >= p.cluster_size_req;
    w.rp_supp[gi] = (int)merge; w.rp_state[gi] = outp ? RP_OUT_SSCS : RP_DROPPED;
    if (outp) d_emit_pair(w, gi, false);
}

__device__ bool finish_cluster_lanes(const DevBatch &b, const DevParams &p, const Work &w, uint32_t g0, uint32_t G, int lane) {
    const bool in = lane < (int)G;
    const uint32_t gme = g0 + (uint32_t)lane;
    uint32_t l = NONE32, r = NONE32, m = 0; uint64_t t0 = 0, t1 = 0; bool two = false, lng = false;
    if (in) {
        const char *u = w.rp_umi[gme]; const int ul = w.rp_umilen[gme];
        l = w.rp_left[gme]; r = w.rp_right[gme]; m = w.rp_merge[gme];
        int s0, l0, s1, l1;
        two = d_split2(u, ul, s0, l0, s1, l1) == 2;
        if (two) {
            if (l0 > 8 || l1 > 8) lng = true;
            else { uint64_t a[1], c2[1]; load_be_words<1>(u + s0, l0, a); load_be_words<1>(u + s1, l1, c2); t0 = a[0]; t1 = c2[0]; }
        }
    }
    if (__any(lng)) return false;
    int st = RP_PENDING;
    for (int idx = (int)G - 1; idx >= 0; idx--) {
        if (__shfl(st, idx) == RP_CONSUMED) continue;
        const uint64_t a0 = (uint64_t)__shfl((long long)t0, idx), a1 = (uint64_t)__shfl((long long)t1, idx);
        const int atwo = __shfl((int)two, idx);
        const bool hit = lane < idx && st == RP_PENDING && two && atwo && a0 == t1 && a1 == t0;
        const unsigned long long hm = __ballot(hit);
        const uint32_t gi = g0 + (uint32_t)idx;
        const uint32_t l1 = (uint32_t)__shfl((int)l, idx), r1 = (uint32_t)__shfl((int)r, idx), m1 = (uint32_t)__shfl((int)m, idx);
        if (hm) {
            const int found = __ffsll((long long)hm) - 1;
            const uint32_t g2 = g0 + (uint32_t)found;
            const uint32_t l2 = (uint32_t)__shfl((int)l, found), r2 = (uint32_t)__shfl((int)r, found), m2 = (uint32_t)__shfl((int)m, found);
            int diff = 0;
            if (l1 != NONE32 && l2 != NONE32) diff += d_duplex_merge_bam(b, l1, l2, lane);
            if (r1 != NONE32 && r2 != NONE32) diff += d_duplex_merge_bam(b, r1, r2, lane);
            const bool outp = diff <= p.duplex_mismatch_thr && (int)(m1 + m2) >= p.cluster_size_req;
            if (lane == idx) st = outp ? RP_OUT_DCS : RP_DROPPED;
            if (lane == found) st = RP_CONSUMED;
            if (lane == 0) {
                w.rp_supp[gi] = (int)(m1 + m2);
                w.rp_rmerge[gi] = m2;
                w.rp_state[gi] = outp ? RP_OUT_DCS : RP_DROPPED;
                w.rp_state[g2] = RP_CONSUMED;
                if (outp) d_emit_pair(w, gi, true);
            }
            WAVE_SYNC();
        } else {
            const bool outp = !p.duplex_only && (int)m1 >= p.cluster_size_req;
            if (lane == idx) st = outp ? RP_OUT_SSCS : RP_DROPPED;
            if (lane == 0) { w.rp_supp[gi] = (int)m1; w.rp_state[gi] = outp ? RP_OUT_SSCS : RP_DROPPED; if (outp) d_emit_pair(w, gi, false); }
        }
    }
    return true;
}
__device__ void finish_cluster(const DevBatch &b, const DevParams &p, const Work &w, uint32_t c, int lane) {
    const uint32_t G = w.cl_ngroups[c];
    const uint32_t g0 = w.cl_gbase[c];
    if (G <= 64u && finish_cluster_lanes(b, p, w, g0, G, lane)) return;
    for (int idx = (int)G - 1; idx >= 0; idx--) {
        uint32_t gi = g0 + idx;
        if (w.rp_state[gi] == RP_CONSUMED) continue;
        const char *u1 = w.rp_umi[gi]; int ul1 = w.rp_umilen[gi];
        uint32_t found = NONE32;
        for (int base = 0; base < idx && found == NONE32; base += 64) {
            int i = base + lane;
            bool hit = i < idx && w.rp_state[g0 + i] == RP_PENDING && d_is_duplex(u1, ul1, w.rp_umi[g0 + i], w.rp_umilen[g0 + i]);
            unsigned long long m = __ballot(hit);
            if (m) found = base + (__ffsll((long long)m) - 1);
        }
        uint32_t l1 = w.rp_left[gi], r1 = w.rp_right[gi], m1 = w.rp_merge[gi];
        if (found != NONE32) {
            uint32_t g2 = g0 + found;
            uint32_t l2 = w.rp_left[g2], r2 = w.rp_right[g2], m2 = w.rp_merge[g2];
            int diff = 0;
            if (l1 != NONE32 && l2 != NONE32) diff += d_duplex_merge_bam(b, l1, l2, lane);
            if (r1 != NONE32 && r2 != NONE32) diff += d_duplex_merge_bam(b, r1, r2, lane);
            bool outp = diff <= p.duplex_mismatch_thr && (int)(m1 + m2) >= p.cluster_size_req;
            if (lane == 0) {
                w.rp_supp[gi] = (int)(m1 + m2);
                w.rp_rmerge[gi] = m2;
                w.rp_state[gi] = outp ? RP_OUT_DCS : RP_DROPPED;
                w.rp_state[g2] = RP_CONSUMED;
                if (outp) d_emit_pair(w, gi, true);
            }
        } else {
            bool outp = !p.duplex_only && (int)m1 >= p.cluster_size_req;
            if (lane == 0) { w.rp_supp[gi] = (int)m1; w.rp_state[gi] = outp ? RP_OUT_SSCS : RP_DROPPED; if (outp) d_emit_pair(w, gi, false); }
        }
        WAVE_SYNC();
    }
}
__global__ __launch_bounds__(256) void k_finish_screen(Work w, uint32_t n_clusters, uint8_t *flag) {
    const uint32_t c = blockIdx.x * blockDim.x + threadIdx.x;
    if (c < n_clusters) flag[c] = w.cl_ngroups[c] >= 2 && (w.cl_hasumi[c] & 1);
}
__global__ __launch_bounds__(256) void k_finish(DevBatch b, DevParams p, Work w, const uint32_t *list, const unsigned long long *list_n) {
    const int lane = lane_id();
    const uint32_t n = (uint32_t)*list_n;
    for (uint32_t k = blockIdx.x * WAVES_PER_BLOCK + (threadIdx.x >> 6); k < n; k += gridDim.x * WAVES_PER_BLOCK) {
        finish_cluster(b, p, w, list[k], lane);
        WAVE_SYNC();
    }
}

__global__ __launch_bounds__(256) void k_raw_emit(DevBatch b, DevParams p, Work w, uint32_t n_clusters) {
    const uint32_t c = blockIdx.x * blockDim.x + threadIdx.x;
    if (c >= n_clusters || d_thr_mode(w.cl_ikey[c], w.si, p) != THR_RAW) return;
    const uint32_t start = w.cl_start[c], n = w.cl_n[c];
    auto same = [&](const char *x, const char *y) { int k = 0; while (x[k] && x[k] == y[k]) k++; return x[k] == y[k]; };
    for (uint32_t a = 0; a < n; a++) {
        const uint32_t ra = w.members[start + a];
        const char *qa = d_qname(b, ra);
        bool first = true;
        for (uint32_t x = 0; x < n && first; x++) { const uint32_t rx = w.members[start + x]; if (rx < ra && same(qa, d_qname(b, rx))) first = false; }
        if (!first) continue;
        uint32_t right = NONE32, prev = ra; uint64_t pu = w.uinfo[ra];
        for (;;) {
            uint32_t nx = NONE32;
            for (uint32_t x = 0; x < n; x++) { const uint32_t rx = w.members[start + x]; if (rx > prev && rx < nx && same(qa, d_qname(b, rx))) nx = rx; }
            if (nx == NONE32) break;
            const uint64_t u = w.uinfo[nx];
            const int ul = uinfo_len(u), pl = uinfo_len(pu);
            bool eq = ul == pl;
            if (eq) { const char *s1 = uinfo_ptr(b, u), *s2 = uinfo_ptr(b, pu); for (int k = 0; k < ul; k++) eq = eq && s1[k] == s2[k]; }
            if (pl != 0 && !eq) raise_error(w.si, GCE_ERR_UMI_MISMATCH, nx); else pu = u;
            right = nx; prev = nx;
        }
        OutRec o; o.nm_new = -1; o.fr = -1; o.rr = -1; o.pad = 0;
        w.out_flag[ra] = 1; o.qname_src = ra; o.mate = right; w.orec[ra] = o;
        if (right != NONE32) { w.out_flag[right] = 1; o.qname_src = right; o.mate = ra; w.orec[right] = o; }
        atomicAdd((unsigned long long *)&w.si->post[8], 1ull); atomicAdd((unsigned long long *)&w.si->post[14 + 1], 1ull);
        atomicAdd((unsigned long long *)&w.si->post[right != NONE32 ? 10 : 9], 1ull);
    }
}

__global__ __launch_bounds__(256) void k_stats(DevBatch b, Work w, uint32_t n_clusters, uint32_t n_groups) {
    __shared__ unsigned long long s_pre[GCE_STATS_WORDS], s_post[GCE_STATS_WORDS], s_np;
    for (int k = threadIdx.x; k < GCE_STATS_WORDS; k += blockDim.x) { s_pre[k] = 0; s_post[k] = 0; }
    if (threadIdx.x == 0) s_np = 0;
    __syncthreads();
    const uint64_t tid0 = (uint64_t)blockIdx.x * blockDim.x + threadIdx.x, stride = (uint64_t)gridDim.x * blockDim.x;
    long long pre[14] = {0, 0, 0, 0, 0, 0, 0, 0, 0, 0, 0, 0, 0, 0}, post[14] = {0, 0, 0, 0, 0, 0, 0, 0, 0, 0, 0, 0, 0, 0}, np = 0, post_h1 = 0;
    for (uint64_t c = tid0; c < n_clusters; c += stride) {
        uint32_t G = w.cl_ngroups[c];
        if (G == 0) continue;
        pre[6] += 1; if (G > 1) pre[7] += 1;
        np += w.cl_npairs[c];
        uint32_t nr = 0; { const uint32_t g0 = w.cl_gbase[c]; for (uint32_t g = 0; g < G; g++) { uint8_t st = w.rp_state[g0 + g]; nr += (st == RP_OUT_SSCS || st == RP_OUT_DCS); } }
        if (nr > 0) { post[6] += 1; if (nr > 1) post[7] += 1; }
    }
    for (uint64_t g = tid0; g < n_groups; g += stride) {
        int supp = w.rp_supp[g];
        if (supp < 0) continue;
        bool pe = w.rp_left[g] != NONE32 && w.rp_right[g] != NONE32;
        pre[8] += 1;
        if (supp < GCE_MAX_SUPPORTING_READS) atomicAdd(&s_pre[14 + supp], 1ull); else pre[13] += 1;
        pre[pe ? 10 : 9] += 1;
        uint8_t st = w.rp_state[g];
        if (st == RP_OUT_SSCS || st == RP_OUT_DCS) {
            post[st == RP_OUT_DCS ? 12 : 11] += 1;
            post[8] += 1; post_h1 += 1; post[pe ? 10 : 9] += 1;
        }
    }
    const int lane = lane_id();
#pragma unroll
    for (int k = 0; k < 14; k++) {
        const long long a = wave_sum64(pre[k]), c2 = wave_sum64(post[k]);
        if (lane == 0) { if (a) atomicAdd(&s_pre[k], (unsigned long long)a); if (c2) atomicAdd(&s_post[k], (unsigned long long)c2); }
    }
    { const long long a = wave_sum64(np), c2 = wave_sum64(post_h1); if (lane == 0) { if (a) atomicAdd(&s_np, (unsigned long long)a); if (c2) atomicAdd(&s_post[14 + 1], (unsigned long long)c2); } }
    __syncthreads();
    for (int k = threadIdx.x; k < GCE_STATS_WORDS; k += blockDim.x) {
        if (s_pre[k]) atomicAdd((unsigned long long *)&w.si->pre[k], s_pre[k]);
        if (s_post[k]) atomicAdd((unsigned long long *)&w.si->post[k], s_post[k]);
    }
    if (threadIdx.x == 0 && s_np) atomicAdd(&w.si->n_pairs_total, s_np);
}

__global__ __launch_bounds__(256) void k_flag_reduce(const uint8_t *flag, uint64_t n, uint64_t *part) {
    __shared__ uint64_t s[4];
    uint64_t base = (uint64_t)blockIdx.x * SCAN_TILE, v = 0;
    for (int k = 0; k < SCAN_TILE / 256; k++) { uint64_t i = base + k * 256 + threadIdx.x; v += (i < n && flag[i]) ? 1 : 0; }
    v = (uint64_t)wave_sum64((long long)v);
    if (lane_id() == 0) s[threadIdx.x >> 6] = v;
    __syncthreads();
    if (threadIdx.x == 0) part[blockIdx.x] = (s[0] + s[1] + s[2] + s[3]) << 32;
}
__global__ __launch_bounds__(256) void k_flag_apply(const uint8_t *flag, uint64_t n, const uint64_t *part, uint32_t *out_index) {
    __shared__ uint32_t s_w[4];
    __shared__ uint32_t s_carry;
    const int lane = lane_id(), wv = threadIdx.x >> 6;
    if (threadIdx.x == 0) s_carry = (uint32_t)(part[blockIdx.x] >> 32);
    __syncthreads();
    uint64_t base = (uint64_t)blockIdx.x * SCAN_TILE;
    for (int k = 0; k < SCAN_TILE / 256; k++) {
        uint64_t i = base + k * 256 + threadIdx.x;
        bool f = i < n && flag[i];
        unsigned long long m = __ballot(f);
        if (lane == 0) s_w[wv] = __popcll(m);
        __syncthreads();
        uint32_t woff = 0;
        for (int q = 0; q < wv; q++) woff += s_w[q];
        uint32_t carry = s_carry;
        if (f) out_index[carry + woff + lanes_below(m)] = (uint32_t)i;
        __syncthreads();
        if (threadIdx.x == 0) s_carry = carry + s_w[0] + s_w[1] + s_w[2] + s_w[3];
        __syncthreads();
    }
}
```

Before: 1.917 billion.

## Fuse per-group statistics into k_group_tail and skip duplex pass when UMIs lack underscores

Statistics for non-duplex groups are now accumulated inside k_group_tail through ballots, shared-memory counters and slotted global atomics, so k_stats only scans duplex clusters and runs only when the duplex pass ran. The clustering kernel records whether any UMI contains an underscore or comes from an MI tag; when none do, the duplex screen/finish kernels and k_stats are skipped. Non-duplex groups also avoid writing many rp_* arrays. The StreamInfo publish can copy only the head portion, which shrinks the host-mapped copy on intermediate syncs. This adds host and device folding of the new tail slots and depends on the underscore heuristic correctly deciding when duplex pairing is impossible.

```diff
diff --git a/gencore_amd/csrc/engine.hip b/gencore_amd/csrc/engine.hip
--- a/gencore_amd/csrc/engine.hip
+++ b/gencore_amd/csrc/engine.hip
@@ -269,6 +269,16 @@
     return GCE_OK;
 }
 
+__host__ __device__ inline void si_add_tail(StreamInfo *si, int k, long long a) {
+    switch (k) {
+    case TS_PRE_CLUSTERS: si->pre[6] += a; break;   case TS_PRE_MULTI: si->pre[7] += a; break;   case TS_PRE_MOLECULES: si->pre[8] += a; break;
+    case TS_PRE_SE: si->pre[9] += a; break;         case TS_PRE_PE: si->pre[10] += a; break;     case TS_PRE_UNCOUNTED: si->pre[13] += a; break;
+    case TS_NPAIRS: si->n_pairs_total += (unsigned long long)a; break;
+    case TS_POST_CLUSTERS: si->post[6] += a; break; case TS_POST_MULTI: si->post[7] += a; break;
+    case TS_POST_SSCS: si->post[11] += a; si->post[8] += a; si->post[14 + 1] += a; break;
+    case TS_POST_SE: si->post[9] += a; break;       case TS_POST_PE: si->post[10] += a; break;
+    }
+}
 struct PreExtra { long long v[6]; };
 __global__ void k_fold_stats(StreamInfo *si, PreExtra x) {
     const int k = threadIdx.x;
@@ -276,6 +286,16 @@
         long long a = 0, c = 0;
         for (int q = 0; q < GCE_PRE_SLOTS; q++) { a += si->pre_slot[q][k]; c += si->post_slot[q][k]; si->pre_slot[q][k] = 0; si->post_slot[q][k] = 0; }
         si->pre[k] += a + x.v[k]; si->post[k] += c;
+    }
+    if (k < TS_WORDS) {
+        long long a = 0;
+        for (int q = 0; q < GCE_TAIL_SLOTS; q++) { a += si->tail_slot[q][k]; si->tail_slot[q][k] = 0; }
+        si_add_tail(si, k, a);
+    }
+    for (int h = k; h < GCE_MAX_SUPPORTING_READS; h += blockDim.x) {
+        long long a = 0;
+        for (int q = 0; q < GCE_TAIL_HSLOTS; q++) { a += si->tail_hist[q][h]; si->tail_hist[q][h] = 0; }
+        si->pre[14 + h] += a;
     }
 }
 __global__ void k_first_contig_ge(const gce_core *core, int64_t n, int32_t maxc, unsigned int *out) {
@@ -500,16 +520,16 @@
     return GCE_OK;
 }
 
-__global__ __launch_bounds__(256) void k_publish_si(const StreamInfo *si, StreamInfo *host, unsigned long long *flag, unsigned long long seq) {
+__global__ __launch_bounds__(256) void k_publish_si(const StreamInfo *si, StreamInfo *host, unsigned long long *flag, unsigned long long seq, unsigned n_words) {
     const uint32_t *src = reinterpret_cast<const uint32_t *>(si);
     uint32_t *dst = reinterpret_cast<uint32_t *>(host);
-    for (unsigned i = threadIdx.x; i < sizeof(StreamInfo) / 4; i += 256) dst[i] = src[i];
+    for (unsigned i = threadIdx.x; i < n_words; i += 256) dst[i] = src[i];
     __threadfence_system();
     __syncthreads();
     if (threadIdx.x == 0) __hip_atomic_store(flag, seq, __ATOMIC_RELEASE, __HIP_MEMORY_SCOPE_SYSTEM);
 }
-static_assert(sizeof(StreamInfo) % 4 == 0, "k_publish_si copies words");
-static int read_si_begin(gce_engine *e, unsigned long long *seq_out) {
+static_assert(sizeof(StreamInfo) % 4 == 0 && GCE_SI_HEAD_BYTES % 4 == 0, "k_publish_si copies words");
+static int read_si_begin(gce_engine *e, unsigned long long *seq_out, bool head_only = false) {
     *seq_out = 0;
     static const bool sync_copy = getenv("GCE_SYNC_COPY") != nullptr;
     if (!sync_copy && !e->si_pin) {
@@ -524,7 +544,7 @@
     if (!sync_copy && e->si_pin) {
         unsigned long long *dflag = reinterpret_cast<unsigned long long *>(reinterpret_cast<char *>(e->si_pin_dev) + ((sizeof(StreamInfo) + 7) & ~size_t(7)));
         const unsigned long long seq = ++e->si_seq;
-        hipLaunchKernelGGL(k_publish_si, dim3(1), dim3(256), 0, e->stream, (const StreamInfo *)e->si.p, reinterpret_cast<StreamInfo *>(e->si_pin_dev), dflag, seq);
+        hipLaunchKernelGGL(k_publish_si, dim3(1), dim3(256), 0, e->stream, (const StreamInfo *)e->si.p, reinterpret_cast<StreamInfo *>(e->si_pin_dev), dflag, seq, (unsigned)((head_only ? GCE_SI_HEAD_BYTES : sizeof(StreamInfo)) / 4));
         HIPCHK(hipGetLastError());
         *seq_out = seq;
     }
@@ -551,12 +571,14 @@
         HIPCHK(hipStreamSynchronize(e->stream));
     }
     for (int k = 0; k < 6; k++) for (int q = 0; q < GCE_PRE_SLOTS; q++) { e->h_si.pre[k] += e->h_si.pre_slot[q][k]; e->h_si.post[k] += e->h_si.post_slot[q][k]; }
+    for (int k = 0; k < TS_WORDS; k++) { long long a = 0; for (int q = 0; q < GCE_TAIL_SLOTS; q++) a += e->h_si.tail_slot[q][k]; si_add_tail(&e->h_si, k, a); }
+    for (int h = 0; h < GCE_MAX_SUPPORTING_READS; h++) for (int q = 0; q < GCE_TAIL_HSLOTS; q++) e->h_si.pre[14 + h] += e->h_si.tail_hist[q][h];
     if (e->h_si.err_key != ~0ull) { e->dev_error = -(int)(e->h_si.err_key & 0xFF); e->dev_error_read = (uint32_t)(e->h_si.err_key >> 8); }
     return GCE_OK;
 }
-static int read_si(gce_engine *e) {
+static int read_si(gce_engine *e, bool head_only = false) {
     unsigned long long seq = 0;
-    const int rc = read_si_begin(e, &seq);
+    const int rc = read_si_begin(e, &seq, head_only);
     return rc != GCE_OK ? rc : read_si_end(e, seq);
 }
 
@@ -619,6 +641,7 @@
     PreExtra pre_extra{};
     int64_t n_sblk = 0, max_events = 0; unsigned nblk_N = 0;
     bool si_behind_describe = false;
+    bool duplex_ran = false;
     explicit Step(gce_engine *e_) : e(e_), s(e_->stream), hb(e_->dev_batch) {}
 
     int check_and_cut() {
@@ -766,7 +789,7 @@
     int describe() {
         int rc;
         unsigned long long si_seq1 = 0;
-        if ((rc = read_si_begin(e, &si_seq1)) != GCE_OK) return rc;
+        if ((rc = read_si_begin(e, &si_seq1, true)) != GCE_OK) return rc;
         if (N > 0) {
 #ifndef GCE_DESCRIBE_BLOCKS
 #define GCE_DESCRIBE_BLOCKS 32768
@@ -848,7 +871,7 @@
         hipLaunchKernelGGL(k_u64_partials, dim3(1), dim3(1024), 0, s, w.scan_part, (const unsigned long long *)&w.si->n_groups, &w.si->vote_weight, &w.si->n_live);
         LAUNCH_EV(k_vote_batches, dim3(nblk_N), dim3(256), s, e->ev[EV_PAIRING], w, (const unsigned long long *)&w.si->n_groups, (const uint64_t *)w.scan_part);
         CANARY("EV_PAIRING");
-        if ((rc = read_si(e)) != GCE_OK) return rc;
+        if ((rc = read_si(e, true)) != GCE_OK) return rc;
         HIPCHK(hipGetLastError());
         si_behind_describe = true;
         NG = (uint32_t)e->h_si.n_groups;
@@ -903,8 +926,10 @@
             hipLaunchKernelGGL(k_vote_deep, dim3(1024), dim3(DV_T), 0, s, b, p, w);
             LAUNCH_EV(k_consensus_slow, dim3(512), dim3(256), s, e->ev[EV_CONSENSUS], (const SlowArgs *)e->slow_args.p);
             CANARY("EV_CONSENSUS");
-            hipLaunchKernelGGL(k_group_tail, dim3(cdiv(NG, 256)), dim3(256), 0, s, b, p, w, NG);
-            if (!p.disable_duplex) {
+            const bool duplex_on = !p.disable_duplex && !(si_behind_describe && e->h_si.umi_us == 0u);
+            hipLaunchKernelGGL(k_group_tail, dim3(cdiv(NG, 256)), dim3(256), 0, s, b, p, w, NG, (int)duplex_on);
+            duplex_ran = duplex_on;
+            if (duplex_on) {
                 hipLaunchKernelGGL(k_finish_screen, dim3(cdiv(C, 256)), dim3(256), 0, s, w, C, w.pf_flag);
                 compact_flags(w.pf_flag, w.pf_list, &w.si->n_pf_items);
                 hipLaunchKernelGGL(k_finish, dim3(4096), dim3(256), 0, s, b, p, w, (const uint32_t *)w.pf_list, (const unsigned long long *)&w.si->n_pf_items);
@@ -930,7 +955,7 @@
             TAKE(o_key, o.key, n1 * sizeof(OutKey)); TAKE(o_rec, o.rec, n1 * sizeof(OutRec)); TAKE(o_ksoff, o.ksoff, n1 * 8); TAKE(o_kqoff, o.kqoff, n1 * 8); TAKE(o_krow, o.krow, n1 * 4); TAKE(o_rank64, o.rank64, (n1 / 64 + 2) * 4);
             const unsigned nblk_O = cdiv(n1, OUT_TILE); TAKE(o_part3, o.part3, (size_t)nblk_O * 24 + 64);
             if (e->h_si.n_raw > 0 && C > 0) hipLaunchKernelGGL(k_raw_emit, dim3(cdiv(C, 256)), dim3(256), 0, s, b, p, w, C);
-            hipLaunchKernelGGL(k_stats, dim3(1024), dim3(256), 0, s, b, w, (NG > 0 ? C : 0u), NG);
+            if (duplex_ran) hipLaunchKernelGGL(k_stats, dim3(1024), dim3(256), 0, s, b, w, NG);
             CANARY("k_stats");
             hipLaunchKernelGGL(k_out_reduce, dim3(nblk_O), dim3(OUT_T), 0, s, b, w, o);
             CANARY("k_out_reduce");
diff --git a/gencore_amd/csrc/gce_cluster.hpp b/gencore_amd/csrc/gce_cluster.hpp
--- a/gencore_amd/csrc/gce_cluster.hpp
+++ b/gencore_amd/csrc/gce_cluster.hpp
@@ -493,6 +493,7 @@
     __shared__ long long s_stat[WAVES_PER_BLOCK][6];
     long long st[6] = {0, 0, 0, 0, 0, 0};
     int lqmin = 0x7FFFFFFF, lqmax = -1;
+    bool any_us = false;
     const int lane = lane_id(), wv = threadIdx.x >> 6;
     for (int cb = 0; cb < tiles_per_block; cb++) {
         const int64_t i = ((int64_t)blockIdx.x * tiles_per_block + cb) * 256 + threadIdx.x;
@@ -524,10 +525,11 @@
                 const char *src2; uint8_t hm = 0;
                 if (b.mi && b.mi_off[i] != 0xFFFFFFFFFFFFFFFFull) { src2 = b.mi + b.mi_off[i]; hm = 1; }
                 else src2 = b.qname + b.qname_off[i];
-                int s0, l0;
-                if (!d_umi_slice(src2, p, s0, l0, hm ? -1 : (int)k.l_qname - 1)) { raise_error(w.si, GCE_ERR_UMI_PARSE, (uint32_t)i); s0 = 0; l0 = 0; }
+                int s0, l0; bool us;
+                if (!d_umi_slice(src2, p, s0, l0, hm ? -1 : (int)k.l_qname - 1, us)) { raise_error(w.si, GCE_ERR_UMI_PARSE, (uint32_t)i); s0 = 0; l0 = 0; }
                 if (l0 > UINFO_MAXLEN) { raise_error(w.si, GCE_ERR_UMI_PARSE, (uint32_t)i); l0 = 0; }
                 w.uinfo[i] = uinfo_pack((hm ? b.mi_off[i] : b.qname_off[i]) + (uint64_t)s0, hm != 0, k.l_qname, l0);
+                any_us |= us || hm;
             }
         }
     }
@@ -537,6 +539,7 @@
         if (lqmin < *(volatile int *)&w.si->lq_min) atomicMin(&w.si->lq_min, lqmin);
         if (lqmax > *(volatile int *)&w.si->lq_max) atomicMax(&w.si->lq_max, lqmax);
     }
+    if (__any(any_us) && lane == 0 && *(volatile unsigned int *)&w.si->umi_us == 0u) atomicOr(&w.si->umi_us, 1u);
     __syncthreads();
     if (threadIdx.x < 6) {
         long long v = s_stat[0][threadIdx.x] + s_stat[1][threadIdx.x] + s_stat[2][threadIdx.x] + s_stat[3][threadIdx.x];
diff --git a/gencore_amd/csrc/gce_device.hpp b/gencore_amd/csrc/gce_device.hpp
--- a/gencore_amd/csrc/gce_device.hpp
+++ b/gencore_amd/csrc/gce_device.hpp
@@ -51,6 +51,8 @@
 };
 
 #define GCE_PRE_SLOTS 64
+#define GCE_TAIL_SLOTS 16
+#define GCE_TAIL_HSLOTS 8
 struct StreamInfo {
     unsigned long long n_clustered;
     unsigned int first_unmapped;
@@ -83,7 +85,13 @@
     long long post[GCE_STATS_WORDS];
     long long post_slot[GCE_PRE_SLOTS][8];
     long long pre_slot[GCE_PRE_SLOTS][8];
+    unsigned int umi_us;
+    unsigned int pad_us;
+    long long tail_slot[GCE_TAIL_SLOTS][16];
+    long long tail_hist[GCE_TAIL_HSLOTS][GCE_MAX_SUPPORTING_READS];
 };
+#define GCE_SI_HEAD_BYTES offsetof(StreamInfo, tail_slot)
+enum { TS_PRE_CLUSTERS = 0, TS_PRE_MULTI, TS_PRE_MOLECULES, TS_PRE_SE, TS_PRE_PE, TS_PRE_UNCOUNTED, TS_NPAIRS, TS_POST_CLUSTERS, TS_POST_MULTI, TS_POST_SSCS, TS_POST_SE, TS_POST_PE, TS_WORDS };
 
 __device__ __forceinline__ void raise_error(StreamInfo *si, int code, uint32_t read) {
     atomicMin(&si->err_key, ((unsigned long long)read << 8) | (unsigned long long)((-code) & 0xFF));
@@ -239,10 +247,11 @@
     return upto_z & ~upto_a;
 }
 
-__device__ inline bool d_umi_slice_bytes(const char *s, const DevParams &p, int &start, int &len, int n);
-
-__device__ inline bool d_umi_slice(const char *s, const DevParams &p, int &start, int &len, int n = -1) {
-    if (n < 0 || p.prefix_len > 4) return d_umi_slice_bytes(s, p, start, len, n);
+__device__ inline bool d_umi_slice_bytes(const char *s, const DevParams &p, int &start, int &len, int n, bool &has_us);
+
+__device__ inline bool d_umi_slice(const char *s, const DevParams &p, int &start, int &len, int n, bool &has_us) {
+    has_us = false;
+    if (n < 0 || p.prefix_len > 4) return d_umi_slice_bytes(s, p, start, len, n, has_us);
     const int base = n > 32 ? n - 32 : 0, nwin = n - base;
     uint64_t w[4];
 #pragma unroll
@@ -261,21 +270,24 @@
     }
     if (wpos < 0) {
         if (base == 0) return true;
-        return d_umi_slice_bytes(s, p, start, len, n);
+        return d_umi_slice_bytes(s, p, start, len, n, has_us);
     }
     if (p.prefix_len > 0) {
         const int wst = wpos + 2;
         if (base + wst > n) return false;
         int l = nwin - wst;
         bool open = true;
+        uint64_t us = 0;
 #pragma unroll
         for (int k = 0; k < 4; k++) {
             if (open && 8 * k + 8 > wst && 8 * k < nwin) {
-                const uint64_t stop = ~d_umi_bytes(w[k]) & 0x8080808080808080ull & d_range_bytes(wst, nwin, k);
+                const uint64_t rng = d_range_bytes(wst, nwin, k), e_us = d_eq_bytes(w[k], '_');
+                const uint64_t stop = ~(d_eq_bytes(w[k], 'A') | d_eq_bytes(w[k], 'T') | d_eq_bytes(w[k], 'C') | d_eq_bytes(w[k], 'G') | e_us) & 0x8080808080808080ull & rng;
+                us |= e_us & rng & (stop ? (stop & (0ull - stop)) - 1ull : ~0ull);
                 if (stop) { l = 8 * k + ((__ffsll((long long)stop) - 1) >> 3) - wst; open = false; }
             }
         }
-        start = base + wst; len = l;
+        start = base + wst; len = l; has_us = us != 0;
         return true;
     }
     const int sep = base + wpos;
@@ -290,13 +302,14 @@
     int st = sep + 1;
     { const int j = wpos + 1; const char c = (char)(w[j >> 3] >> (8 * (j & 7))); if (st < n - 1 && c == '_') { st++; us--; } }
     if (!ok || us > 1) return true;
-    start = st; len = n - st;
+    start = st; len = n - st; has_us = us > 0;
     return true;
 }
-
-__device__ inline bool d_umi_slice_bytes(const char *s, const DevParams &p, int &start, int &len, int n) {
+__device__ inline bool d_umi_slice(const char *s, const DevParams &p, int &start, int &len, int n = -1) { bool u; return d_umi_slice(s, p, start, len, n, u); }
+
+__device__ inline bool d_umi_slice_bytes(const char *s, const DevParams &p, int &start, int &len, int n, bool &has_us) {
     if (n < 0) { n = 0; while (s[n]) n++; }
-    start = 0; len = 0;
+    start = 0; len = 0; has_us = false;
     if (p.prefix_len > 0) {
         int pos = -1;
         for (int i = n - 1; i >= 0; i--) {
@@ -309,7 +322,7 @@
         int st = pos + 2;
         if (st > n) return false;
         int l = 0;
-        while (st + l < n && d_is_umi_char(s[st + l])) l++;
+        while (st + l < n && d_is_umi_char(s[st + l])) { has_us |= s[st + l] == '_'; l++; }
         start = st; len = l;
         return true;
     }
@@ -325,7 +338,7 @@
     int st = sep + 1;
     if (st < n - 1 && s[st] == '_') { st++; us--; }
     if (!ok || us > 1) return true;
-    start = st; len = n - st;
+    start = st; len = n - st; has_us = us > 0;
     return true;
 }
 
diff --git a/gencore_amd/csrc/gce_kernels.hpp b/gencore_amd/csrc/gce_kernels.hpp
--- a/gencore_amd/csrc/gce_kernels.hpp
+++ b/gencore_amd/csrc/gce_kernels.hpp
@@ -1567,45 +1567,56 @@
     return wave_sum(diff) + (l1 > l2 ? l1 - l2 : l2 - l1);
 }
 
-__device__ inline void d_emit_pair(const Work &w, uint32_t gi, bool duplex) {
-    uint32_t l = w.rp_left[gi], r = w.rp_right[gi];
-    int fr = (int)min(w.rp_merge[gi], 65535u) & 0xFF;
-    int rr = (int)min(w.rp_rmerge[gi], 65535u) & 0xFF;
+__device__ inline void d_emit_pair(const Work &w, uint32_t l, uint32_t r, uint32_t merge, uint32_t rmerge, uint32_t qsl, uint32_t qsr, int nml, int nmr, bool duplex) {
+    int fr = (int)min(merge, 65535u) & 0xFF;
+    int rr = (int)min(rmerge, 65535u) & 0xFF;
     OutRec o; o.fr = (int16_t)fr; o.rr = duplex ? (int16_t)rr : (int16_t)-1; o.pad = 0;
-    if (l != NONE32) { w.out_flag[l] = 1; o.qname_src = w.rp_qsl[gi]; o.mate = r; o.nm_new = (int16_t)w.rp_nm[gi * 2]; w.orec[l] = o; }
-    if (r != NONE32) { w.out_flag[r] = 1; o.qname_src = w.rp_qsr[gi]; o.mate = l; o.nm_new = (int16_t)w.rp_nm[gi * 2 + 1]; w.orec[r] = o; }
-}
-
-__global__ __launch_bounds__(256) void k_group_tail(DevBatch b, DevParams p, Work w, uint32_t n_groups) {
-    const uint32_t gi = blockIdx.x * blockDim.x + threadIdx.x;
-    if (gi >= n_groups) return;
-    const uint32_t c = w.gl_cluster[gi];
+    if (l != NONE32) { w.out_flag[l] = 1; o.qname_src = qsl; o.mate = r; o.nm_new = (int16_t)nml; w.orec[l] = o; }
+    if (r != NONE32) { w.out_flag[r] = 1; o.qname_src = qsr; o.mate = l; o.nm_new = (int16_t)nmr; w.orec[r] = o; }
+}
+__device__ inline void d_emit_group(const Work &w, uint32_t gi, uint32_t l, uint32_t r, uint32_t merge, uint32_t rmerge, bool duplex) {
+    const int2 nv = *reinterpret_cast<const int2 *>(w.rp_nm + 2 * (size_t)gi);
+    d_emit_pair(w, l, r, merge, rmerge, w.rp_qsl[gi], w.rp_qsr[gi], nv.x, nv.y, duplex);
+}
+
+enum { TF_FINAL = 1, TF_PE = 2, TF_OUT = 4, TF_CFIRST = 8, TF_CMULTI = 16, TF_POSTC = 32, TF_POSTM = 64 };
+__device__ __forceinline__ uint32_t d_group_tail(const DevBatch &b, const DevParams &p, const Work &w, uint32_t gi, bool duplex_on, uint32_t &supp, uint32_t &cl_pairs) {
+    const uint32_t c = w.gl_cluster[gi], c_prev = gi ? w.gl_cluster[gi - 1] : NONE32;
     const uint32_t begin = w.g_begin[gi], np = w.g_np[gi];
+    const uint32_t left = w.rp_left[gi], right = w.rp_right[gi];
+    int2 nmv = *reinterpret_cast<const int2 *>(w.rp_nm + 2 * (size_t)gi);
     const uint8_t cflags = w.cl_hasumi[c];
     const uint32_t G = w.cl_ngroups[c];
+    const uint64_t uL = left != NONE32 ? w.uinfo[left] : 0ull, uR = right != NONE32 ? w.uinfo[right] : 0ull;
+    const bool duplex_cluster = duplex_on && (cflags & 1) && !p.disable_duplex && G >= 2;
+    uint32_t tf = 0;
+    if (!duplex_cluster && c_prev != c) {
+        tf |= TF_CFIRST | (G > 1 ? TF_CMULTI : 0);
+        cl_pairs = w.cl_npairs[c];
+        if (G > 1 && !p.duplex_only) {
+            uint32_t nr = 0;
+            for (uint32_t g = 0; g < G && nr < 2; g++) nr += (int)w.g_np[gi + g] >= p.cluster_size_req;
+            tf |= (nr > 0 ? TF_POSTC : 0) | (nr > 1 ? TF_POSTM : 0);
+        }
+    }
     if (d_group_skipped(p, cflags, G, np)) {
-        w.rp_left[gi] = w.gpl[begin]; w.rp_right[gi] = w.gpr[begin];
-        w.rp_supp[gi] = 1; w.rp_state[gi] = RP_DROPPED;
-        return;
-    }
-    uint32_t left = w.rp_left[gi], right = w.rp_right[gi];
+        supp = 1;
+        return tf | TF_FINAL | ((w.gpl[begin] != NONE32 && w.gpr[begin] != NONE32) ? TF_PE : 0);
+    }
     {
-        const int2 nv = *reinterpret_cast<const int2 *>(w.rp_nm + 2 * (size_t)gi);
-        if (NM_IS_DEFERRED(nv.x) || NM_IS_DEFERRED(nv.y)) {
-            int2 o = nv;
+        if (NM_IS_DEFERRED(nmv.x) || NM_IS_DEFERRED(nmv.y)) {
             auto resolve = [&](int v, uint32_t out) -> int {
                 if (!NM_IS_DEFERRED(v)) return v;
                 const int minc = v - NM_DEFER, ty = b.nm_type[out], nn = b.nm[out] + minc;
                 if (ty == 0) { raise_error(w.si, GCE_ERR_NM_MISSING, out); return -1; }
                 return (minc <= 5 && ty == 'C' && nn >= 0 && nn <= 255) ? nn : -1;
             };
-            o.x = resolve(nv.x, left); o.y = resolve(nv.y, right);
-            *reinterpret_cast<int2 *>(w.rp_nm + 2 * (size_t)gi) = o;
+            nmv.x = resolve(nmv.x, left); nmv.y = resolve(nmv.y, right);
+            if (duplex_cluster) *reinterpret_cast<int2 *>(w.rp_nm + 2 * (size_t)gi) = nmv;
         }
     }
     const bool single = np == 1 && w.gpr[begin] == NONE32;
     uint32_t qsl = left, qsr = right;
-    const uint64_t uL = left != NONE32 ? w.uinfo[left] : 0ull, uR = right != NONE32 ? w.uinfo[right] : 0ull;
     if (!single) {
         if (cflags & 2) {
             uint32_t ntc = NONE32; int bl = 0;
@@ -1623,9 +1634,7 @@
             else qsl = right;
         }
     }
-    w.rp_qsl[gi] = qsl; w.rp_qsr[gi] = qsr;
     const uint32_t merge = single ? 1 : np;
-    const bool duplex_cluster = (cflags & 1) && !p.disable_duplex && G >= 2;
     const char *u = nullptr; int ul = 0;
     if ((cflags & 1) || b.mi) {
         auto rec_umi = [&](uint64_t vrec, uint32_t src, const char *&uo, int &ulo) {
@@ -1650,11 +1659,46 @@
             u = u2; ul = ul2;
         }
     }
-    w.rp_merge[gi] = merge; w.rp_rmerge[gi] = 0; w.rp_umi[gi] = u; w.rp_umilen[gi] = (uint16_t)ul;
-    if (duplex_cluster) { w.rp_state[gi] = RP_PENDING; w.rp_supp[gi] = -1; return; }
+    if (duplex_cluster) {
+        w.rp_qsl[gi] = qsl; w.rp_qsr[gi] = qsr;
+        w.rp_merge[gi] = merge; w.rp_rmerge[gi] = 0; w.rp_umi[gi] = u; w.rp_umilen[gi] = (uint16_t)ul;
+        w.rp_state[gi] = RP_PENDING; w.rp_supp[gi] = -1;
+        return tf;
+    }
     const bool outp = !p.duplex_only && (int)merge >= p.cluster_size_req;
-    w.rp_supp[gi] = (int)merge; w.rp_state[gi] = outp ? RP_OUT_SSCS : RP_DROPPED;
-    if (outp) d_emit_pair(w, gi, false);
+    if (outp) d_emit_pair(w, left, right, merge, 0u, qsl, qsr, nmv.x, nmv.y, false);
+    if (G == 1 && outp) tf |= TF_POSTC;
+    supp = merge;
+    return tf | TF_FINAL | ((left != NONE32 && right != NONE32) ? TF_PE : 0) | (outp ? TF_OUT : 0);
+}
+__global__ __launch_bounds__(256) void k_group_tail(DevBatch b, DevParams p, Work w, uint32_t n_groups, int duplex_on) {
+    __shared__ unsigned int s_hist[GCE_MAX_SUPPORTING_READS];
+    __shared__ unsigned long long s_ts[TS_WORDS];
+    if (threadIdx.x < GCE_MAX_SUPPORTING_READS) s_hist[threadIdx.x] = 0;
+    if (threadIdx.x < TS_WORDS) s_ts[threadIdx.x] = 0;
+    __syncthreads();
+    const uint32_t gi = blockIdx.x * blockDim.x + threadIdx.x;
+    uint32_t tf = 0, supp = 0, cl_pairs = 0;
+    if (gi < n_groups) tf = d_group_tail(b, p, w, gi, duplex_on != 0, supp, cl_pairs);
+    const bool fin = tf & TF_FINAL, out = tf & TF_OUT, pe = tf & TF_PE;
+    const bool uncounted = fin && supp >= (uint32_t)GCE_MAX_SUPPORTING_READS;
+    if (fin && !uncounted) atomicAdd(&s_hist[supp], 1u);
+    unsigned int cnt[TS_WORDS];
+    cnt[TS_PRE_CLUSTERS] = __popcll(__ballot(tf & TF_CFIRST)); cnt[TS_PRE_MULTI] = __popcll(__ballot(tf & TF_CMULTI));
+    cnt[TS_PRE_MOLECULES] = __popcll(__ballot(fin)); cnt[TS_PRE_SE] = __popcll(__ballot(fin && !pe)); cnt[TS_PRE_PE] = __popcll(__ballot(fin && pe));
+    cnt[TS_PRE_UNCOUNTED] = __popcll(__ballot(uncounted));
+    cnt[TS_NPAIRS] = 0;
+    cnt[TS_POST_CLUSTERS] = __popcll(__ballot(tf & TF_POSTC)); cnt[TS_POST_MULTI] = __popcll(__ballot(tf & TF_POSTM));
+    cnt[TS_POST_SSCS] = __popcll(__ballot(out)); cnt[TS_POST_SE] = __popcll(__ballot(out && !pe)); cnt[TS_POST_PE] = __popcll(__ballot(out && pe));
+    const long long npw = wave_sum64((long long)cl_pairs);
+    if (lane_id() == 0) {
+#pragma unroll
+        for (int k = 0; k < TS_WORDS; k++) if (cnt[k]) atomicAdd(&s_ts[k], (unsigned long long)cnt[k]);
+        if (npw) atomicAdd(&s_ts[TS_NPAIRS], (unsigned long long)npw);
+    }
+    __syncthreads();
+    if (threadIdx.x < TS_WORDS && s_ts[threadIdx.x]) atomicAdd((unsigned long long *)&w.si->tail_slot[blockIdx.x & (GCE_TAIL_SLOTS - 1)][threadIdx.x], s_ts[threadIdx.x]);
+    if (threadIdx.x < GCE_MAX_SUPPORTING_READS && s_hist[threadIdx.x]) atomicAdd((unsigned long long *)&w.si->tail_hist[(blockIdx.x >> 4) & (GCE_TAIL_HSLOTS - 1)][threadIdx.x], (unsigned long long)s_hist[threadIdx.x]);
 }
 
 __device__ bool finish_cluster_lanes(const DevBatch &b, const DevParams &p, const Work &w, uint32_t g0, uint32_t G, int lane) {
@@ -1696,13 +1740,13 @@
                 w.rp_rmerge[gi] = m2;
                 w.rp_state[gi] = outp ? RP_OUT_DCS : RP_DROPPED;
                 w.rp_state[g2] = RP_CONSUMED;
-                if (outp) d_emit_pair(w, gi, true);
+                if (outp) d_emit_group(w, gi, l1, r1, m1, m2, true);
             }
             WAVE_SYNC();
         } else {
             const bool outp = !p.duplex_only && (int)m1 >= p.cluster_size_req;
             if (lane == idx) st = outp ? RP_OUT_SSCS : RP_DROPPED;
-            if (lane == 0) { w.rp_supp[gi] = (int)m1; w.rp_state[gi] = outp ? RP_OUT_SSCS : RP_DROPPED; if (outp) d_emit_pair(w, gi, false); }
+            if (lane == 0) { w.rp_supp[gi] = (int)m1; w.rp_state[gi] = outp ? RP_OUT_SSCS : RP_DROPPED; if (outp) d_emit_group(w, gi, l1, r1, m1, 0u, false); }
         }
     }
     return true;
@@ -1735,11 +1779,11 @@
                 w.rp_rmerge[gi] = m2;
                 w.rp_state[gi] = outp ? RP_OUT_DCS : RP_DROPPED;
                 w.rp_state[g2] = RP_CONSUMED;
-                if (outp) d_emit_pair(w, gi, true);
+                if (outp) d_emit_group(w, gi, l1, r1, m1, m2, true);
             }
         } else {
             bool outp = !p.duplex_only && (int)m1 >= p.cluster_size_req;
-            if (lane == 0) { w.rp_supp[gi] = (int)m1; w.rp_state[gi] = outp ? RP_OUT_SSCS : RP_DROPPED; if (outp) d_emit_pair(w, gi, false); }
+            if (lane == 0) { w.rp_supp[gi] = (int)m1; w.rp_state[gi] = outp ? RP_OUT_SSCS : RP_DROPPED; if (outp) d_emit_group(w, gi, l1, r1, m1, 0u, false); }
         }
         WAVE_SYNC();
     }
@@ -1788,22 +1832,23 @@
     }
 }
 
-__global__ __launch_bounds__(256) void k_stats(DevBatch b, Work w, uint32_t n_clusters, uint32_t n_groups) {
+__global__ __launch_bounds__(256) void k_stats(DevBatch b, Work w, uint32_t n_groups) {
     __shared__ unsigned long long s_pre[GCE_STATS_WORDS], s_post[GCE_STATS_WORDS], s_np;
     for (int k = threadIdx.x; k < GCE_STATS_WORDS; k += blockDim.x) { s_pre[k] = 0; s_post[k] = 0; }
     if (threadIdx.x == 0) s_np = 0;
     __syncthreads();
     const uint64_t tid0 = (uint64_t)blockIdx.x * blockDim.x + threadIdx.x, stride = (uint64_t)gridDim.x * blockDim.x;
     long long pre[14] = {0, 0, 0, 0, 0, 0, 0, 0, 0, 0, 0, 0, 0, 0}, post[14] = {0, 0, 0, 0, 0, 0, 0, 0, 0, 0, 0, 0, 0, 0}, np = 0, post_h1 = 0;
-    for (uint64_t c = tid0; c < n_clusters; c += stride) {
-        uint32_t G = w.cl_ngroups[c];
-        if (G == 0) continue;
-        pre[6] += 1; if (G > 1) pre[7] += 1;
-        np += w.cl_npairs[c];
-        uint32_t nr = 0; { const uint32_t g0 = w.cl_gbase[c]; for (uint32_t g = 0; g < G; g++) { uint8_t st = w.rp_state[g0 + g]; nr += (st == RP_OUT_SSCS || st == RP_OUT_DCS); } }
-        if (nr > 0) { post[6] += 1; if (nr > 1) post[7] += 1; }
-    }
     for (uint64_t g = tid0; g < n_groups; g += stride) {
+        const uint32_t c = w.gl_cluster[g];
+        const uint32_t G = w.cl_ngroups[c];
+        if (!(w.cl_hasumi[c] & 1) || G < 2) continue;
+        if (g == 0 || w.gl_cluster[g - 1] != c) {
+            pre[6] += 1; pre[7] += 1;
+            np += w.cl_npairs[c];
+            uint32_t nr = 0; for (uint32_t k = 0; k < G; k++) { uint8_t st = w.rp_state[g + k]; nr += (st == RP_OUT_SSCS || st == RP_OUT_DCS); }
+            if (nr > 0) { post[6] += 1; if (nr > 1) post[7] += 1; }
+        }
         int supp = w.rp_supp[g];
         if (supp < 0) continue;
         bool pe = w.rp_left[g] != NONE32 && w.rp_right[g] != NONE32;
```

After: 1.961 billion (median of 6 runs). +2.3%, better.
